# hsinnan75/GSAlign

Hardware: AMD Instinct MI355X
Metric: aligned query Gbp/s (whole node) (higher is better)
Workload: dtype u8; 1 GPU; full-human-sized pair (BASELINE configs[4]): 24 contigs with GRCh38 chromosome lengths, 3.08 Gbp, repeat injection, vs 1; inflight_contexts_per_gpu=8, world_size=1, parallelism=one GPU

## Files before the change

### gsalign_amd/csrc/gsa_api.hip

```cpp
#include <algorithm>
#include <atomic>
#include <chrono>
#include <cstring>
#include <mutex>
#include <thread>
#include <pthread.h>
#include <sched.h>
#include "gsa_ctx.h"

static thread_local std::string g_create_error;

int gsa_fail(gsa_ctx *ctx, int code, const std::string &msg)
{
	if (ctx) ctx->err = msg; else g_create_error = msg;
	return code;
}

int host_stage4_5_6(gsa_ctx *c, int stage);
int host_stage8_finish(gsa_ctx *c);
int build_block_view(gsa_ctx *c);
void bundle_split_lists(gsa_ctx *c);
void bundle_join_lists(gsa_ctx *c);

void collect_events(gsa_ctx *c)
{
	if (!c->profiling && !c->prof_seed) { c->ev_pending = 0; return; }
	float ms;
	if ((c->ev_pending & 1) && !c->profiling) { if (hipEventElapsedTime(&ms, c->ev[0], c->ev[1]) == hipSuccess) { c->kernel_ms[0] = ms; c->acc_seed_ms += ms; } c->ev_pending = 0; (void)hipGetLastError(); return; }
	if (c->ev_pending & 1) {
		if (hipEventElapsedTime(&ms, c->ev[0], c->ev[1]) == hipSuccess) c->kernel_ms[0] = ms;
		if (hipEventElapsedTime(&ms, c->ev[1], c->ev[2]) == hipSuccess) c->kernel_ms[1] = ms;
		if (hipEventElapsedTime(&ms, c->ev[2], c->ev[3]) == hipSuccess) c->kernel_ms[2] = ms;
	}
	if (c->ev_pending & 2) { if (hipEventElapsedTime(&ms, c->ev[4], c->ev[5]) == hipSuccess) c->kernel_ms[3] = ms; }
	c->ev_pending = 0;
	(void)hipGetLastError();
}

void Uploader::run()
{
	(void)hipSetDevice(device);
	for (;;) {
		Job j;
		{ std::unique_lock<std::mutex> g(mu); cv.wait(g, [&] { return stop || !q.empty(); }); if (q.empty()) return; j = std::move(q.front()); q.pop_front(); if (n_demand > 0) n_demand--; }
		const auto t0 = std::chrono::steady_clock::now();
		hipError_t e_first = hipSuccess;
		for (const Piece &p : j.pieces) if (p.n) { const hipError_t e = hipMemcpyAsync(p.dst, p.src, p.n, hipMemcpyHostToDevice, st); if (e != hipSuccess && e_first == hipSuccess) e_first = e; bytes += p.n; }
		{ const hipError_t e = hipStreamSynchronize(st); if (e != hipSuccess && e_first == hipSuccess) e_first = e; }
		(void)hipGetLastError();
		if (e_first != hipSuccess && j.err) { int none = 0; j.err->compare_exchange_strong(none, (int)e_first); }
		const auto t1 = std::chrono::steady_clock::now();
		{ std::lock_guard<std::mutex> g(mu); copy_ms += std::chrono::duration<double, std::milli>(t1 - t0).count(); wait_ms += std::chrono::duration<double, std::milli>(t0 - j.t_push).count(); jobs++; }
		j.busy->fetch_sub(1, std::memory_order_release);
	}
}

static int uploader_start(gsa_ctx *c)
{
	Uploader *u = new Uploader(); u->device = c->device;
	if (hipStreamCreateWithFlags(&u->st, hipStreamNonBlocking) != hipSuccess) { delete u; return gsa_fail(c, GSA_ERR_HIP, "hipStreamCreate (upload stream)"); }
	u->th = std::thread([u] { u->run(); });
	c->up = u; c->own_up = true;
	return GSA_OK;
}

static void uploader_stop(gsa_ctx *c)
{
	if (!c->up || !c->own_up) { c->up = nullptr; return; }
	Uploader *u = c->up;
	{ std::lock_guard<std::mutex> g(u->mu); u->stop = true; }
	u->cv.notify_all();
	if (u->th.joinable()) u->th.join();
#ifdef GSA_EXPERIMENTS
	if (getenv("GSA_UP_STATS") && u->jobs) fprintf(stderr, "[uploader] %lld jobs, %.1f MB each, %.2f ms in the queue, %.2f ms copying (%.1f GB/s)\n", (long long)u->jobs, u->bytes / 1e6 / u->jobs, u->wait_ms / u->jobs, u->copy_ms / u->jobs, u->bytes / 1e6 / u->copy_ms);
#endif
	if (u->st) hipStreamDestroy(u->st);
	delete u; c->up = nullptr;
}

static inline void slot_wait(QuerySlot &s) { while (s.busy.load(std::memory_order_acquire) > 0) std::this_thread::yield(); }
static void slot_demand(gsa_ctx *c, QuerySlot &s)
{
	if (s.busy.load(std::memory_order_acquire) > 0 && c->up) {
		Uploader *u = c->up;
		std::lock_guard<std::mutex> g(u->mu);
		for (size_t k = u->n_demand; k < u->q.size(); k++) if (u->q[k].busy == &s.busy) {
			Uploader::Job j = std::move(u->q[k]); u->q.erase(u->q.begin() + (long)k); u->q.insert(u->q.begin() + (long)u->n_demand, std::move(j)); u->n_demand++;
			break;
		}
	}
	slot_wait(s);
}

static int ctx_private_init(gsa_ctx *c, gsa_ctx *share = nullptr)
{
#ifdef GSA_EXPERIMENTS
	static const int prio = [] { const char *e = getenv("GSA_STREAM_PRIO"); return e ? atoi(e) : 0; }();
	if (prio) {
		int lo = 0, hi = 0; GSA_CHECK(c, hipDeviceGetStreamPriorityRange(&lo, &hi));
		GSA_CHECK(c, hipStreamCreateWithPriority(&c->stream, hipStreamDefault, hi));
		for (int i = 0; i < 4; i++) GSA_CHECK(c, hipStreamCreateWithPriority(&c->stream_aux[i], hipStreamDefault, (i == 0 || i == 3 || (prio > 1 && i == 1)) ? lo : hi));
	} else
#endif
	if (c->prio_mode > 0) {
		int lo = 0, hi = 0; GSA_CHECK(c, hipDeviceGetStreamPriorityRange(&lo, &hi));
		const int mid = (lo + hi) / 2;
		GSA_CHECK(c, hipStreamCreateWithPriority(&c->stream, hipStreamDefault, hi));
		GSA_CHECK(c, hipStreamCreateWithPriority(&c->stream_seed, hipStreamDefault, c->prio_mode == 2 ? lo : mid));
		GSA_CHECK(c, hipEventCreateWithFlags(&c->ev_seed_fork, hipEventDisableTiming));
		for (int i = 0; i < 4; i++) GSA_CHECK(c, hipStreamCreateWithPriority(&c->stream_aux[i], hipStreamDefault, (c->prio_mode == 3 && (i == 0 || i == 3)) ? lo : mid));
	} else {
	GSA_CHECK(c, hipStreamCreate(&c->stream));
	for (int i = 0; i < 4; i++) GSA_CHECK(c, hipStreamCreate(&c->stream_aux[i]));
	}
	if (share) { c->up = share->up; c->own_up = false; } else if (int rc = uploader_start(c)) return rc;
	for (int i = 0; i < 28; i++) GSA_CHECK(c, hipEventCreate(&c->ev[i]));
	GSA_CHECK(c, hipMalloc(&c->d_zero.p, 256)); c->d_zero.cap = 256; GSA_CHECK(c, hipMemset(c->d_zero.p, 0, 256));
	GSA_CHECK(c, hipMalloc(&c->d_cnt.p, 32 * sizeof(u64))); c->d_cnt.cap = 32 * sizeof(u64); GSA_CHECK(c, hipMemset(c->d_cnt.p, 0, 32 * sizeof(u64)));
	GSA_CHECK(c, hipHostMalloc((void **)&c->h_cnt, 16 * sizeof(u64)));
	GSA_CHECK(c, hipMalloc(&c->d_mail.p, MAIL_N * sizeof(i32))); c->d_mail.cap = MAIL_N * sizeof(i32);
	GSA_CHECK(c, hipMemset(c->d_mail.p, 0, MAIL_N * sizeof(i32)));
	GSA_CHECK(c, hipHostMalloc((void **)&c->h_mail, MAIL_N * sizeof(i32)));
	return GSA_OK;
}

static hipError_t h2d_big(void *dst, const void *src, size_t bytes)
{
	if (bytes >= ((size_t)64 << 20) && hipHostRegister(const_cast<void *>(src), bytes, hipHostRegisterDefault) == hipSuccess) {
		const hipError_t e = hipMemcpy(dst, src, bytes, hipMemcpyHostToDevice);
		(void)hipHostUnregister(const_cast<void *>(src));
		return e;
	}
	(void)hipGetLastError();
	return hipMemcpy(dst, src, bytes, hipMemcpyHostToDevice);
}

struct ReservedBuf { void *p = nullptr; size_t bytes = 0; };
static std::mutex g_res_mu; static ReservedBuf g_res[64][2];
void *dev_take_reserved(int device, size_t bytes, size_t *got)
{
	std::lock_guard<std::mutex> g(g_res_mu);
	for (int k = 0; k < 2; k++) { ReservedBuf &r = g_res[device & 63][k]; if (r.p && r.bytes >= bytes && r.bytes <= bytes + bytes / 8 + 4096) { void *p = r.p; *got = r.bytes; r.p = nullptr; r.bytes = 0; return p; } }
	return nullptr;
}

extern "C" {

void gsa_default_params(gsa_params *p)
{
	p->min_seed_len = 15; p->max_indel = 25; p->min_block_score = 200; p->min_aln_len = 200; p->min_identity = 70;
	p->sensitive = 0; p->one_on_one = 0;
}

const char *gsa_last_error(gsa_ctx *ctx) { return ctx ? ctx->err.c_str() : g_create_error.c_str(); }

static int reset_run_state(gsa_ctx *c)
{
	if (c->early_in_flight) { GSA_CHECK(c, hipStreamSynchronize(c->stream_aux[0])); c->early_in_flight = false; }
	c->n_early = 0; c->early_listed = false; c->early_consumed = false;
	c->stage = 0; c->split = false; c->b_lists.clear();
	c->n_seeds = 0; c->n_groups = 0; c->n_blocks2 = 0; c->blocks.clear(); c->frags_stage = 0; c->have_host_seeds = false; c->ev_pending = 0; c->s2_host = false;
	memset(c->counters, 0, sizeof(c->counters)); memset(c->kernel_ms, 0, sizeof(c->kernel_ms));
	return GSA_OK;
}

int gsa_set_params(gsa_ctx *c, const gsa_params *p)
{
	if (!c || !p) return GSA_ERR_ARG;
	if (p->min_seed_len < 1 || p->max_indel < 0) return gsa_fail(c, GSA_ERR_ARG, "bad parameter");
	GSA_CHECK(c, hipSetDevice(c->device));
	if (c->n_borrowers.load() > 0 && (p->sensitive ? 10 : p->min_seed_len) != c->prm.MinSeedLength)
		return gsa_fail(c, GSA_ERR_STATE, "gsa_set_params: contexts cloned from this one read its seed tables -- change -slen / -sen on the clones, or destroy them first");
	if (int rc = reset_run_state(c)) return rc;
	c->prm.MinSeedLength = p->sensitive ? 10 : p->min_seed_len;
	c->prm.MaxIndelSize = p->max_indel; c->prm.MinAlnBlockScore = p->min_block_score; c->prm.MinAlnLength = p->min_aln_len;
	c->prm.MinSeqIdy = p->min_identity; c->prm.bSensitive = p->sensitive ? 1 : 0; c->prm.OneOnOne = p->one_on_one ? 1 : 0;
	return build_presence(c);
}

int gsa_create(int device, const gsa_index_view *idx, const gsa_params *prm, gsa_ctx **out)
{
	return gsa_create_opts(device, idx, prm, 0u, out);
}

int gsa_create_opts(int device, const gsa_index_view *idx, const gsa_params *prm, uint32_t flags, gsa_ctx **out)
{
	if (!idx || !out || !idx->bwt || !idx->sa || !idx->ref || !idx->chr_len || idx->n_chr <= 0 || idx->G <= 0) return gsa_fail(nullptr, GSA_ERR_ARG, "gsa_create: bad index view");
	if (idx->L2[4] != (uint64_t)(2 * idx->G)) return gsa_fail(nullptr, GSA_ERR_ARG, "gsa_create: L2[4] != 2G");
	int ndev = 0;
	if (hipGetDeviceCount(&ndev) != hipSuccess || ndev <= 0) return gsa_fail(nullptr, GSA_ERR_HIP, "no HIP device available (libgsa_hip.so has no CPU path)");
	if (device < 0 || device >= ndev) return gsa_fail(nullptr, GSA_ERR_ARG, "gsa_create: bad device ordinal");
	if (flags & ~(uint32_t)(GSA_CREATE_WIDE | GSA_CREATE_KMER_K(15) | GSA_CREATE_PRIO(3) | GSA_CREATE_REF_PAC)) return gsa_fail(nullptr, GSA_ERR_ARG, "gsa_create_opts: unknown flag");
	{ const uint32_t kk = (flags >> 8) & 15u; if (kk == 1) return gsa_fail(nullptr, GSA_ERR_ARG, "gsa_create_opts: GSA_CREATE_KMER_K takes 2 .. 15 (0: chosen by text length and free memory)"); }
	gsa_ctx *c = new gsa_ctx();
	c->device = device; c->force_wide = (flags & GSA_CREATE_WIDE) != 0; c->opt.kmer_k = (int)((flags >> 8) & 15u); c->prio_mode = (int)((flags >> 16) & 3u);
	memset(c->kernel_ms, 0, sizeof(c->kernel_ms)); memset(c->counters, 0, sizeof(c->counters));
#define CK(call) do { hipError_t e_ = (call); if (e_ != hipSuccess) { gsa_fail(nullptr, GSA_ERR_HIP, std::string(#call) + ": " + hipGetErrorString(e_)); gsa_destroy(c); return GSA_ERR_HIP; } } while (0)
	CK(hipSetDevice(device));
	(void)hipSetDeviceFlags(hipDeviceScheduleSpin);
	(void)hipGetLastError();
	if (int rcp = ctx_private_init(c)) { g_create_error = c->err; gsa_destroy(c); return rcp; }
	const size_t bwt_bytes = ((idx->bwt_words + 15) / 16) * 64;
	CK(hipMalloc(&c->d_bwt_ref.p, bwt_bytes + 64)); c->d_bwt_ref.cap = bwt_bytes + 64;
	CK(hipMemset(c->d_bwt_ref.p, 0, bwt_bytes + 64));
	CK(h2d_big(c->d_bwt_ref.p, idx->bwt, idx->bwt_words * 4));
	CK(hipMalloc(&c->d_sa.p, idx->n_sa * 8)); c->d_sa.cap = idx->n_sa * 8;
	CK(h2d_big(c->d_sa.p, idx->sa, idx->n_sa * 8));
	CK(hipMalloc(&c->d_ref.p, (size_t)2 * idx->G + 64)); c->d_ref.cap = (size_t)2 * idx->G + 64;
	if (flags & GSA_CREATE_REF_PAC) {
		const size_t pac_bytes = ((size_t)idx->G + 3) / 4;
		void *d_pac = nullptr;
		CK(hipMalloc(&d_pac, pac_bytes + 64));
		if (h2d_big(d_pac, idx->ref, pac_bytes) != hipSuccess) { hipFree(d_pac); gsa_fail(nullptr, GSA_ERR_HIP, "hipMemcpy (.pac)"); gsa_destroy(c); return GSA_ERR_HIP; }
		const int rcu = unpack_pac(c, (const uint8_t *)d_pac, idx->G, (uint8_t *)c->d_ref.p);
		(void)hipStreamSynchronize(c->stream); hipFree(d_pac);
		if (rcu) { g_create_error = c->err; gsa_destroy(c); return rcu; }
	} else
	CK(h2d_big(c->d_ref.p, idx->ref, (size_t)2 * idx->G));
	c->G = idx->G;
	{
		i64 tot = 0; std::vector<std::pair<i64, i32> > ends;
		for (int i = 0; i < idx->n_chr; i++) {
			c->h_chr_len.push_back(idx->chr_len[i]); c->h_chr_fwd.push_back(tot); tot += idx->chr_len[i];
			ends.push_back(std::make_pair(c->h_chr_fwd[i] + idx->chr_len[i] - 1, i));
			ends.push_back(std::make_pair(2 * idx->G - tot + idx->chr_len[i] - 1, i));
		}
		if (tot != idx->G) { gsa_fail(nullptr, GSA_ERR_ARG, "gsa_create: sum(chr_len) != G"); gsa_destroy(c); return GSA_ERR_ARG; }
		std::sort(ends.begin(), ends.end());
		for (size_t i = 0; i < ends.size(); i++) { c->h_chr_end.push_back(ends[i].first); c->h_chr_of_end.push_back(ends[i].second); }
	}
	c->d_chr_end.cap = c->h_chr_end.size() * 8; c->d_chr_of_end.cap = c->h_chr_of_end.size() * 4;
	CK(hipMalloc(&c->d_chr_end.p, c->h_chr_end.size() * 8)); CK(hipMemcpy(c->d_chr_end.p, c->h_chr_end.data(), c->h_chr_end.size() * 8, hipMemcpyHostToDevice));
	CK(hipMalloc(&c->d_chr_of_end.p, c->h_chr_of_end.size() * 4)); CK(hipMemcpy(c->d_chr_of_end.p, c->h_chr_of_end.data(), c->h_chr_of_end.size() * 4, hipMemcpyHostToDevice));
#undef CK
	c->di.primary = idx->primary; for (int i = 0; i < 5; i++) c->di.L2[i] = idx->L2[i]; c->di.L2[0] = 0;
	c->di.seq_len = idx->L2[4];
	c->di.bwt = nullptr; c->di.occ_base = nullptr; c->di.occ_shift = 0; c->di.sa = c->d_sa.as<u64>(); c->di.ref = c->d_ref.as<uint8_t>(); c->di.G = idx->G;
	c->di.chr_end = c->d_chr_end.as<i64>(); c->di.chr_of_end = c->d_chr_of_end.as<i32>(); c->di.n_ends = (i32)c->h_chr_end.size();
	c->di.sa32 = nullptr; c->di.sa64 = nullptr; c->di.kmer = nullptr; c->di.kmer_k = 0; c->di.kmer_lo = nullptr; c->di.kmer_lo_k = 0; c->di.kmer_e16 = 0; c->di.ref2 = nullptr; c->di.pres = nullptr; c->di.pres_k = 0;
	{
		const int rco = build_occ(c, c->d_bwt_ref.p, bwt_bytes / 64);
		hipFree(c->d_bwt_ref.p); c->d_bwt_ref.p = nullptr; c->d_bwt_ref.cap = 0;
		if (rco) { g_create_error = c->err; gsa_destroy(c); return rco; }
	}
	if (int rcd = build_dense_sa(c, idx->n_sa)) { g_create_error = c->err; gsa_destroy(c); return rcd; }
	gsa_params dp; gsa_default_params(&dp);
	int rc = gsa_set_params(c, prm ? prm : &dp);
	if (rc) { g_create_error = c->err; gsa_destroy(c); return rc; }
	gsa_release_reserved(device);
	if (const unsigned long long ov = gsa_take_grid_overflow()) { gsa_fail(nullptr, GSA_ERR_LIMIT, "gsa_create: a table build needed a launch of " + std::to_string(ov) + " work-items (>= 2^32)"); gsa_destroy(c); return GSA_ERR_LIMIT; }
	*out = c;
	return GSA_OK;
}

#define GSA_DEVBUFS(X) X(d_bwt) X(d_bwt_ref) X(d_occ_base) X(d_sa) X(d_ref) X(d_chr_end) X(d_chr_of_end) X(qs[0].d_query) X(qs[1].d_query) X(qs[0].d_bndtab) X(qs[1].d_bndtab) X(tmp) X(d_cnt) X(d_zero) X(d_mail) X(d_lb_status[0]) X(d_lb_status[1]) X(d_sa_dense) X(d_kmer) X(d_kmer_lo) X(d_pres) X(d_ref2) X(d_cand_s) X(d_cand_len) X(d_cand_x0) X(d_cand_freq) X(d_onpath) X(d_cand_cnt) X(d_heavy) X(dn_lf) X(dn_x0) X(d_chunk_hits) X(d_chunk_base) X(d_key_a) X(d_key_b) X(d_val_a) X(d_val_b) X(s_q) X(s_len) X(s_r) X(s_gid) X(d_flag) X(d_scan) X(g_beg) X(w_j0) X(d_pdbm) X(d_pdby) X(d_pdcb) X(d_gpre) X(d_key_c) X(d_val_c) X(a_q) X(a_len) X(a_r) X(a_gb) X(a_ge) X(a_uniq) X(a_cu) X(a_alive) X(a_ws) X(a_wid) X(a_next) X(a_brk) X(a_aurank) X(a_aulist) X(a_runinfo) X(w_best) X(w_sum) X(w_n) X(d_btab) X(d_flag2) X(d_scan2) X(d_i64a) X(b_q) X(b_len) X(b_r) X(b_gb) X(b_ge) X(c_q) X(c_len) X(c_r) X(c_gb) X(c_ge) X(c_bid) X(blk_beg) X(blk_end) X(blk_score) X(r_q) X(r_len) X(r_r) X(r_bid) X(r_tmp_q) X(r_tmp_len) X(r_tmp_r) X(r_tmp_bid) X(r_cut4) X(r_cut5) X(r_simjob) X(r_simres) X(d_leaf) X(fb_seedbase) X(fb_sbeg) X(fb_fragbase) X(f_rec) X(f_rec16) X(f_type) X(f_mism) X(f_alnlen) X(f_job) X(f_score) X(d_dp_tiny) X(d_dp_bnd) X(d_dp_ctr) X(d_dp_jobs) X(d_dp_large) X(d_tail) X(e_id) X(e_rec) X(e_list) X(e_off1) X(e_off2) X(e_opsoff) X(e_nops) X(e_ops) X(e_rev) X(r_head) X(f_early) X(r_orig) X(r_tmp_orig) X(j_frag) X(j_opsoff) X(j_nops) X(d_ops) X(j_cells) X(d_alnoff) X(bl_alnlen) X(bl_score) X(d_bblk) X(d_dp_arena) X(d_vblk) X(d_vcnt) X(d_vwg) X(d_var) X(d_cblk) X(d_cout) X(d_ccnt) X(d_cwg) X(d_cpre) X(d_crun) X(d_cops) X(leaf[0]) X(leaf[1]) X(leaf[2]) X(leaf[3]) X(leaf[4]) X(leaf[5]) X(leaf[6]) X(leaf[7]) X(leaf[8])
void gsa_destroy(gsa_ctx *c)
{
	if (!c) return;
	hipSetDevice(c->device);
	if (c->stream) hipStreamSynchronize(c->stream);
	for (int i = 0; i < 2; i++) slot_wait(c->qs[i]);
	uploader_stop(c);
	if (c->lender) c->lender->n_borrowers.fetch_sub(1);
#define X(n) &c->n,
	DevBuf *bufs[] = { GSA_DEVBUFS(X) };
#undef X
	for (DevBuf *b : bufs) if (b->p) hipFree(b->p);
	if (c->h_cnt) hipHostFree(c->h_cnt);
	if (c->h_mail) hipHostFree(c->h_mail);
	for (DevBuf *b : { &c->p_frags, &c->p_tail, &c->p_leaf, &c->p_blk, &c->p_dp, &c->p_sj, &c->p_sj_early, &c->p_jpatch, &c->p_early, &c->qs[0].p_bndtab, &c->qs[1].p_bndtab, &c->p_bblk, &c->p_ba0, &c->p_vblk, &c->p_vhdr, &c->p_var, &c->p_cblk, &c->p_chdr, &c->p_cout, &c->p_cops }) if (b->p) hipHostFree(b->p);
	for (int i = 0; i < 2; i++) if (c->ev_var[i]) hipEventDestroy(c->ev_var[i]);
	for (int i = 0; i < 28; i++) if (c->ev[i]) hipEventDestroy(c->ev[i]);
	for (int i = 0; i < 4; i++) if (c->stream_aux[i]) hipStreamDestroy(c->stream_aux[i]);
	if (c->stream_seed) hipStreamDestroy(c->stream_seed);
	if (c->ev_seed_fork) hipEventDestroy(c->ev_seed_fork);
	if (c->stream) hipStreamDestroy(c->stream);
	delete c;
}

int gsa_clone(gsa_ctx *parent, gsa_ctx **out)
{
	if (!parent || !out) return GSA_ERR_ARG;
	if (hipSetDevice(parent->device) != hipSuccess) return gsa_fail(nullptr, GSA_ERR_HIP, "hipSetDevice");
	gsa_ctx *c = new gsa_ctx();
	c->device = parent->device; c->force_wide = parent->force_wide; c->prio_mode = parent->prio_mode;
	c->index_owner = parent->index_owner ? parent->index_owner : parent; c->seed_budget = parent->seed_budget; c->opt = parent->opt;
	memset(c->kernel_ms, 0, sizeof(c->kernel_ms)); memset(c->counters, 0, sizeof(c->counters));
	if (int rc = ctx_private_init(c, c->index_owner)) { g_create_error = c->err; gsa_destroy(c); return rc; }
	c->di = parent->di; c->G = parent->G;
	c->lender = parent; parent->n_borrowers.fetch_add(1);
	c->h_chr_end = parent->h_chr_end; c->h_chr_fwd = parent->h_chr_fwd; c->h_chr_of_end = parent->h_chr_of_end; c->h_chr_len = parent->h_chr_len;
	c->prm = parent->prm;
	*out = c;
	return GSA_OK;
}

int gsa_clone_to_device(gsa_ctx *parent, int device, gsa_ctx **out)
{
	if (!parent || !out) return GSA_ERR_ARG;
	int ndev = 0;
	if (hipGetDeviceCount(&ndev) != hipSuccess || device < 0 || device >= ndev) { (void)hipGetLastError(); return gsa_fail(nullptr, GSA_ERR_ARG, "gsa_clone_to_device: bad device ordinal"); }
	gsa_ctx *own = parent->index_owner ? parent->index_owner : parent;
	if (hipSetDevice(parent->device) != hipSuccess) return gsa_fail(nullptr, GSA_ERR_HIP, "hipSetDevice");
	if (hipStreamSynchronize(parent->stream) != hipSuccess || hipStreamSynchronize(own->stream) != hipSuccess) return gsa_fail(nullptr, GSA_ERR_HIP, "gsa_clone_to_device: the parent's stream");
	if (hipSetDevice(device) != hipSuccess) return gsa_fail(nullptr, GSA_ERR_HIP, "hipSetDevice");
	(void)hipSetDeviceFlags(hipDeviceScheduleSpin); (void)hipGetLastError();
	gsa_ctx *c = new gsa_ctx();
	c->device = device; c->force_wide = parent->force_wide; c->prio_mode = parent->prio_mode; c->seed_budget = parent->seed_budget; c->opt = parent->opt;
	memset(c->kernel_ms, 0, sizeof(c->kernel_ms)); memset(c->counters, 0, sizeof(c->counters));
	if (int rc = ctx_private_init(c)) { g_create_error = c->err; gsa_destroy(c); return rc; }
	struct Pair { const DevBuf *src; DevBuf *dst; };
	std::vector<Pair> tab = { { &own->d_bwt, &c->d_bwt }, { &own->d_occ_base, &c->d_occ_base }, { &own->d_sa, &c->d_sa }, { &own->d_ref, &c->d_ref }, { &own->d_chr_end, &c->d_chr_end },
		{ &own->d_chr_of_end, &c->d_chr_of_end }, { &own->d_sa_dense, &c->d_sa_dense }, { &own->d_kmer, &c->d_kmer }, { &own->d_ref2, &c->d_ref2 } };
	for (gsa_ctx *src = parent; src; src = src->lender) {
		if (!c->d_pres.cap && src->d_pres.p && (const void *)parent->di.pres == src->d_pres.p) { tab.push_back({ &src->d_pres, &c->d_pres }); c->d_pres.cap = 1; }
		if (!c->d_kmer_lo.cap && src->d_kmer_lo.p && (const void *)parent->di.kmer_lo == src->d_kmer_lo.p) { tab.push_back({ &src->d_kmer_lo, &c->d_kmer_lo }); c->d_kmer_lo.cap = 1; }
	}
	c->d_pres.cap = c->d_kmer_lo.cap = 0;
	auto fail = [&](int code, const std::string &m) { gsa_fail(nullptr, code, m); gsa_destroy(c); return code; };
	for (const Pair &t : tab) {
		if (!t.src->p) continue;
		const size_t bytes = t.src->len ? t.src->len : t.src->cap;
		if (bytes == 0) return fail(GSA_ERR_STATE, "gsa_clone_to_device: an index table of unknown size");
		if (hipMalloc(&t.dst->p, bytes + 256) != hipSuccess) { (void)hipGetLastError(); return fail(GSA_ERR_NOMEM, "gsa_clone_to_device: hipMalloc of an index table"); }
		t.dst->cap = bytes + 256; t.dst->len = bytes;
		const hipError_t e = (device == own->device) ? hipMemcpyAsync(t.dst->p, t.src->p, bytes, hipMemcpyDeviceToDevice, c->stream)
		                                             : hipMemcpyPeerAsync(t.dst->p, device, t.src->p, own->device, bytes, c->stream);
		if (e != hipSuccess) return fail(GSA_ERR_HIP, std::string("gsa_clone_to_device: device-to-device copy: ") + hipGetErrorString(e));
	}
	c->di = parent->di;
	auto move_ptr = [&](const void *p) -> const void * {
		if (!p) return nullptr;
		for (const Pair &t : tab) if (t.src->p && (const char *)p >= (const char *)t.src->p && (const char *)p < (const char *)t.src->p + (t.src->len ? t.src->len : t.src->cap)) return (const char *)t.dst->p + ((const char *)p - (const char *)t.src->p);
		return (const void *)~(uintptr_t)0;
	};
	bool lost = false;
#define MOVE(field, T) do { const void *q_ = move_ptr((const void *)c->di.field); if (q_ == (const void *)~(uintptr_t)0) lost = true; c->di.field = (T)q_; } while (0)
	MOVE(bwt, const uint4 *); MOVE(occ_base, const u64 *); MOVE(sa, const u64 *); MOVE(sa32, const u32 *); MOVE(sa64, const u64 *); MOVE(ref, const uint8_t *); MOVE(ref2, const u32 *);
	MOVE(chr_end, const i64 *); MOVE(chr_of_end, const i32 *); MOVE(kmer, const u64 *); MOVE(kmer_lo, const u64 *); MOVE(pres, const u32 *);
#undef MOVE
	if (lost) return fail(GSA_ERR_STATE, "gsa_clone_to_device: an index pointer outside the tables of its owner");
	c->G = parent->G;
	c->h_chr_end = parent->h_chr_end; c->h_chr_fwd = parent->h_chr_fwd; c->h_chr_of_end = parent->h_chr_of_end; c->h_chr_len = parent->h_chr_len;
	c->prm = parent->prm;
	if (hipStreamSynchronize(c->stream) != hipSuccess) return fail(GSA_ERR_HIP, "gsa_clone_to_device: waiting for the copies");
	*out = c;
	return GSA_OK;
}

static bool device_local_cpus(int device, cpu_set_t *set)
{
	char bus[64] = { 0 };
	if (hipDeviceGetPCIBusId(bus, (int)sizeof(bus) - 1, device) != hipSuccess) { (void)hipGetLastError(); return false; }
	for (char *p = bus; *p; p++) if (*p >= 'A' && *p <= 'Z') *p = (char)(*p - 'A' + 'a');
	char path[160]; snprintf(path, sizeof(path), "/sys/bus/pci/devices/%s/local_cpulist", bus);
	FILE *f = fopen(path, "r"); if (!f) return false;
	char line[4096]; const bool got = fgets(line, sizeof(line), f) != nullptr; fclose(f);
	if (!got) return false;
	CPU_ZERO(set); int n = 0;
	for (char *p = line; *p;) {
		while (*p == ',' || *p == ' ' || *p == '\n') p++;
		if (!*p) break;
		char *e; long a = strtol(p, &e, 10), b = a; if (e == p) break;
		if (*e == '-') { p = e + 1; b = strtol(p, &e, 10); if (e == p) break; }
		for (long k = a; k <= b && k < CPU_SETSIZE; k++) { CPU_SET((int)k, set); n++; }
		p = e;
	}
	return n > 0;
}
int gsa_reserve_index(int device, uint64_t seq_len, uint32_t flags)
{
	int ndev = 0;
	if (hipGetDeviceCount(&ndev) != hipSuccess || device < 0 || device >= ndev || seq_len == 0) { (void)hipGetLastError(); return GSA_ERR_ARG; }
	if (hipSetDevice(device) != hipSuccess) return GSA_ERR_HIP;
	const bool wide = (flags & GSA_CREATE_WIDE) != 0 || seq_len >= 0xFFFFFFF0ull;
	size_t want[2];
	want[0] = ((size_t)seq_len + 1 + 32) * (wide ? 8 : 4) + 256;
	{
		int k = 0; while ((1ull << (2 * k)) < seq_len) k++;
		k += 2; if (k > 15) k = 15;
		size_t fr = 0, tot = 0; if (hipMemGetInfo(&fr, &tot) != hipSuccess) { (void)hipGetLastError(); fr = 8ull << 30; }
		const size_t esz = wide ? 32 : 16;
		while (k > 2 && ((size_t)esz << (2 * k)) > fr / 4) k--;
		const int kk = (int)((flags >> 8) & 15u); if (kk >= 2 && kk <= 15 && ((size_t)esz << (2 * kk)) <= fr / 2) k = kk;
		want[1] = k >= 2 ? ((size_t)esz << (2 * k)) : 0;
	}
	gsa_release_reserved(device);
	for (int k = 0; k < 2; k++) {
		if (!want[k]) continue;
		void *p = nullptr;
		if (hipMalloc(&p, want[k]) != hipSuccess) { (void)hipGetLastError(); continue; }
		std::lock_guard<std::mutex> g(g_res_mu);
		g_res[device & 63][k].p = p; g_res[device & 63][k].bytes = want[k];
	}
	return GSA_OK;
}
void gsa_release_reserved(int device)
{
	void *f[2] = { nullptr, nullptr };
	{ std::lock_guard<std::mutex> g(g_res_mu); for (int k = 0; k < 2; k++) { f[k] = g_res[device & 63][k].p; g_res[device & 63][k].p = nullptr; g_res[device & 63][k].bytes = 0; } }
	if (f[0] || f[1]) { (void)hipSetDevice(device); for (int k = 0; k < 2; k++) if (f[k]) hipFree(f[k]); }
}

int gsa_bind_host_thread(int device)
{
	cpu_set_t set;
	if (!device_local_cpus(device, &set)) return GSA_OK;
	(void)pthread_setaffinity_np(pthread_self(), sizeof(set), &set);
	return GSA_OK;
}

void *gsa_host_alloc(size_t bytes)
{
	void *p = nullptr;
	if (hipHostMalloc(&p, bytes ? bytes : 1) != hipSuccess) { (void)hipGetLastError(); return nullptr; }
	return p;
}
void gsa_host_free(void *p) { if (p) (void)hipHostFree(p); }
int gsa_host_register(void *p, size_t bytes)
{
	if (!p || !bytes) return GSA_ERR_ARG;
	if (hipHostRegister(p, bytes, hipHostRegisterDefault) != hipSuccess) { (void)hipGetLastError(); return GSA_ERR_HIP; }
	return GSA_OK;
}
int gsa_host_unregister(void *p)
{
	if (!p) return GSA_ERR_ARG;
	if (hipHostUnregister(p) != hipSuccess) { (void)hipGetLastError(); return GSA_ERR_HIP; }
	return GSA_OK;
}

int gsa_set_option(gsa_ctx *c, const char *name, int64_t value)
{
	if (!c || !name) return GSA_ERR_ARG;
	const std::string k(name);
	auto in = [&](int64_t lo, int64_t hi) { return value >= lo && value <= hi; };
	const int64_t BIG = (int64_t)1 << 40;
	if (k == "split_min") { if (!in(0, BIG)) return gsa_fail(c, GSA_ERR_ARG, "split_min: 0 .. 2^40 bases"); c->opt.split_min = value; }
	else if (k == "bundle_contig") { if (!in(0, BIG)) return gsa_fail(c, GSA_ERR_ARG, "bundle_contig: 0 (no bundles) .. 2^40 bases"); c->opt.bundle_contig = value; }
	else if (k == "bundle_cap") { if (!in(1, BIG)) return gsa_fail(c, GSA_ERR_ARG, "bundle_cap: 1 .. 2^40 bases"); c->opt.bundle_cap = value; }
	else if (k == "seed_budget") { if (!in(1, 0xffffffffll)) return gsa_fail(c, GSA_ERR_ARG, "seed_budget: 1 .. 2^32 - 1 wave-iterations"); c->seed_budget = (u32)value; }
	else if (k == "dp_lane") { if (!in(0, 1 << 20)) return gsa_fail(c, GSA_ERR_ARG, "dp_lane: 0 (round 2's tiny / small split) .. 2^20 cells"); c->opt.dp_lane = (int)value; }
	else if (k == "seed_mode") { if (value < 0 || value > 2) return gsa_fail(c, GSA_ERR_ARG, "seed_mode: 0 sweep, 1 speculative, 2 search"); c->opt.seed_mode = (int)value; }
	else if (k == "pd_bitmap") c->opt.pd_bitmap = value != 0;
	else if (k == "dp_side") c->opt.dp_side = value != 0;
	else if (k == "dp_small_side") c->opt.dp_small_side = value != 0;
	else if (k == "pd_two_level_min") { if (!in(0, BIG)) return gsa_fail(c, GSA_ERR_ARG, "pd_two_level_min: >= 0 blocks"); c->opt.pd_two_level_min = value; }
	else if (k == "dp_occupancy") { if (!in(0, 16)) return gsa_fail(c, GSA_ERR_ARG, "dp_occupancy: 0 (off) .. 16 workgroups per CU"); c->opt.dp_occupancy = (int)value; }
	else if (k == "pd_bytes") { if (!in(0, 2)) return gsa_fail(c, GSA_ERR_ARG, "pd_bytes: 0 never, 1 by the hit count, 2 always"); c->opt.pd_bytes = (int)value; }
	else if (k == "pres_from_kmer") c->opt.pres_from_kmer = value != 0;
	else if (k == "walk_chain_min") { if (!in(0, BIG)) return gsa_fail(c, GSA_ERR_ARG, "walk_chain_min: >= 0 seeds"); c->opt.walk_chain_min = value; }
	else if (k == "sweep_shape") { if (value < -1 || value > 1) return gsa_fail(c, GSA_ERR_ARG, "sweep_shape: -1, 0 or 1"); c->opt.sweep_shape = (int)value; }
	else if (k == "dp_safe") c->dp_safe = value != 0;
	else if (k == "dp_fake_timeout") { if (!in(0, 1 << 20)) return gsa_fail(c, GSA_ERR_ARG, "dp_fake_timeout: >= 0"); c->dp_fake_timeout = (int)value; }
	else return gsa_fail(c, GSA_ERR_ARG, "gsa_set_option: unknown option " + k);
	return GSA_OK;
}

int gsa_get_wall_sums(gsa_ctx *c, double ms[10], int64_t *n)
{
	if (!c || !ms || !n) return GSA_ERR_ARG;
	memcpy(ms, c->wall_ms, sizeof(c->wall_ms)); *n = c->wall_n;
	if (c->up && c->own_up) { std::lock_guard<std::mutex> g(c->up->mu); ms[9] = c->up->jobs ? c->up->copy_ms / (double)c->up->jobs * (double)c->wall_n : 0.0; }
	return GSA_OK;
}

int gsa_get_alloc_stats(gsa_ctx *c, double *ms, int64_t *n, int64_t *bytes)
{
	if (!c) return GSA_ERR_ARG;
	if (ms) *ms = c->alloc_ms; if (n) *n = c->alloc_n; if (bytes) *bytes = c->alloc_bytes;
	return GSA_OK;
}
int gsa_debug_buffers(gsa_ctx *c, int top)
{
	if (!c) return GSA_ERR_ARG;
	struct E { const char *name; size_t cap, len; };
	std::vector<E> v;
#define X(n) if (c->n.p) v.push_back({ #n, c->n.cap, c->n.len });
	GSA_DEVBUFS(X)
#undef X
	std::sort(v.begin(), v.end(), [](const E &a, const E &b) { return a.cap > b.cap; });
	size_t tot = 0; for (const E &e : v) tot += e.cap;
	fprintf(stderr, "[gsa_debug_buffers] %zu device buffers, %.2f GB held\n", v.size(), (double)tot / 1e9);
	for (size_t k = 0; k < v.size() && (int)k < top; k++) fprintf(stderr, "  %-16s %10.1f MB held  %10.1f MB asked\n", v[k].name, (double)v[k].cap / 1e6, (double)v[k].len / 1e6);
	return GSA_OK;
}
int gsa_set_profiling(gsa_ctx *c, int enable) { if (!c) return GSA_ERR_ARG; c->acc_seed_ms = 0.0; memset(c->wall_ms, 0, sizeof(c->wall_ms)); c->wall_n = 0; if (c->up && c->own_up) { std::lock_guard<std::mutex> g(c->up->mu); c->up->copy_ms = c->up->wait_ms = c->up->bytes = 0; c->up->jobs = 0; } c->var_ms_sum = 0; c->var_calls = 0; c->prof_var = (enable & 8) != 0; c->profiling = (enable & 1) != 0; c->count_blocks = (enable & 2) != 0; c->prof_seed = (enable & 4) != 0; return GSA_OK; }

static int query_geometry(gsa_ctx *c, int32_t qlen)
{
	c->qlen = qlen;
	c->bnd.n = 0; c->bnd.lmax = qlen; c->bnd.pds = 0; c->bnd.off = (const i32 *)c->d_zero.p; c->bnd.chunk_contig = (const uint16_t *)c->d_zero.p;
	c->qbits = ceil_log2_u64((u64)qlen + 1); if (c->qbits < 1) c->qbits = 1;
	c->pd_span = 2 * c->G + (i64)qlen + 2;
	c->pdbits = ceil_log2_u64((u64)c->pd_span);
	if (c->qbits + c->pdbits > 64) return gsa_fail(c, GSA_ERR_LIMIT, "contig too long for the 64-bit seed key");
	return GSA_OK;
}

#define GSA_BUNDLE_MAX_CONTIGS 4096
static void *slot_ensure_bytes(gsa_ctx *c, DevBuf &b, size_t bytes, bool pinned)
{
	if (bytes && bytes <= b.cap) return b.p;
	return pinned ? (void *)pin_ensure<uint8_t>(c, b, bytes) : (void *)dev_ensure<uint8_t>(c, b, bytes);
}

static int slot_layout(gsa_ctx *c, QuerySlot &s, const char *const *query, const int32_t *qlen, int32_t n)
{
	s.b_off.assign((size_t)n + 1, 0); s.b_qlen.assign(qlen, qlen + n); s.src.assign(query, query + n);
	i64 tot = 0; i32 lmax = 0;
	for (int k = 0; k < n; k++) {
		if (qlen[k] < 0 || (qlen[k] > 0 && !query[k])) return GSA_ERR_ARG;
		s.b_off[(size_t)k] = (i32)tot;
		tot += ((i64)qlen[k] + GSA_CHUNK - 1) / GSA_CHUNK * GSA_CHUNK;
		if (tot >= (1ll << 31) - 2 * GSA_CHUNK) return gsa_fail(c, GSA_ERR_LIMIT, "bundle longer than 2^31 bases");
		if (qlen[k] > lmax) lmax = qlen[k];
	}
	s.b_off[(size_t)n] = (i32)tot; s.tot = tot; s.lmax = lmax; s.n = n;
	return GSA_OK;
}

__global__ void __launch_bounds__(256) k_bundle_pad(const i32 *__restrict__ off, const i32 *__restrict__ len, uint8_t *dst)
{
	const i32 k = blockIdx.x; const i64 b = (i64)off[k] + len[k], e = off[k + 1];
	for (i64 t = b + threadIdx.x; t < e; t += 256) dst[t] = (uint8_t)'N';
}

static int slot_upload(gsa_ctx *c, QuerySlot &s, const char *const *query, const int32_t *qlen, int32_t n)
{
	slot_wait(s);
	s.up_err.store(0);
	Uploader::Job job; job.busy = &s.busy; job.err = &s.up_err;
	if (n == 0) {
		s.n = 0; s.tot = qlen[0]; s.lmax = qlen[0]; s.src.assign(1, query[0]); s.b_qlen.assign(1, qlen[0]); s.b_off.clear();
		if (!slot_ensure_bytes(c, s.d_query, (size_t)qlen[0] + 64, false)) return GSA_ERR_NOMEM;
		size_t nb = (size_t)qlen[0];
#ifdef GSA_EXPERIMENTS
		{ static const long long cap = [] { const char *e = getenv("GSA_X_UPBYTES"); return e ? atoll(e) : -1ll; }(); if (cap >= 0 && (size_t)cap < nb) nb = (size_t)cap; }
#endif
		if (nb > 0) { job.pieces.push_back({ s.d_query.p, query[0], nb }); c->up->push(std::move(job)); }
		return GSA_OK;
	}
	if (int rc = slot_layout(c, s, query, qlen, n)) return rc;
	const i64 n_chunks = s.tot / GSA_CHUNK;
	s.o_cc = ((size_t)n + 1) * 4; s.o_src = (s.o_cc + (size_t)n_chunks * 2 + 15) & ~(size_t)15;
	const size_t t_bytes = s.o_src + (size_t)n * 4;
	if (!slot_ensure_bytes(c, s.p_bndtab, t_bytes + 16, true) || !slot_ensure_bytes(c, s.d_bndtab, t_bytes + 16, false) || !slot_ensure_bytes(c, s.d_query, (size_t)s.tot + 64, false)) return GSA_ERR_NOMEM;
	uint8_t *ht = s.p_bndtab.as<uint8_t>();
	memcpy(ht, s.b_off.data(), s.o_cc);
	{ uint16_t *cc = (uint16_t *)(ht + s.o_cc); for (int k = 0; k < n; k++) for (i64 ch = s.b_off[(size_t)k] / GSA_CHUNK; ch < s.b_off[(size_t)k + 1] / GSA_CHUNK; ch++) cc[ch] = (uint16_t)k; }
	memcpy(ht + s.o_src, qlen, (size_t)n * 4);
	job.pieces.push_back({ s.d_bndtab.p, ht, t_bytes });
	for (int k = 0; k < n; k++) if (qlen[k] > 0) job.pieces.push_back({ s.d_query.as<uint8_t>() + s.b_off[(size_t)k], query[k], (size_t)qlen[k] });
	c->up->push(std::move(job));
	return GSA_OK;
}

static int slot_finish(gsa_ctx *c, QuerySlot &s)
{
	slot_demand(c, s);
	if (const int e = s.up_err.exchange(0)) return gsa_fail(c, GSA_ERR_HIP, std::string("query upload (hipMemcpyAsync H2D): ") + hipGetErrorString((hipError_t)e));
	if (s.n > 0 && s.tot > 0) {
		const uint8_t *dt = s.d_bndtab.as<uint8_t>();
		hipLaunchKernelGGL(k_bundle_pad, dim3((unsigned)s.n), dim3(256), 0, c->stream, (const i32 *)dt, (const i32 *)(dt + s.o_src), s.d_query.as<uint8_t>());
		GSA_CHECK(c, hipGetLastError());
	}
	return GSA_OK;
}

static bool slot_holds(const QuerySlot &s, const char *const *query, const int32_t *qlen, int32_t n)
{
	if (!s.pending || s.n != n) return false;
	const int32_t m = n ? n : 1;
	if ((int32_t)s.src.size() != m || (int32_t)s.b_qlen.size() != m) return false;
	for (int32_t k = 0; k < m; k++) if (s.src[(size_t)k] != query[k] || s.b_qlen[(size_t)k] != qlen[k]) return false;
	return true;
}

static int slot_acquire(gsa_ctx *c, const char *const *query, const int32_t *qlen, int32_t n, int *which)
{
	for (int i = 0; i < 2; i++) if (slot_holds(c->qs[i], query, qlen, n)) {
		c->qs[i].pending = false; *which = i;
		return slot_finish(c, c->qs[i]);
	}
	int i = (c->q_cur == 1 && !c->qs[1].pending) ? 1 : 0;
	if (c->qs[i].pending) i ^= 1;
	if (c->qs[i].pending) return gsa_fail(c, GSA_ERR_STATE, "both query slots hold prefetched contigs: align them (or gsa_cancel_prefetch) first");
	*which = i;
	if (int rc = slot_upload(c, c->qs[i], query, qlen, n)) return rc;
	return slot_finish(c, c->qs[i]);
}

static int prefetch(gsa_ctx *c, const char *const *query, const int32_t *qlen, int32_t n)
{
	GSA_CHECK(c, hipSetDevice(c->device));
	int i = c->q_cur == 0 ? 1 : 0;
	if (c->qs[i].pending) i ^= 1;
	if (c->qs[i].pending) return gsa_fail(c, GSA_ERR_STATE, "gsa_prefetch: two contigs are waiting already");
	if (i == c->q_cur && c->stage > 0 && c->stage < 8) return gsa_fail(c, GSA_ERR_STATE, "gsa_prefetch: the free query slot holds the contig whose stages are still running (finish it with gsa_run_to(8) or gsa_set_query first)");
	if (i == c->q_cur) c->q_cur = -2;
	int rc = slot_upload(c, c->qs[i], query, qlen, n);
	if (rc == GSA_OK) c->qs[i].pending = true;
	return rc;
}

int gsa_prefetch_contig(gsa_ctx *c, const char *query, int32_t qlen)
{
	if (!c || !query || qlen < 0) return GSA_ERR_ARG;
	return prefetch(c, &query, &qlen, 0);
}

int gsa_prefetch_bundle(gsa_ctx *c, const char *const *query, const int32_t *qlen, int32_t n)
{
	if (!c || !query || !qlen) return GSA_ERR_ARG;
	if (n < 1 || n > GSA_BUNDLE_MAX_CONTIGS) return gsa_fail(c, GSA_ERR_ARG, "gsa_prefetch_bundle: 1 .. 4096 contigs");
	return prefetch(c, query, qlen, n);
}

int gsa_cancel_prefetch(gsa_ctx *c)
{
	if (!c) return GSA_ERR_ARG;
	if (!c->qs[0].pending && !c->qs[1].pending) return GSA_OK;
	c->qs[0].pending = c->qs[1].pending = false;
	return GSA_OK;
}

int gsa_set_query(gsa_ctx *c, const char *query, int32_t qlen)
{
	if (!c || !query || qlen < 0) return GSA_ERR_ARG;
	GSA_CHECK(c, hipSetDevice(c->device));
	if (int rc = reset_run_state(c)) return rc;
	int w = 0;
	const auto t0 = std::chrono::steady_clock::now();
	if (int rc = slot_acquire(c, &query, &qlen, 0, &w)) return rc;
	c->wall_ms[0] += std::chrono::duration<double, std::milli>(std::chrono::steady_clock::now() - t0).count();
	c->q_cur = w; c->q_dev = c->qs[w].d_query.as<uint8_t>();
	return query_geometry(c, qlen);
}

int gsa_set_query_device(gsa_ctx *c, const char *d_query, int32_t qlen)
{
	if (!c || !d_query || qlen < 0) return GSA_ERR_ARG;
	if (((uintptr_t)d_query & 15) != 0) return gsa_fail(c, GSA_ERR_ARG, "gsa_set_query_device: the buffer must be 16-byte aligned");
	GSA_CHECK(c, hipSetDevice(c->device));
	hipPointerAttribute_t at;
	if (hipPointerGetAttributes(&at, d_query) != hipSuccess || at.type != hipMemoryTypeDevice || at.device != c->device) { (void)hipGetLastError(); return gsa_fail(c, GSA_ERR_ARG, "gsa_set_query_device: not a device buffer of this context's GPU"); }
	if (int rc = reset_run_state(c)) return rc;
	c->q_dev = (const uint8_t *)d_query; c->q_cur = -1;
	return query_geometry(c, qlen);
}

void *gsa_device_alloc(int device, size_t bytes)
{
	void *p = nullptr;
	if (hipSetDevice(device) != hipSuccess || hipMalloc(&p, (bytes ? bytes : 1) + 64) != hipSuccess) { (void)hipGetLastError(); return nullptr; }
	return p;
}
void gsa_device_free(int device, void *p) { if (p && hipSetDevice(device) == hipSuccess) (void)hipFree(p); }
int gsa_device_upload(int device, void *dst, const void *src, size_t bytes)
{
	if (!dst || (!src && bytes)) return GSA_ERR_ARG;
	if (hipSetDevice(device) != hipSuccess || hipMemcpy(dst, src, bytes, hipMemcpyHostToDevice) != hipSuccess) { (void)hipGetLastError(); return GSA_ERR_HIP; }
	return GSA_OK;
}

static int rewind_to_hits(gsa_ctx *c)
{
	const i64 n_seeds = c->n_seeds; const i32 n_groups = c->n_groups;
	if (int rc = reset_run_state(c)) return rc;
	GSA_CHECK(c, hipStreamSynchronize(c->stream));
	c->n_seeds = n_seeds; c->n_groups = n_groups; c->counters[2] = c->counters[3] = (u64)n_seeds;
	c->stage = 1;
	return stage1_restore_pdbm(c);
}

int gsa_rewind(gsa_ctx *c)
{
	if (!c) return GSA_ERR_ARG;
	if (c->qlen <= 0) return gsa_fail(c, GSA_ERR_STATE, "gsa_set_query first");
	if (c->q_cur == -2) return gsa_fail(c, GSA_ERR_STATE, "gsa_rewind: the contig's device copy was overwritten by a prefetch");
	GSA_CHECK(c, hipSetDevice(c->device));
	return reset_run_state(c);
}

int gsa_run_to(gsa_ctx *c, int stage)
{
	if (!c || stage < 0 || stage > 8) return GSA_ERR_ARG;
	if (c->bnd.n && stage < 8 && !c->bundle_call) return gsa_fail(c, GSA_ERR_STATE, "gsa_run_to: the context holds a bundle (gsa_align_bundle runs it); gsa_set_query first");
	if (c->split) return gsa_fail(c, GSA_ERR_STATE, "gsa_run_to: a split contig is finished with gsa_finish_contig");
	GSA_CHECK(c, hipSetDevice(c->device));
	int rc = GSA_OK;
	auto t_prev = std::chrono::steady_clock::now();
	while (c->stage < stage && rc == GSA_OK) {
		const int next = c->stage + 1;
		switch (next) {
		case 1: rc = stage1_seed(c); break;
		case 2: rc = stage2_chain(c); break;
		case 3: rc = stage345_refine(c); if (rc == GSA_OK && c->bnd.n) bundle_split_lists(c); break;
		case 4: case 5: case 6: rc = host_stage4_5_6(c, next); break;
		case 7: if (c->bnd.n) bundle_join_lists(c); rc = stage7_fill(c); break;
		case 8: rc = stage78_extend(c); if (rc == GSA_OK) rc = host_stage8_finish(c); break;
		}
		if (rc == GSA_OK) { c->stage = next; c->frags_stage = (next == 8) ? 8 : 0; }
		{ const auto t_now = std::chrono::steady_clock::now(); c->wall_ms[next] += std::chrono::duration<double, std::milli>(t_now - t_prev).count(); t_prev = t_now; }
	}
	if (stage == 8) c->wall_n++;
	if (const unsigned long long ov = gsa_take_grid_overflow()) rc = gsa_fail(c, GSA_ERR_LIMIT, "a kernel launch of " + std::to_string(ov) + " work-items (>= 2^32) was needed: contig too large for this build");
	if (rc == GSA_OK) { GSA_CHECK(c, hipStreamSynchronize(c->stream)); collect_events(c); }
	if (c->early_in_flight && (rc != GSA_OK || !c->early_consumed)) GSA_CHECK(c, hipStreamSynchronize(c->stream_aux[0]));
	return rc;
}

static int align_uploaded(gsa_ctx *c, gsa_result *out);
int gsa_align_contig(gsa_ctx *c, const char *query, int32_t qlen, gsa_result *out)
{
	if (!c || !out) return GSA_ERR_ARG;
	int rc = gsa_set_query(c, query, qlen); if (rc) return rc;
	return align_uploaded(c, out);
}
int gsa_align_contig_device(gsa_ctx *c, const char *d_query, int32_t qlen, gsa_result *out)
{
	if (!c || !out) return GSA_ERR_ARG;
	int rc = gsa_set_query_device(c, d_query, qlen); if (rc) return rc;
	return align_uploaded(c, out);
}
static int align_uploaded(gsa_ctx *c, gsa_result *out)
{
	int rc;
	c->dp_timeout = false;
	rc = gsa_run_to(c, 8);
	if (rc == GSA_ERR_STATE && c->dp_timeout && !c->dp_safe) {
		c->dp_timeout = false; c->dp_safe = true;
		rc = gsa_rewind(c);
		if (rc == GSA_OK) rc = gsa_run_to(c, 8);
		c->dp_safe = false;
	}
	if (rc) return rc;
	return gsa_get_blocks(c, out);
}

struct BundleSrc { const uint8_t *p; i32 len, _pad; };
__global__ void __launch_bounds__(256) k_bundle_gather(const i32 *__restrict__ off, const uint16_t *__restrict__ chunk_contig, const BundleSrc *__restrict__ src, uint8_t *dst)
{
	const i32 chunk = blockIdx.x, ci = chunk_contig[chunk];
	const i64 g0 = (i64)chunk * GSA_CHUNK; const i32 l0 = (i32)(g0 - off[ci]);
	const BundleSrc sc = src[ci];
	const i32 have = sc.len - l0 < GSA_CHUNK ? sc.len - l0 : GSA_CHUNK;
	for (i32 t = threadIdx.x; t < GSA_CHUNK; t += 256) dst[g0 + t] = t < have ? sc.p[l0 + t] : (uint8_t)'N';
}

static int set_query_bundle(gsa_ctx *c, const char *const *query, const int32_t *qlen, int32_t n, bool dev_q)
{
	if (n < 1 || n > GSA_BUNDLE_MAX_CONTIGS) return gsa_fail(c, GSA_ERR_ARG, "gsa_align_bundle: 1 .. 4096 contigs");
	GSA_CHECK(c, hipSetDevice(c->device));
	if (int rc = reset_run_state(c)) return rc;
	int w = 0;
	if (!dev_q) { if (int rc = slot_acquire(c, query, qlen, n, &w)) return rc; }
	else {
		w = (c->q_cur == 1 && !c->qs[1].pending) ? 1 : 0;
		if (c->qs[w].pending) w ^= 1;
		if (c->qs[w].pending) return gsa_fail(c, GSA_ERR_STATE, "both query slots hold prefetched contigs");
		QuerySlot &s = c->qs[w];
		slot_wait(s);
		for (int k = 0; k < n; k++) if (qlen[k] > 0) {
			hipPointerAttribute_t at;
			if (!query[k] || hipPointerGetAttributes(&at, query[k]) != hipSuccess || at.type != hipMemoryTypeDevice || at.device != c->device) { (void)hipGetLastError(); return gsa_fail(c, GSA_ERR_ARG, "gsa_align_bundle (GSA_MANY_DEVICE): not a device buffer of this context's GPU"); }
		}
		if (int rc = slot_layout(c, s, query, qlen, n)) return rc;
		const i64 n_chunks = s.tot / GSA_CHUNK;
		s.o_cc = ((size_t)n + 1) * 4; s.o_src = (s.o_cc + (size_t)n_chunks * 2 + 15) & ~(size_t)15;
		const size_t t_bytes = s.o_src + (size_t)n * sizeof(BundleSrc);
		if (!slot_ensure_bytes(c, s.p_bndtab, t_bytes + 16, true) || !slot_ensure_bytes(c, s.d_bndtab, t_bytes + 16, false) || !slot_ensure_bytes(c, s.d_query, (size_t)s.tot + 64, false)) return GSA_ERR_NOMEM;
		uint8_t *ht = s.p_bndtab.as<uint8_t>();
		memcpy(ht, s.b_off.data(), s.o_cc);
		{ uint16_t *cc = (uint16_t *)(ht + s.o_cc); for (int k = 0; k < n; k++) for (i64 ch = s.b_off[(size_t)k] / GSA_CHUNK; ch < s.b_off[(size_t)k + 1] / GSA_CHUNK; ch++) cc[ch] = (uint16_t)k; }
		{ BundleSrc *bs = (BundleSrc *)(ht + s.o_src); for (int k = 0; k < n; k++) { bs[k].p = (const uint8_t *)query[k]; bs[k].len = qlen[k]; bs[k]._pad = 0; } }
		GSA_CHECK(c, hipMemcpyAsync(s.d_bndtab.p, ht, t_bytes, hipMemcpyHostToDevice, c->stream));
		const uint8_t *dt = s.d_bndtab.as<uint8_t>();
		if (s.tot > 0) {
			hipLaunchKernelGGL(k_bundle_gather, dim3((unsigned)n_chunks), dim3(256), 0, c->stream, (const i32 *)dt, (const uint16_t *)(dt + s.o_cc), (const BundleSrc *)(dt + s.o_src), s.d_query.as<uint8_t>());
			GSA_CHECK(c, hipGetLastError());
		}
	}
	const QuerySlot &s = c->qs[w];
	c->q_cur = w; c->b_off = s.b_off; c->b_qlen = s.b_qlen;
	const uint8_t *dt = s.d_bndtab.as<uint8_t>();
	c->q_dev = s.d_query.as<uint8_t>();
	c->qlen = (i32)s.tot;
	c->bnd.n = n; c->bnd.lmax = s.lmax; c->bnd.off = (const i32 *)dt; c->bnd.chunk_contig = (const uint16_t *)(dt + s.o_cc);
	c->bnd.pds = (2 * c->G + (i64)s.lmax + (i64)c->prm.MaxIndelSize + 64 + 31) & ~31ll;
	c->qbits = ceil_log2_u64((u64)s.tot + 1); if (c->qbits < 1) c->qbits = 1;
	c->pd_span = (i64)n * c->bnd.pds + 2;
	c->pdbits = ceil_log2_u64((u64)c->pd_span);
	if (c->qbits + c->pdbits > 64) return gsa_fail(c, GSA_ERR_LIMIT, "bundle too long for the 64-bit seed key");
	return GSA_OK;
}

static void bundle_result(gsa_ctx *c, int k, const std::vector<i64> &a0, size_t blk_at, gsa_result *out)
{
	out->n_blocks = c->b_nblk[(size_t)k]; out->blocks = c->h_blocks.data() + blk_at;
	out->n_frags = c->b_frag0[(size_t)k + 1] - c->b_frag0[(size_t)k]; out->recs = c->p_frags.as<gsa_rec>() + c->b_frag0[(size_t)k];
	out->n_aln = a0[(size_t)k + 1] - a0[(size_t)k]; out->aln1 = c->h_taln1 + a0[(size_t)k]; out->aln2 = c->h_taln2 + a0[(size_t)k];
}

int gsa_align_bundle(gsa_ctx *c, const char *const *query, const int32_t *qlen, int32_t n, uint32_t flags, gsa_result *out)
{
	if (!c || !query || !qlen || !out || (flags & ~(uint32_t)GSA_MANY_DEVICE)) return GSA_ERR_ARG;
	int rc = set_query_bundle(c, query, qlen, n, (flags & GSA_MANY_DEVICE) != 0); if (rc) return rc;
	c->dp_timeout = false;
	c->bundle_call = true;
	struct Clear { gsa_ctx *c; ~Clear() { c->bundle_call = false; } } clear_{ c };
	rc = gsa_run_to(c, 8);
	if (rc == GSA_ERR_STATE && c->dp_timeout && !c->dp_safe) {
		c->dp_timeout = false; c->dp_safe = true;
		{ const Bundle keep = c->bnd; rc = reset_run_state(c); c->bnd = keep; }
		if (rc == GSA_OK) rc = gsa_run_to(c, 8);
		c->dp_safe = false;
	}
	if (rc) return rc;
	const size_t nfb = c->b_blk0.empty() ? 0 : (size_t)c->b_blk0[(size_t)n];
	if (nfb == 0 || c->n_frags == 0) {
		for (int k = 0; k < n; k++) { out[k].n_blocks = 0; out[k].n_frags = 0; out[k].n_aln = 0; out[k].blocks = nullptr; out[k].recs = nullptr; out[k].aln1 = out[k].aln2 = nullptr; }
		return GSA_OK;
	}
	std::vector<i64> a0((size_t)n + 1, c->n_aln);
	for (int k = n - 1; k >= 0; k--) a0[(size_t)k] = c->b_blk0[(size_t)k] < c->b_blk0[(size_t)k + 1] ? c->p_ba0.as<i64>()[k] : a0[(size_t)k + 1];
	size_t at = 0;
	for (int k = 0; k < n; k++) { bundle_result(c, k, a0, at, &out[k]); at += (size_t)c->b_nblk[(size_t)k]; }
	return GSA_OK;
}

int gsa_seed_chunks(gsa_ctx *c, const char *query, int32_t qlen, int32_t chunk_beg, int32_t chunk_end)
{
	if (!c || chunk_beg < 0 || chunk_end < chunk_beg) return GSA_ERR_ARG;
	int rc = gsa_set_query(c, query, qlen); if (rc) return rc;
	c->split = true; c->rng_beg = chunk_beg; c->rng_end = chunk_end;
	rc = stage1_seed(c);
	if (rc == GSA_OK) GSA_CHECK(c, hipStreamSynchronize(c->stream));
	collect_events(c);
	return rc;
}

int64_t gsa_hit_count(gsa_ctx *c) { return (c && c->split) ? c->n_seeds : 0; }

int gsa_export_hits(gsa_ctx *c, uint64_t *keys, uint32_t *vals)
{
	if (!c || !c->split) return c ? gsa_fail(c, GSA_ERR_STATE, "gsa_seed_chunks first") : GSA_ERR_ARG;
	if (c->n_seeds == 0) return GSA_OK;
	if (!keys || !vals) return GSA_ERR_ARG;
	GSA_CHECK(c, hipSetDevice(c->device));
	GSA_CHECK(c, hipMemcpyAsync(keys, c->d_key_a.p, (size_t)c->n_seeds * 8, hipMemcpyDefault, c->stream));
	GSA_CHECK(c, hipMemcpyAsync(vals, c->d_val_a.p, (size_t)c->n_seeds * 4, hipMemcpyDefault, c->stream));
	GSA_CHECK(c, hipStreamSynchronize(c->stream));
	return GSA_OK;
}

int gsa_import_hits(gsa_ctx *c, const uint64_t *keys, const uint32_t *vals, int64_t n)
{
	if (!c || n < 0 || (n > 0 && (!keys || !vals))) return GSA_ERR_ARG;
	if (!c->split || c->stage != 0) return gsa_fail(c, GSA_ERR_STATE, "gsa_seed_chunks first");
	GSA_CHECK(c, hipSetDevice(c->device));
	return stage1_import_hits(c, (const u64 *)keys, (const u32 *)vals, n);
}

int gsa_finish_contig(gsa_ctx *c, gsa_result *out)
{
	if (!c || !out) return GSA_ERR_ARG;
	if (!c->split || c->stage != 0) return gsa_fail(c, GSA_ERR_STATE, "gsa_seed_chunks first");
	GSA_CHECK(c, hipSetDevice(c->device));
	int rc = stage1_finish_split(c); if (rc) return rc;
	c->stage = 1; c->split = false;
	c->dp_timeout = false;
	rc = gsa_run_to(c, 8);
	if (rc == GSA_ERR_STATE && c->dp_timeout && !c->dp_safe) {
		c->dp_timeout = false; c->dp_safe = true;
		rc = rewind_to_hits(c);
		if (rc == GSA_OK) rc = gsa_run_to(c, 8);
		c->dp_safe = false;
	}
	if (rc) return rc;
	return gsa_get_blocks(c, out);
}

int gsa_hit_buffers(gsa_ctx *c, const uint64_t **keys, const uint32_t **vals)
{
	if (!c || !keys || !vals) return GSA_ERR_ARG;
	if (!c->split) return gsa_fail(c, GSA_ERR_STATE, "gsa_seed_chunks first");
	*keys = c->d_key_a.as<uint64_t>(); *vals = c->d_val_a.as<uint32_t>();
	return GSA_OK;
}

static int align_split(gsa_ctx *const *grp, int n_grp, const char *query, int32_t qlen, gsa_result *out)
{
	const int32_t n_chunks = (int32_t)(((int64_t)qlen + GSA_CHUNK - 1) / GSA_CHUNK);
	std::vector<int> rcs((size_t)n_grp, GSA_OK);
	std::vector<std::thread> th;
	auto range = [&](int k, int32_t &b, int32_t &e) { const int32_t base = n_chunks / n_grp, extra = n_chunks % n_grp; b = k * base + (k < extra ? k : extra); e = b + base + (k < extra ? 1 : 0); };
	for (int k = 1; k < n_grp; k++) th.emplace_back([&, k] { int32_t b, e; range(k, b, e); rcs[(size_t)k] = gsa_seed_chunks(grp[k], query, qlen, b, e); });
	{ int32_t b, e; range(0, b, e); rcs[0] = gsa_seed_chunks(grp[0], query, qlen, b, e); }
	for (std::thread &t : th) t.join();
	for (int k = 0; k < n_grp; k++) if (rcs[(size_t)k] != GSA_OK) { if (k) gsa_fail(grp[0], rcs[(size_t)k], std::string("helper context: ") + gsa_last_error(grp[k])); return rcs[(size_t)k]; }
	for (int k = 1; k < n_grp; k++) {
		const uint64_t *kp = nullptr; const uint32_t *vp = nullptr;
		int rc = gsa_hit_buffers(grp[k], &kp, &vp);
		if (rc == GSA_OK) rc = gsa_import_hits(grp[0], kp, vp, gsa_hit_count(grp[k]));
		if (rc != GSA_OK) return rc;
	}
	return gsa_finish_contig(grp[0], out);
}

int gsa_call_variants(gsa_ctx *c, int32_t k, gsa_variants *out)
{
	if (!c || !out) return GSA_ERR_ARG;
	out->n = 0; out->v = nullptr; out->n_snv = out->n_ins = out->n_del = 0;
	if (c->stage != 8 || c->split) return gsa_fail(c, GSA_ERR_STATE, "gsa_call_variants: the context holds no finished (stage 8) result");
	if (c->q_cur == -2) return gsa_fail(c, GSA_ERR_STATE, "gsa_call_variants: the contig's device copy was overwritten by a prefetch");
	if (k < 0 || k >= (c->bnd.n ? c->bnd.n : 1)) return gsa_fail(c, GSA_ERR_ARG, "gsa_call_variants: contig index out of range");
	GSA_CHECK(c, hipSetDevice(c->device));
	return call_variants(c, k, out);
}

int gsa_get_variant_timing(gsa_ctx *c, double *ms_sum, int64_t *n_calls)
{
	if (!c || !ms_sum || !n_calls) return GSA_ERR_ARG;
	*ms_sum = c->var_ms_sum; *n_calls = (int64_t)c->var_calls;
	return GSA_OK;
}

int gsa_block_cigars(gsa_ctx *c, int32_t k, gsa_cigars *out)
{
	if (!c || !out) return GSA_ERR_ARG;
	out->n_blocks = 0; out->n_ops = 0; out->blk = nullptr; out->ops = nullptr;
	if (c->stage != 8 || c->split) return gsa_fail(c, GSA_ERR_STATE, "gsa_block_cigars: the context holds no finished (stage 8) result");
	if (c->q_cur == -2) return gsa_fail(c, GSA_ERR_STATE, "gsa_block_cigars: the contig's device copy was overwritten by a prefetch");
	if (k < 0 || k >= (c->bnd.n ? c->bnd.n : 1)) return gsa_fail(c, GSA_ERR_ARG, "gsa_block_cigars: contig index out of range");
	GSA_CHECK(c, hipSetDevice(c->device));
	const auto t0 = std::chrono::steady_clock::now();
	const int rc = block_cigars(c, k, out);
	c->cig_ms_sum += std::chrono::duration<double, std::milli>(std::chrono::steady_clock::now() - t0).count(); c->cig_calls++;
	return rc;
}

int gsa_get_cigar_timing(gsa_ctx *c, double *ms_sum, int64_t *n_calls)
{
	if (!c || !ms_sum || !n_calls) return GSA_ERR_ARG;
	*ms_sum = c->cig_ms_sum; *n_calls = (int64_t)c->cig_calls;
	return GSA_OK;
}

struct ManySink { gsa_result_fn on_result = nullptr; gsa_result_var_fn on_var = nullptr; gsa_result_ex_fn on_ex = nullptr; uint32_t want = 0; };
static int align_many_impl(gsa_ctx *const *ctx, int32_t n_ctx, const char *const *query, const int32_t *qlen, int32_t n, uint32_t flags, const ManySink &sk, void *user)
{
	auto deliver = [&](gsa_ctx *c, int32_t k, int32_t ci, const gsa_result *res) -> int {
		if (sk.on_var) { gsa_variants var; const int rcv = gsa_call_variants(c, k, &var); return rcv != GSA_OK ? rcv : sk.on_var(user, ci, res, &var); }
		if (sk.on_ex) {
			gsa_variants var; gsa_cigars cig; gsa_extras ex = { nullptr, nullptr };
			if (sk.want & GSA_WANT_VARIANTS) { const int rcv = gsa_call_variants(c, k, &var); if (rcv != GSA_OK) return rcv; ex.var = &var; }
			if (sk.want & GSA_WANT_CIGARS) { const int rcc = gsa_block_cigars(c, k, &cig); if (rcc != GSA_OK) return rcc; ex.cig = &cig; }
			return sk.on_ex(user, ci, res, &ex);
		}
		return sk.on_result ? sk.on_result(user, ci, res) : GSA_OK;
	};
	if (flags & ~(uint32_t)(GSA_MANY_IN_ORDER | GSA_MANY_DEVICE | GSA_MANY_NO_SPLIT | GSA_MANY_NO_BUNDLE | GSA_MANY_NO_PREFETCH)) return GSA_ERR_ARG;
	if (!ctx || n_ctx <= 0 || n < 0 || (n > 0 && (!query || !qlen))) return GSA_ERR_ARG;
	for (int k = 0; k < n_ctx; k++) if (!ctx[k]) return GSA_ERR_ARG;
	const bool dev_q = (flags & GSA_MANY_DEVICE) != 0;
	if (dev_q) for (int k = 1; k < n_ctx; k++) if (ctx[k]->device != ctx[0]->device) return gsa_fail(ctx[0], GSA_ERR_ARG, "GSA_MANY_DEVICE: the contexts must share one GPU (the contigs live in its memory)");
	if (n == 0) return GSA_OK;
	std::vector<int32_t> order((size_t)n);
	for (int32_t i = 0; i < n; i++) order[(size_t)i] = i;
	if (!(flags & GSA_MANY_IN_ORDER)) std::stable_sort(order.begin(), order.end(), [&](int32_t a, int32_t b) { return qlen[a] > qlen[b]; });
	std::atomic<int> err(GSA_OK);
	const int64_t split_min = ctx[0]->opt.split_min;
	int64_t longest = 0; for (int32_t i = 0; i < n; i++) if (qlen[i] > longest) longest = qlen[i];
	if (n < n_ctx && !dev_q && !(flags & GSA_MANY_NO_SPLIT) && longest >= split_min) {
		std::vector<int> gsz((size_t)n, 1);
		for (int left = n_ctx - n; left > 0; left--) {
			int best = -1; double load = 0;
			for (int i = 0; i < n; i++) { const int32_t ci = order[(size_t)i]; if ((int64_t)qlen[ci] < split_min) continue; const double l = (double)qlen[ci] / gsz[(size_t)i]; if (l > load) { load = l; best = i; } }
			if (best < 0) break;
			gsz[(size_t)best]++;
		}
		std::vector<std::thread> th; int at = 0;
		for (int i = 0; i < n; i++) {
			const int32_t ci = order[(size_t)i]; gsa_ctx *const *grp = ctx + at; const int ng = gsz[(size_t)i]; at += ng;
			th.emplace_back([&, ci, grp, ng] {
				gsa_result res;
				int rc = ng > 1 ? align_split(grp, ng, query[ci], qlen[ci], &res) : gsa_align_contig(grp[0], query[ci], qlen[ci], &res);
				if (rc == GSA_OK) rc = deliver(grp[0], 0, ci, &res);
				if (rc != GSA_OK) { int ok = GSA_OK; err.compare_exchange_strong(ok, rc); }
			});
		}
		for (std::thread &t : th) t.join();
		return err.load();
	}
	const int64_t bundle_contig = ctx[0]->opt.bundle_contig, bundle_cap = ctx[0]->opt.bundle_cap;
	std::vector<std::vector<int32_t> > units;
	{
		bool may = !(flags & GSA_MANY_NO_BUNDLE) && bundle_contig > 0;
		for (int k = 0; k < n_ctx; k++) if (ctx[k]->profiling || ctx[k]->count_blocks) may = false;
		int64_t small_total = 0; int32_t n_small = 0;
		for (int32_t i = 0; i < n; i++) if ((int64_t)qlen[i] <= bundle_contig) { small_total += qlen[i]; n_small++; }
		if (n_small < 2) may = false;
		size_t max_contigs = GSA_BUNDLE_MAX_CONTIGS;
		{
			const int qb = ceil_log2_u64((u64)(bundle_cap + bundle_cap / 8 + bundle_contig) + 1);
			const u64 stride = (u64)(2 * ctx[0]->G) + (u64)bundle_contig + (u64)ctx[0]->prm.MaxIndelSize + 96;
			const u64 fit = qb < 62 ? (1ull << (63 - qb)) / stride : 0;
			if (fit < max_contigs) max_contigs = (size_t)fit;
			if (max_contigs < 2) may = false;
		}
#ifdef GSA_EXPERIMENTS
		static const int64_t bundle_target = [] { const char *e = getenv("GSA_BUNDLE_TARGET"); return e ? (int64_t)atoll(e) : 0ll; }();
#else
		const int64_t bundle_target = 0;
#endif
		int64_t n_bundles = (small_total + bundle_cap - 1) / (bundle_cap > 0 ? bundle_cap : 1); if (n_bundles < 1) n_bundles = 1;
		n_bundles = (n_bundles + n_ctx - 1) / n_ctx * n_ctx;
		int64_t target = small_total / n_bundles + 1;
		if (bundle_target > 0) target = bundle_target;
		int64_t cur = 0;
		for (int32_t i = 0; i < n; i++) {
			const int32_t ci = order[(size_t)i];
			const bool small = may && (int64_t)qlen[ci] <= bundle_contig;
			if (!small) { units.push_back(std::vector<int32_t>(1, ci)); cur = 0; continue; }
			const int64_t padded = ((int64_t)qlen[ci] + GSA_CHUNK - 1) / GSA_CHUNK * GSA_CHUNK;
			if (cur > 0 && (cur + padded / 2 > target || cur + padded > bundle_cap + bundle_cap / 8 || units.back().size() >= max_contigs)) cur = 0;
			if (cur == 0) units.push_back(std::vector<int32_t>());
			units.back().push_back(ci); cur += padded > 0 ? padded : 1;
		}
	}
	const int32_t n_units = (int32_t)units.size();
	std::atomic<int32_t> next(0);
	auto one = [&](gsa_ctx *c, int32_t ci) {
		gsa_result res;
		int rc = dev_q ? gsa_align_contig_device(c, query[ci], qlen[ci], &res) : gsa_align_contig(c, query[ci], qlen[ci], &res);
		if (rc == GSA_OK) rc = deliver(c, 0, ci, &res);
		return rc;
	};
	const bool pre = !dev_q && !(flags & GSA_MANY_NO_PREFETCH);
	auto loop = [&](gsa_ctx *c) {
		std::vector<const char *> bq, pq; std::vector<int32_t> bl, pl; std::vector<gsa_result> br;
		auto fetch = [&](int32_t u) {
			if (!pre || u >= n_units) return;
			const std::vector<int32_t> &un = units[(size_t)u];
			if (un.size() == 1) (void)gsa_prefetch_contig(c, query[un[0]], qlen[un[0]]);
			else { pq.clear(); pl.clear(); for (int32_t ci : un) { pq.push_back(query[ci]); pl.push_back(qlen[ci]); } (void)gsa_prefetch_bundle(c, pq.data(), pl.data(), (int32_t)un.size()); }
		};
		(void)gsa_cancel_prefetch(c);
		int32_t u = next.fetch_add(1);
		fetch(u);
		for (;;) {
			if (u >= n_units || err.load() != GSA_OK) { (void)gsa_cancel_prefetch(c); return; }
			const int32_t u_next = next.fetch_add(1);
			fetch(u_next);
			const std::vector<int32_t> &un = units[(size_t)u];
			int rc = GSA_OK;
			if (un.size() == 1) rc = one(c, un[0]);
			else {
				bq.clear(); bl.clear(); br.resize(un.size());
				for (int32_t ci : un) { bq.push_back(query[ci]); bl.push_back(qlen[ci]); }
				rc = gsa_align_bundle(c, bq.data(), bl.data(), (int32_t)un.size(), dev_q ? GSA_MANY_DEVICE : 0u, br.data());
				if (rc == GSA_OK) { for (size_t k = 0; k < un.size() && rc == GSA_OK; k++) rc = deliver(c, (int32_t)k, un[k], &br[k]); }
				else if (rc == GSA_ERR_LIMIT) { rc = GSA_OK; for (size_t k = 0; k < un.size() && rc == GSA_OK; k++) rc = one(c, un[k]); }
			}
			if (rc != GSA_OK) { int ok = GSA_OK; err.compare_exchange_strong(ok, rc); (void)gsa_cancel_prefetch(c); return; }
			u = u_next;
		}
	};
	std::vector<std::thread> th;
	for (int k = 1; k < n_ctx && k < n_units; k++) th.emplace_back(loop, ctx[k]);
	loop(ctx[0]);
	for (std::thread &t : th) t.join();
	return err.load();
}

int gsa_align_many(gsa_ctx *const *ctx, int32_t n_ctx, const char *const *query, const int32_t *qlen, int32_t n, uint32_t flags, gsa_result_fn on_result, void *user)
{
	ManySink sk; sk.on_result = on_result;
	return align_many_impl(ctx, n_ctx, query, qlen, n, flags, sk, user);
}
int gsa_align_many_variants(gsa_ctx *const *ctx, int32_t n_ctx, const char *const *query, const int32_t *qlen, int32_t n, uint32_t flags, gsa_result_var_fn on_result, void *user)
{
	if (!on_result) return GSA_ERR_ARG;
	ManySink sk; sk.on_var = on_result;
	return align_many_impl(ctx, n_ctx, query, qlen, n, flags, sk, user);
}
int gsa_align_many_ex(gsa_ctx *const *ctx, int32_t n_ctx, const char *const *query, const int32_t *qlen, int32_t n, uint32_t flags, uint32_t want, gsa_result_ex_fn on_result, void *user)
{
	if (!on_result || (want & ~(uint32_t)(GSA_WANT_VARIANTS | GSA_WANT_CIGARS))) return GSA_ERR_ARG;
	ManySink sk; sk.on_ex = on_result; sk.want = want;
	return align_many_impl(ctx, n_ctx, query, qlen, n, flags, sk, user);
}

int64_t gsa_seed_count(gsa_ctx *c) { return c ? c->n_seeds : 0; }

int gsa_get_seeds(gsa_ctx *c, gsa_seed *out)
{
	if (!c || (!out && c->n_seeds)) return GSA_ERR_ARG;
	if (c->stage < 1) return gsa_fail(c, GSA_ERR_STATE, "run stage 1 first");
	const size_t n = (size_t)c->n_seeds; if (!n) return GSA_OK;
	{ int rc = seed_view_sort(c); if (rc) return rc; GSA_CHECK(c, hipStreamSynchronize(c->stream)); }
	std::vector<i32> q(n), l(n); std::vector<i64> r(n);
	GSA_CHECK(c, hipMemcpy(q.data(), c->s_q.p, n * 4, hipMemcpyDeviceToHost));
	GSA_CHECK(c, hipMemcpy(l.data(), c->s_len.p, n * 4, hipMemcpyDeviceToHost));
	GSA_CHECK(c, hipMemcpy(r.data(), c->s_r.p, n * 8, hipMemcpyDeviceToHost));
	for (size_t i = 0; i < n; i++) { out[i].qpos = q[i]; out[i].len = l[i]; out[i].rpos = r[i]; }
	return GSA_OK;
}

int gsa_group_count(gsa_ctx *c)
{
	if (!c) return 0;
	if (c->n_groups < 0) {
		if (seed_view_sort(c) != GSA_OK) return 0;
		hipStreamSynchronize(c->stream);
		i32 ng = 0;
		if (hipMemcpy(&ng, c->d_mail.as<i32>() + M_NG, 4, hipMemcpyDeviceToHost) != hipSuccess) return 0;
		c->n_groups = ng;
	}
	return c->n_groups;
}

int gsa_get_groups(gsa_ctx *c, int32_t *beg, int32_t *end)
{
	if (!c) return GSA_ERR_ARG;
	if (c->stage < 1) return gsa_fail(c, GSA_ERR_STATE, "run stage 1 first");
	const size_t ng = (size_t)gsa_group_count(c); if (!ng) return GSA_OK;
	std::vector<i32> gb(ng + 1);
	GSA_CHECK(c, hipMemcpy(gb.data(), c->g_beg.p, (ng + 1) * 4, hipMemcpyDeviceToHost));
	for (size_t i = 0; i < ng; i++) { beg[i] = gb[i]; end[i] = gb[i + 1]; }
	return GSA_OK;
}

int gsa_get_blocks(gsa_ctx *c, gsa_result *out)
{
	if (!c || !out) return GSA_ERR_ARG;
	if (c->stage < 2) return gsa_fail(c, GSA_ERR_STATE, "run stage 2 first");
	if (c->bnd.n && c->stage < 8) return gsa_fail(c, GSA_ERR_STATE, "gsa_get_blocks: the context holds a bundle -- only its finished result (gsa_align_bundle's out[]) is defined per contig");
	if (c->frags_stage != c->stage) { int rc = build_block_view(c); if (rc) return rc; }
	out->n_blocks = (int32_t)c->h_blocks.size(); out->blocks = c->h_blocks.data();
	if (c->result_pinned && c->stage == 8) {
		out->n_frags = c->n_frags; out->n_aln = c->n_aln;
		out->recs = c->p_frags.as<gsa_rec>(); out->aln1 = c->h_taln1; out->aln2 = c->h_taln2;
	} else {
		out->n_frags = (int64_t)c->h_frags.size(); out->n_aln = (int64_t)c->h_aln1.size();
		out->recs = c->h_frags.data(); out->aln1 = c->h_aln1.data(); out->aln2 = c->h_aln2.data();
	}
	return GSA_OK;
}

int gsa_get_counters(gsa_ctx *c, uint64_t counters[8]) { if (!c) return GSA_ERR_ARG; memcpy(counters, c->counters, sizeof(c->counters)); return GSA_OK; }
int gsa_get_timings(gsa_ctx *c, float ms[8]) { if (!c) return GSA_ERR_ARG; memcpy(ms, c->kernel_ms, sizeof(c->kernel_ms)); if (c->prof_seed && !c->profiling) ms[6] = (float)c->acc_seed_ms; return GSA_OK; }
int gsa_get_seed_stats(gsa_ctx *c, uint64_t st[8]) { if (!c) return GSA_ERR_ARG; memcpy(st, c->dbg, sizeof(c->dbg)); return GSA_OK; }

}
```

### gsalign_amd/csrc/gsa_ctx.h

```cpp
#ifndef GSA_CTX_H
#define GSA_CTX_H
#include <atomic>
#include <chrono>
#include <condition_variable>
#include <deque>
#include <mutex>
#include <thread>
#include "gsa_internal.h"

struct Leaf {
	i32 beg, end;
	i32 sumlen;
	i32 q_first, q_last_end;
	i64 r_first, r_last_end;
	i32 blk;
	i32 cut4, cut5;
	i32 blk_score;
};

enum { M_NB = 0, M_NC = 1, M_NBLK = 2, M_NG = 3, M_NR = 4, M_NJ = 5, M_NL = 6, M_LBERR = 7, M_ANY = 8, M_NTINY = 40, M_TICKET = 48, M_NBRAW = 49, M_NR2 = 50, M_NF = 51, M_NJOB = 52, M_OPSTOT = 53, M_NALN = 54, M_DPERR = 64, M_NLARGE = 65, M_DPERR2 = 66, M_CELLS = 68  , M_DPERR3 = 41, M_LBDONE = 42, M_LFSTEPS = 44 , M_NEARLY = 62, M_EOPS = 63, M_NTOUCH = 46 , M_MAXBLK = 56 , MAIL_N = 72 };
#define LEAF_CHUNK 1024

struct HostBlock {
	i32 leaf_beg, leaf_end;
	i32 score;
	i32 bdup;
	i32 aln_len, bdir, gpos, chr;
};

struct QuerySlot {
	DevBuf d_query;
	DevBuf d_bndtab, p_bndtab;
	std::vector<i32> b_off, b_qlen;
	std::vector<const char *> src;
	i32 n = 0;
	i32 lmax = 0; i64 tot = 0; size_t o_cc = 0, o_src = 0;
	bool pending = false;
	std::atomic<int> busy{0};
	std::atomic<int> up_err{0};
};

struct Uploader {
	struct Piece { void *dst; const void *src; size_t n; };
	struct Job { std::vector<Piece> pieces; std::atomic<int> *busy; std::atomic<int> *err; std::chrono::steady_clock::time_point t_push; };
	double copy_ms = 0, wait_ms = 0, bytes = 0; long long jobs = 0;
	int device = 0; hipStream_t st = nullptr;
	std::thread th; std::mutex mu; std::condition_variable cv; std::deque<Job> q; bool stop = false;
	size_t n_demand = 0;
	void run();
	void push(Job &&j) { j.busy->fetch_add(1); j.t_push = std::chrono::steady_clock::now(); { std::lock_guard<std::mutex> g(mu); q.push_back(std::move(j)); } cv.notify_one(); }
};

struct Options {
	int64_t split_min = 20000000;
	int64_t bundle_contig = 16000000;
	int64_t bundle_cap = 64000000;
	int dp_lane = 512;
	int seed_mode = 1;
	int pd_bitmap = 1;
	int sweep_shape = -1;
	int dp_small_side = 0;
	int dp_side = 0;
	int64_t walk_chain_min = 100000;
	int64_t pd_two_level_min = 2000000;
	int dp_occupancy = 0;
	int pd_bytes = 1;
	int pres_from_kmer = 1;
	int kmer_k = 0;
};

struct gsa_ctx {
	int device = 0;
	Options opt;
	Uploader *up = nullptr; bool own_up = false;
	hipStream_t stream = nullptr;
	hipStream_t stream_seed = nullptr;
	hipEvent_t ev_seed_fork = nullptr;
	u64 seed_ticket = 0;
	int n_cus = 0;
	hipStream_t stream_aux[4] = {nullptr, nullptr, nullptr, nullptr};
	std::string err;
	Params prm;
	DevIndex di;
	gsa_ctx *index_owner = nullptr;
	gsa_ctx *lender = nullptr;
	std::atomic<int> n_borrowers{0};
	int prio_mode = 0;
	bool force_wide = false;
	bool profiling = false;
	bool prof_seed = false;
	bool count_blocks = false;
	u64 dbg[8] = {0, 0, 0, 0, 0, 0, 0, 0};
	hipEvent_t ev[28];
	float kernel_ms[8];
	double wall_ms[10] = {0, 0, 0, 0, 0, 0, 0, 0, 0, 0}; int64_t wall_n = 0;
	double acc_seed_ms = 0.0;
	u64 counters[8];

	DevBuf d_bwt, d_bwt_ref, d_occ_base, d_sa, d_ref, d_chr_end, d_chr_of_end;
	std::vector<i64> h_chr_end, h_chr_fwd; std::vector<i32> h_chr_of_end, h_chr_len;
	i64 G = 0;

	QuerySlot qs[2]; int q_cur = -1;
	i32 qlen = 0; int stage = 0;
	const uint8_t *q_dev = nullptr;
	bool split = false; i64 rng_beg = 0, rng_end = 0;
	int qbits = 1, pdbits = 1;
	i64 pd_span = 0;

	Bundle bnd = { 0, 0, 0, nullptr, nullptr }; bool bundle_call = false;
	std::vector<i32> b_off, b_qlen;
	std::vector<std::vector<HostBlock> > b_lists;
	std::vector<i32> b_blk0;
	DevBuf d_bblk, p_bblk, p_ba0;
	std::vector<i32> b_nblk; std::vector<i64> b_frag0;

	DevBuf tmp;
	DevBuf leaf[9];
	DevBuf d_cnt; u64 *h_cnt = nullptr;
	DevBuf d_mail; i32 *h_mail = nullptr;
	DevBuf d_lb_status[2]; u32 lb_epoch = 0, lb_base = 0;
	DevBuf p_leaf;
	int ev_pending = 0;
	bool s2_host = false;

	DevBuf d_ref2;
	DevBuf d_kmer;
	DevBuf d_kmer_lo;
	DevBuf d_pres;
	DevBuf d_sa_dense;
	DevBuf d_cand_s, d_cand_len, d_cand_x0, d_cand_freq, d_onpath, d_cand_cnt;
	size_t cand_cap_per_chunk = 1536;
	DevBuf d_heavy, dn_lf, dn_x0;
	bool seed_sweep_next = false, seed_sweep_probe = false; int seed_sweep_run = 0, seed_sweep_period = 8;
	u32 seed_budget = 256;
	DevBuf d_chunk_hits, d_chunk_base;
	DevBuf d_key_a, d_key_b, d_val_a, d_val_b;
	i64 n_seeds = 0; bool hits_sorted = false;
	DevBuf s_q, s_len, s_r, s_gid;
	DevBuf d_flag, d_scan;
	i32 n_groups = 0;
	bool pd_path = false, seed_view_ready = false, pdbm_dirty = true; i64 pd_words = 0;
	DevBuf w_j0; u32 walk_ticket = 0, walk_epoch = 0;
	DevBuf d_zero;
	DevBuf d_pdby; bool pd_bytes = false;
	DevBuf d_pdcb;
	DevBuf d_pdbm, d_gpre, d_key_c, d_val_c;
	DevBuf g_beg;

	i64 n_a = 0;
	DevBuf a_q, a_len, a_r, a_gb, a_ge;
	DevBuf a_uniq, a_cu, a_alive, a_ws, a_wid;
	DevBuf a_next, a_brk, a_aurank, a_aulist, a_runinfo;
	DevBuf w_best, w_sum, w_n;
	DevBuf d_btab;
	DevBuf d_flag2, d_scan2, d_i64a;
	i64 n_b = 0, n_c = 0;
	DevBuf b_q, b_len, b_r, b_gb, b_ge;
	DevBuf c_q, c_len, c_r, c_gb, c_ge;
	DevBuf c_bid;
	i32 n_blocks2 = 0;
	DevBuf blk_beg, blk_end, blk_score;
	std::vector<i32> h_blk_beg, h_blk_end, h_blk_score;

	i64 n_r = 0;
	DevBuf r_q, r_len, r_r, r_bid, r_tmp_q, r_tmp_len, r_tmp_r, r_tmp_bid;
	DevBuf r_cut4, r_cut5, r_simjob, r_simres;
	DevBuf d_leaf; std::vector<Leaf> h_leaf;
	std::vector<HostBlock> blocks;
	std::vector<i32> h_r_q, h_r_len; std::vector<i64> h_r_r;
	bool have_host_seeds = false;

	i64 n_frags = 0, n_aln = 0;
	i32 n_large = 0;
	DevBuf p_jpatch; i32 n_jobs = 0;
	DevBuf d_tail, p_tail;
	const i32 *h_tmail = nullptr, *h_tpatch = nullptr; char *h_taln1 = nullptr, *h_taln2 = nullptr;
	i64 nf_ub = 0, span_ub = 0;
	DevBuf fb_seedbase, fb_sbeg, fb_fragbase;
	DevBuf f_rec;
	DevBuf f_rec16;
	DevBuf f_type, f_mism, f_alnlen, f_job, f_score;
	DevBuf j_frag, j_opsoff, j_nops, d_ops, j_cells;
	DevBuf d_dp_tiny;
	DevBuf d_dp_arena;
	DevBuf d_dp_bnd, d_dp_ctr, d_dp_jobs, d_dp_large;
	DevBuf e_id, e_rec, e_list, e_off1, e_off2, e_opsoff, e_nops, e_ops, e_rev, r_head, f_early, r_orig, r_tmp_orig, p_early;
	bool early_consumed = false;
	bool early_listed = false;
	i32 n_early = 0; bool early_in_flight = false; std::vector<i32> h_early;
	bool dp_dirty = true;
	bool dp_timeout = false, dp_safe = false;
	int dp_fake_timeout = 0;
	u32 dp_epoch = 0;
	DevBuf p_dp, p_sj, p_sj_early;
	DevBuf d_alnoff;
	DevBuf bl_alnlen, bl_score;
	std::vector<gsa_rec> h_frags; std::vector<gsa_block> h_blocks; std::vector<char> h_aln1, h_aln2;
	int frags_stage = 0;
	DevBuf p_frags, p_blk; bool result_pinned = false;
	DevBuf d_vblk, d_vcnt, d_vwg, d_var, p_vblk, p_vhdr, p_var;
	bool prof_var = false; hipEvent_t ev_var[2] = {nullptr, nullptr}; double var_ms_sum = 0; long long var_calls = 0;
	DevBuf d_cblk, d_cout, d_ccnt, d_cwg, d_cpre, d_crun, d_cops, p_cblk, p_chdr, p_cout, p_cops;
	double cig_ms_sum = 0; long long cig_calls = 0;
	double alloc_ms = 0; long long alloc_n = 0, alloc_bytes = 0;
};

static inline void ctx_quiesce(gsa_ctx *c)
{
	hipStreamSynchronize(c->stream);
	for (int i = 0; i < 4; i++) if (c->stream_aux[i]) hipStreamSynchronize(c->stream_aux[i]);
}

void *dev_take_reserved(int device, size_t bytes, size_t *got);
template <class T> static inline T *dev_ensure(gsa_ctx *c, DevBuf &b, size_t n, bool exact = false)
{
	size_t bytes = (n ? n : 1) * sizeof(T);
	b.len = bytes;
	if (bytes <= b.cap) return (T *)b.p;
	const auto t0_ = std::chrono::steady_clock::now();
	if (b.p) { ctx_quiesce(c); hipFree(b.p); b.p = nullptr; b.cap = 0; }
	size_t want = exact ? bytes + 256 : bytes + bytes / 2 + 256;
	if (exact && bytes >= ((size_t)1 << 30)) { size_t got = 0; if (void *r = dev_take_reserved(c->device, want, &got)) { b.p = r; b.cap = got; return (T *)b.p; } }
	if (hipMalloc(&b.p, want) != hipSuccess) { gsa_fail(c, GSA_ERR_NOMEM, "hipMalloc"); return nullptr; }
	b.cap = want;
	c->alloc_ms += std::chrono::duration<double, std::milli>(std::chrono::steady_clock::now() - t0_).count(); c->alloc_n++; c->alloc_bytes += (long long)want;
	return (T *)b.p;
}

template <class T> static inline T *pin_ensure(gsa_ctx *c, DevBuf &b, size_t n)
{
	size_t bytes = (n ? n : 1) * sizeof(T);
	if (bytes <= b.cap) return (T *)b.p;
	const auto t0_ = std::chrono::steady_clock::now();
	if (b.p) { ctx_quiesce(c); hipHostFree(b.p); b.p = nullptr; b.cap = 0; }
	size_t want = bytes + bytes / 4 + 4096;
	if (hipHostMalloc(&b.p, want) != hipSuccess) { gsa_fail(c, GSA_ERR_NOMEM, "hipHostMalloc"); return nullptr; }
	b.cap = want;
	c->alloc_ms += std::chrono::duration<double, std::milli>(std::chrono::steady_clock::now() - t0_).count(); c->alloc_n++; c->alloc_bytes += (long long)want;
	return (T *)b.p;
}

int build_dense_sa(gsa_ctx *c, u64 n_sa);
int unpack_pac(gsa_ctx *c, const uint8_t *d_pac, i64 G, uint8_t *d_ref);
int build_occ(gsa_ctx *c, const void *ref_layout, u64 n_blocks128);
int build_presence(gsa_ctx *c);
int stage1_seed(gsa_ctx *c);
int stage1_import_hits(gsa_ctx *c, const u64 *keys, const u32 *vals, i64 n);
int stage1_finish_split(gsa_ctx *c);
int stage1_restore_pdbm(gsa_ctx *c);
int seed_view_sort(gsa_ctx *c);
int stage2_chain(gsa_ctx *c);
int launch_early_dp(gsa_ctx *c);
int stage2_fetch_host(gsa_ctx *c);
void collect_events(gsa_ctx *c);
int stage345_refine(gsa_ctx *c);
int stage7_fill(gsa_ctx *c);
i64 frags_count(gsa_ctx *c);
int stage78_extend(gsa_ctx *c);
int run_gapsim_jobs(gsa_ctx *c, i32 n, const i32 *d_n, const i32 *d_q1, const i32 *d_q2, const i64 *d_r1, const i64 *d_r2, i32 *d_res, const i32 *d_jseed, i32 *d_cut4);
void dp_count_cells(gsa_ctx *c, i32 n_ub, const i32 *len1, const i32 *len2, hipStream_t stream);
int call_variants(gsa_ctx *c, i32 k, gsa_variants *out);
int block_cigars(gsa_ctx *c, i32 k, gsa_cigars *out);
struct LgJob { i32 job, m, n; };
int launch_stripes(gsa_ctx *c, hipStream_t ss, std::vector<LgJob> &large, const uint8_t *pool1, const i64 *off1, const uint8_t *pool2, const i64 *off2,
                   uint8_t *ops, const i64 *ops_off, i32 *ops_len, uint8_t *rev, int err_slot);
struct Ksw2Launch { i32 n = 0, nsmall = 0, nlarge = 0; bool small_in_flight = false; };
int run_ksw2_jobs(gsa_ctx *c, i32 n_ub, const uint8_t *pool1, const i64 *off1, const i32 *len1,
                  const uint8_t *pool2, const i64 *off2, const i32 *len2, uint8_t *ops, const i64 *ops_off, i32 *ops_len, i64 ops_total, Ksw2Launch *out,
                  const i32 *jfrag = nullptr, gsa_frag *frag = nullptr, bool mail_clean = false);

#endif
```

### gsalign_amd/csrc/gsa_scan.h

```cpp
#ifndef GSA_SCAN_H
#define GSA_SCAN_H
#include <algorithm>
#include "gsa_ctx.h"

#ifndef LB_TPB
#define LB_TPB 256
#endif
#ifndef LB_GRID_PER_CU
#define LB_GRID_PER_CU 2
#endif
#ifndef LB_BATCH
#define LB_BATCH 4
#endif
#ifndef LB_ITEMS
#define LB_ITEMS 8
#endif

#ifdef LB_TIMING
static __device__ unsigned long long g_lb_prof[8];
#define LB_T(K) { if (tid == 0) { const unsigned long long t_ = wall_clock64(); atomicAdd(&g_lb_prof[K], t_ - t_last); t_last = t_; } }
#else
#define LB_T(K)
#endif
struct LbArgs {
	unsigned long long *status[2];
	u32 *ticket;
	u32 base, epoch; i32 n_tiles;
	i32 *err;
	u32 *finished;
};
#include <type_traits>
template <class T, class = void> struct lb_has_finish : std::false_type {};
template <class T> struct lb_has_finish<T, std::void_t<decltype(&T::finish)>> : std::true_type {};
template <class T, class = void> struct lb_has_item : std::false_type {};
template <class T> struct lb_has_item<T, std::void_t<typename T::Item>> : std::true_type {};
template <class T, class = void> struct lb_is_clamped : std::false_type {};
template <class T> struct lb_is_clamped<T, std::void_t<decltype(T::clamped)>> : std::integral_constant<bool, T::clamped> {};
template <class T, class = void> struct lb_has_prep : std::false_type {};
template <class T> struct lb_has_prep<T, std::void_t<decltype(&T::prep)>> : std::true_type {};
template <class T> __device__ __forceinline__ void lb_pin(T &x)
{
	static_assert(sizeof(T) % 4 == 0, "Items are made of 32- and 64-bit fields");
	u32 w[sizeof(T) / 4];
	__builtin_memcpy(w, &x, sizeof(T));
#pragma unroll
	for (unsigned k = 0; k < sizeof(T) / 4; k++) asm volatile("" : "+v"(w[k]));
	__builtin_memcpy(&x, w, sizeof(T));
}
template <class T, class = void> struct lb_has_emit_all : std::false_type {};
template <class T> struct lb_has_emit_all<T, std::void_t<decltype(T::has_emit_all)>> : std::true_type {};
template <class T, bool = lb_has_item<T>::value> struct lb_item_of { struct type {}; };
template <class T> struct lb_item_of<T, true> { using type = typename T::Item; };

__device__ __forceinline__ unsigned long long lb_pack(u32 epoch, u32 flag, u32 val) { return ((unsigned long long)(epoch & 0x3fffffffu) << 34) | ((unsigned long long)flag << 32) | val; }

template <int NV>
__device__ __forceinline__ void lb_tile_prefix(const LbArgs &lb, int tile, const i32 (&agg)[NV], i32 (&pre)[NV], i32 *s_bcast)
{
	const int tid = threadIdx.x, lane = tid & 63;
	const u32 ep = lb.epoch & 0x3fffffffu;
	if (tile == 0) {
		if (tid == 0) {
#pragma unroll
			for (int c = 0; c < NV; c++) { __hip_atomic_store(&lb.status[c][0], lb_pack(ep, 2, (u32)agg[c]), __ATOMIC_RELAXED, __HIP_MEMORY_SCOPE_AGENT); s_bcast[c] = 0; }
		}
	} else if (tid < 64) {
		if (lane == 0) {
#pragma unroll
			for (int c = 0; c < NV; c++) __hip_atomic_store(&lb.status[c][tile], lb_pack(ep, 1, (u32)agg[c]), __ATOMIC_RELAXED, __HIP_MEMORY_SCOPE_AGENT);
		}
		i32 excl[NV]; bool fin[NV];
#pragma unroll
		for (int c = 0; c < NV; c++) { excl[c] = 0; fin[c] = false; }
#ifndef LB_WAIT_TICKS
#define LB_WAIT_TICKS 500000000ull
#endif
#ifndef LB_WIN
#define LB_WIN 64
#endif
		for (int base = tile - 1;; base -= LB_WIN) {
			const int idx = base - lane;
			unsigned long long w[NV];
			int first[NV];
			u32 spins = 0; unsigned long long t_spin0 = 0;
			for (;;) {
				bool settled = true;
#pragma unroll
				for (int c = 0; c < NV; c++) {
					w[c] = lb_pack(ep, 2, 0);
					first[c] = 0;
					if (fin[c]) continue;
					if (LB_WIN < 64 && lane >= LB_WIN) w[c] = lb_pack(ep, 1, 0);
					else if (idx >= 0) w[c] = __hip_atomic_load(&lb.status[c][idx], __ATOMIC_RELAXED, __HIP_MEMORY_SCOPE_AGENT);
				}
#pragma unroll
				for (int c = 0; c < NV; c++) {
					if (fin[c]) continue;
					const bool rdy = (u32)(w[c] >> 34) == ep && ((w[c] >> 32) & 3) != 0;
					const unsigned long long p2 = __ballot(rdy && ((w[c] >> 32) & 3) == 2), nr = __ballot(!rdy);
					first[c] = p2 ? __ffsll((long long)p2) - 1 : 64;
					const unsigned long long need = first[c] >= 63 ? ~0ull : ((2ull << first[c]) - 1ull);
					if (nr & need) settled = false;
				}
				if (settled) break;
				if ((++spins & 1023u) == 0 && (t_spin0 == 0 ? (t_spin0 = wall_clock64(), false) : wall_clock64() - t_spin0 > LB_WAIT_TICKS)) {
					if (lane == 0) *lb.err = 1;
#pragma unroll
					for (int c = 0; c < NV; c++) { w[c] = lb_pack(ep, 2, 0); first[c] = 0; }
					break;
				}
				__builtin_amdgcn_s_sleep(1);
			}
			bool all_fin = true;
#pragma unroll
			for (int c = 0; c < NV; c++) {
				if (fin[c]) continue;
				i32 v = lane <= first[c] ? (i32)(u32)w[c] : 0;
				for (int o = 32; o; o >>= 1) v += __shfl_xor(v, o);
				excl[c] += v;
				if (first[c] < 64) fin[c] = true; else all_fin = false;
			}
			if (all_fin) break;
		}
		if (lane == 0) {
#pragma unroll
			for (int c = 0; c < NV; c++) { __hip_atomic_store(&lb.status[c][tile], lb_pack(ep, 2, (u32)(excl[c] + agg[c])), __ATOMIC_RELAXED, __HIP_MEMORY_SCOPE_AGENT); s_bcast[c] = excl[c]; }
		}
	}
	__syncthreads();
#pragma unroll
	for (int c = 0; c < NV; c++) pre[c] = s_bcast[c];
}

__device__ __forceinline__ void lb_pub(i32 *p, i32 v) { __hip_atomic_store(p, v, __ATOMIC_RELAXED, __HIP_MEMORY_SCOPE_AGENT); }

__device__ __forceinline__ void lb_copy_out(i32 *dst, const i32 *src, i32 n, int tid)
{
	for (i32 t0 = 0; t0 < n; t0 += 8 * LB_TPB) {
		i32 v[8];
#pragma unroll
		for (int u = 0; u < 8; u++) { const i32 t = t0 + u * LB_TPB + tid; v[u] = t < n ? __hip_atomic_load(&src[t], __ATOMIC_RELAXED, __HIP_MEMORY_SCOPE_AGENT) : 0; }
#pragma unroll
		for (int u = 0; u < 8; u++) { const i32 t = t0 + u * LB_TPB + tid; if (t < n) dst[t] = v[u]; }
	}
}

#ifndef LB_MIN_WAVES
#define LB_MIN_WAVES 1
#endif
#ifdef LB_BISECT
template <class T, class = void> struct lb_id_of { static constexpr int value = -1; };
template <class T> struct lb_id_of<T, std::void_t<decltype(T::lb_id)>> { static constexpr int value = T::lb_id; };
#define LB_BOUND_OF(Op_) (lb_id_of<Op_>::value == (LB_BISECT) ? 4 : 1)
#else
#define LB_BOUND_OF(Op_) LB_MIN_WAVES
#endif
template <int NV, class Op, int ITEMS>
__global__ void __launch_bounds__(LB_TPB, LB_BOUND_OF(Op)) k_lb_pass(i64 n, Op op, LbArgs lb)
{
	constexpr int LB_TILE = LB_TPB * ITEMS;
	__shared__ i32 s_tile, s_bcast[2], s_wsum[NV][ITEMS][LB_TPB / 64];
	const int tid = threadIdx.x, lane = tid & 63, wv = tid >> 6;
#ifdef LB_TIMING
	unsigned long long t_last = wall_clock64();
#endif
	for (bool first = true;; first = false) {
	if (!first && (i32)gridDim.x >= lb.n_tiles) break;
	__syncthreads();
	if (tid == 0) s_tile = (i32)(atomicAdd(lb.ticket, 1u) - lb.base);
	__syncthreads();
	const int tile = s_tile;
	LB_T(0)
	if (tile >= lb.n_tiles) break;
	const i64 i0 = (i64)tile * LB_TILE + tid;
	i32 v[NV][ITEMS], inc[NV][ITEMS];
	typename lb_item_of<Op>::type item[ITEMS];
	if constexpr (lb_has_item<Op>::value) {
		if constexpr (lb_is_clamped<Op>::value) {
			if (n > 0) {
#pragma unroll
				for (int k0 = 0; k0 < ITEMS; k0 += LB_BATCH) {
#pragma unroll
					for (int k = k0; k < k0 + LB_BATCH && k < ITEMS; k++) { const i64 i = i0 + (i64)k * LB_TPB; item[k] = op.load(i < n ? i : n - 1); }
#pragma unroll
					for (int k = k0; k < k0 + LB_BATCH && k < ITEMS; k++) lb_pin(item[k]);
					if constexpr (lb_has_prep<Op>::value) {
#pragma unroll
						for (int k = k0; k < k0 + LB_BATCH && k < ITEMS; k++) { const i64 i = i0 + (i64)k * LB_TPB; if (i < n) op.prep(item[k], i); }
					}
				}
			}
		} else {
#pragma unroll
			for (int k = 0; k < ITEMS; k++) { const i64 i = i0 + (i64)k * LB_TPB; if (i < n) item[k] = op.load(i); }
			if constexpr (lb_has_prep<Op>::value) {
#pragma unroll
				for (int k = 0; k < ITEMS; k++) { const i64 i = i0 + (i64)k * LB_TPB; if (i < n) op.prep(item[k], i); }
			}
		}
	}
#pragma unroll
	for (int k = 0; k < ITEMS; k++) {
		const i64 i = i0 + (i64)k * LB_TPB;
#pragma unroll
		for (int c = 0; c < NV; c++) {
			if constexpr (lb_has_item<Op>::value) v[c][k] = i < n ? op.value(item[k], i, c) : 0;
			else v[c][k] = i < n ? op.value(i, c) : 0;
		}
	}
#pragma unroll
	for (int c = 0; c < NV; c++)
#pragma unroll
		for (int k = 0; k < ITEMS; k++) {
			i32 x = v[c][k];
			for (int o = 1; o < 64; o <<= 1) { const i32 t = __shfl_up(x, o); if (lane >= o) x += t; }
			inc[c][k] = x;
			if (lane == 63) s_wsum[c][k][wv] = x;
		}
	__syncthreads();
	i32 agg[NV];
#pragma unroll
	for (int c = 0; c < NV; c++) {
		i32 run = 0;
#pragma unroll
		for (int k = 0; k < ITEMS; k++) {
			i32 wo = 0, tot = 0;
#pragma unroll
			for (int w = 0; w < LB_TPB / 64; w++) { const i32 sw = s_wsum[c][k][w]; if (w < wv) wo += sw; tot += sw; }
			inc[c][k] += run + wo - v[c][k];
			run += tot;
		}
		agg[c] = run;
	}
	i32 pre[NV];
	LB_T(1)
	lb_tile_prefix<NV>(lb, tile, agg, pre, s_bcast);
	LB_T(2)
#ifdef LB_TIMING
	if (tid == 0) atomicAdd(&g_lb_prof[4], 1ull);
#endif
	i32 vv[NV], ee[NV];
	if constexpr (lb_has_emit_all<Op>::value) {
		static_assert(NV == 1, "emit_all: one component");
		i32 ex0[ITEMS]; bool in[ITEMS];
#pragma unroll
		for (int k = 0; k < ITEMS; k++) { ex0[k] = pre[0] + inc[0][k]; in[k] = i0 + (i64)k * LB_TPB < n; }
		op.emit_all(item, i0, in, v[0], ex0);
#pragma unroll
		for (int k = 0; k < ITEMS; k++) if (i0 + (i64)k * LB_TPB == n - 1) { i32 tt[1] = { ex0[k] + v[0][k] }; op.done(tt); }
	} else {
#pragma unroll
	for (int k = 0; k < ITEMS; k++) {
		const i64 i = i0 + (i64)k * LB_TPB;
#pragma unroll
		for (int c = 0; c < NV; c++) { vv[c] = v[c][k]; ee[c] = pre[c] + inc[c][k]; }
		if (i < n) {
			if constexpr (lb_has_item<Op>::value) op.emit(item[k], i, vv, ee);
			else op.emit(i, vv, ee);
			if (i == n - 1) { i32 tt[NV]; for (int c = 0; c < NV; c++) tt[c] = ee[c] + vv[c]; op.done(tt); }
		}
	}
	}
	if (n == 0 && tile == 0 && tid == 0) { i32 tt[NV]; for (int c = 0; c < NV; c++) tt[c] = 0; op.done(tt); }
#ifdef LB_TIMING
	asm volatile("s_waitcnt vmcnt(0)" ::: "memory");
#endif
	LB_T(3)
	}
	if constexpr (lb_has_finish<Op>::value) {
		__shared__ int s_last;
		asm volatile("s_waitcnt vmcnt(0)" ::: "memory");
		__syncthreads();
		if (tid == 0) {
			__builtin_amdgcn_fence(__ATOMIC_RELEASE, "workgroup");
			const u32 t = __hip_atomic_fetch_add(lb.finished, 1u, __ATOMIC_RELAXED, __HIP_MEMORY_SCOPE_AGENT);
			s_last = t == gridDim.x - 1 ? 1 : 0;
			if (s_last) __hip_atomic_store(lb.finished, 0u, __ATOMIC_RELAXED, __HIP_MEMORY_SCOPE_AGENT);
		}
		__syncthreads();
		if (s_last) op.finish(tid);
	}
}

template <int NV, int ITEMS = LB_ITEMS, class Op>
static inline int lb_launch(gsa_ctx *c, i64 n, const Op &op, hipStream_t stream = nullptr, int grid_per_cu = LB_GRID_PER_CU)
{
	if (!stream) stream = c->stream;
	if (c->n_cus <= 0) { hipDeviceProp_t pr; GSA_CHECK(c, hipGetDeviceProperties(&pr, c->device)); c->n_cus = pr.multiProcessorCount; }
	if constexpr (ITEMS > 4) { if (n <= (i64)LB_TPB * 4 * grid_per_cu * c->n_cus) return lb_launch<NV, 4>(c, n, op, stream, grid_per_cu); }
	constexpr i64 LB_TILE = (i64)LB_TPB * ITEMS;
	const size_t tiles = n > 0 ? (size_t)((n + LB_TILE - 1) / LB_TILE) : 1;
	for (int k = 0; k < 2; k++) {
		if (c->d_lb_status[k].cap < tiles * 8) {
			if (!dev_ensure<unsigned long long>(c, c->d_lb_status[k], tiles + 1024)) return GSA_ERR_NOMEM;
			GSA_CHECK(c, hipMemsetAsync(c->d_lb_status[k].p, 0, c->d_lb_status[k].cap, stream));
		}
	}
	c->lb_epoch++;
	if ((c->lb_epoch & 0x3fffffffu) == 0) {
		for (int k = 0; k < 2; k++) GSA_CHECK(c, hipMemsetAsync(c->d_lb_status[k].p, 0, c->d_lb_status[k].cap, stream));
		c->lb_epoch = 1;
	}
	LbArgs lb;
	lb.status[0] = c->d_lb_status[0].as<unsigned long long>(); lb.status[1] = c->d_lb_status[1].as<unsigned long long>();
	lb.ticket = c->d_mail.as<u32>() + M_TICKET; lb.base = c->lb_base; lb.epoch = c->lb_epoch; lb.err = c->d_mail.as<i32>() + M_LBERR; lb.finished = c->d_mail.as<u32>() + M_LBDONE;
	lb.n_tiles = (i32)tiles;
	const size_t grid = std::min<size_t>(tiles, (size_t)grid_per_cu * (size_t)c->n_cus);
	hipLaunchKernelGGL((k_lb_pass<NV, Op, ITEMS>), dim3((unsigned)grid), dim3(LB_TPB), 0, stream, n, op, lb);
	GSA_CHECK(c, hipGetLastError());
#ifdef LB_SYNC_DEBUG
	{ const hipError_t e_ = hipStreamSynchronize(stream); if (e_ != hipSuccess) { fprintf(stderr, "[LB_SYNC_DEBUG] %s: n = %lld, tiles = %zu, grid = %zu: %s\n", __PRETTY_FUNCTION__, (long long)n, tiles, grid, hipGetErrorString(e_)); return gsa_fail(c, GSA_ERR_HIP, "fused pass failed (LB_SYNC_DEBUG)"); } }
#endif
	c->lb_base += (u32)(tiles + (grid < tiles ? grid : 0));
	return GSA_OK;
}

#endif
```

### gsalign_amd/csrc/k_dp.hip

```cpp
#include <algorithm>
#include <cstring>
#include "gsa_ctx.h"
#include "gsa_dp.h"
#include "gsa_scan.h"
#include "gsa_gap.h"

#define SMALL_WAVES 4

__global__ void __launch_bounds__(64 * SMALL_WAVES) k_dp_small(i32 n_jobs, const i32 *__restrict__ order, const uint8_t *__restrict__ pool1, const i64 *__restrict__ off1,
                                                                const i32 *__restrict__ len1, const uint8_t *__restrict__ pool2, const i64 *__restrict__ off2,
                                                                const i32 *__restrict__ len2, uint8_t *ops, const i64 *__restrict__ ops_off, i32 *ops_len,
                                                                const i32 *__restrict__ jfrag, gsa_frag *frag)
{
	__shared__ uint8_t s_dir[SMALL_WAVES][(SMALL_ROWS / 2) * 64];
	__shared__ uint8_t s_rev[SMALL_WAVES][SMALL_ROWS + 64];
	__shared__ int s_n[SMALL_WAVES];
	const int w = threadIdx.x >> 6, lane = threadIdx.x & 63;
	const i32 slot = blockIdx.x * SMALL_WAVES + w;
	if (slot >= n_jobs) return;
	const i32 job = __builtin_amdgcn_readfirstlane(order[slot]);
	const int m = __builtin_amdgcn_readfirstlane(len1[job]), n = __builtin_amdgcn_readfirstlane(len2[job]);
	const uint8_t *s1 = pool1 + off1[job], *s2 = pool2 + off2[job];
	uint8_t *dir = s_dir[w], *rev = s_rev[w];
	const int cq = lane < n ? gsa_nt4(s2[lane]) : 4;
	const int c1a = lane < m ? gsa_nt4(s1[lane]) : 4, c1b = lane + 64 < m ? gsa_nt4(s1[lane + 64]) : 4;
	int u = lane ? 2 : 0, v = 0, x = 0, y = 0, wref = 4, dacc = 0;
	const int nr = m + n - 1;
	for (int r = 0; r < nr; r++) {
		const int inb = r < m ? (r < 64 ? __builtin_amdgcn_readlane(c1a, r) : __builtin_amdgcn_readlane(c1b, r - 64)) : 4;
		wref = wave_shr1(wref, inb);
		const int xt1 = wave_shr1(x, 0), vt1 = wave_shr1(v, r ? 2 : 0);
		const int jj = r - lane;
		int d = 0;
		if (lane < n && jj >= 0 && jj < m) {
			int un, vn, xn, yn;
			d = dp_cell(xt1, vt1, u, y, cq, wref, un, vn, xn, yn);
			u = un; v = vn; x = xn; y = yn;
		}
		const int nib = (d & 3) | ((d & 0x18) >> 1);
		if (r & 1) dir[(r >> 1) * 64 + lane] = (uint8_t)(dacc | (nib << 4)); else dacc = nib;
	}
	if (nr & 1) dir[(nr >> 1) * 64 + lane] = (uint8_t)dacc;
	__builtin_amdgcn_fence(__ATOMIC_RELEASE, "workgroup");
	__builtin_amdgcn_wave_barrier();
	__builtin_amdgcn_fence(__ATOMIC_ACQUIRE, "workgroup");
	if (lane == 0) {
		int i = n - 1, j = m - 1, state = 0, k = 0;
		while (i >= 0 && j >= 0) {
			const u32 nb = ((u32)dir[((i + j) >> 1) * 64 + i] >> (((i + j) & 1) << 2)) & 15u;
			const u32 tmp = (nb & 3u) | ((nb & 0xCu) << 1);
			int ns = state;
			if (ns != 0 && !((tmp >> (ns + 2)) & 1)) ns = 0;
			if (ns == 0) ns = (int)(tmp & 7);
			state = ns;
			const int isM = ns == 0 ? 1 : 0, isD = (ns == 1 || ns == 3) ? 1 : 0;
			rev[k++] = (uint8_t)(isM ? 'M' : (isD ? 'D' : 'I'));
			i -= isM | isD; j -= isM | (1 - isD);
		}
		for (; i >= 0; --i) rev[k++] = 'D';
		for (; j >= 0; --j) rev[k++] = 'I';
		s_n[w] = k;
	}
	__builtin_amdgcn_fence(__ATOMIC_RELEASE, "workgroup");
	__builtin_amdgcn_wave_barrier();
	__builtin_amdgcn_fence(__ATOMIC_ACQUIRE, "workgroup");
	const int nops = s_n[w];
	uint8_t *op = ops + ops_off[job];
	for (int p = lane; p < nops; p += 64) op[p] = rev[nops - 1 - p];
	if (lane == 0) { ops_len[job] = nops; if (frag) frag[jfrag[job]].aln_len = nops; }
}

#define TINY_ROWS 64
#define TINY_WAVES 4
__device__ __forceinline__ int row_shr1(int v, int fill) { return __builtin_amdgcn_update_dpp(fill, v, 0x111, 0xf, 0xf, false); }

__global__ void __launch_bounds__(64 * TINY_WAVES) k_dp_tiny(i32 n_jobs, const i32 *__restrict__ order, const uint8_t *__restrict__ pool1, const i64 *__restrict__ off1,
                                                              const i32 *__restrict__ len1, const uint8_t *__restrict__ pool2, const i64 *__restrict__ off2,
                                                              const i32 *__restrict__ len2, uint8_t *ops, const i64 *__restrict__ ops_off, i32 *ops_len,
                                                              const i32 *__restrict__ jfrag, gsa_frag *frag)
{
	__shared__ uint8_t s_dir[TINY_WAVES][TINY_ROWS * 64];
	__shared__ uint8_t s_ref[TINY_WAVES][4][TINY_ROWS];
	__shared__ uint8_t s_rev[TINY_WAVES][4][TINY_ROWS + 32];
	__shared__ int s_n[TINY_WAVES][4];
	const int w = threadIdx.x >> 6, lane = threadIdx.x & 63, q = lane >> 4, tl = lane & 15;
	const i32 slot = (blockIdx.x * TINY_WAVES + w) * 4 + q;
	if ((blockIdx.x * TINY_WAVES + w) * 4 >= n_jobs) return;
	const bool have = slot < n_jobs;
	const i32 job = have ? order[slot] : 0;
	const int m = have ? len1[job] : 0, n = have ? len2[job] : 0;
	const uint8_t *s1 = pool1 + off1[job], *s2 = pool2 + off2[job];
	uint8_t *dir = s_dir[w];
	for (int k = tl; k < TINY_ROWS; k += 16) s_ref[w][q][k] = (uint8_t)(k < m ? gsa_nt4(s1[k]) : 4);
	const int cq = tl < n ? gsa_nt4(s2[tl]) : 4;
	int u = tl ? 2 : 0, v = 0, x = 0, y = 0, wref = 4;
	int nr = have ? m + n - 1 : 0;
	nr = max(max(__builtin_amdgcn_readlane(nr, 0), __builtin_amdgcn_readlane(nr, 16)), max(__builtin_amdgcn_readlane(nr, 32), __builtin_amdgcn_readlane(nr, 48)));
	__builtin_amdgcn_fence(__ATOMIC_RELEASE, "workgroup");
	__builtin_amdgcn_wave_barrier();
	__builtin_amdgcn_fence(__ATOMIC_ACQUIRE, "workgroup");
	int inb = s_ref[w][q][0];
	for (int r = 0; r < nr; r++) {
		const int inb_next = s_ref[w][q][r + 1 < TINY_ROWS ? r + 1 : TINY_ROWS - 1];
		wref = row_shr1(wref, r < m ? inb : 4);
		const int xt1 = row_shr1(x, 0), vt1 = row_shr1(v, r ? 2 : 0);
		const int jj = r - tl;
		if (tl < n && jj >= 0 && jj < m) {
			int un, vn, xn, yn;
			const int d = dp_cell(xt1, vt1, u, y, cq, wref, un, vn, xn, yn);
			u = un; v = vn; x = xn; y = yn;
			dir[r * 64 + lane] = (uint8_t)d;
		}
		inb = inb_next;
	}
	__builtin_amdgcn_fence(__ATOMIC_RELEASE, "workgroup");
	__builtin_amdgcn_wave_barrier();
	__builtin_amdgcn_fence(__ATOMIC_ACQUIRE, "workgroup");
	if (tl == 0 && have) {
		uint8_t *rev = s_rev[w][q];
		int i = n - 1, j = m - 1, state = 0, k = 0;
		while (i >= 0 && j >= 0) {
			const u32 tmp = dir[(i + j) * 64 + (q << 4) + i];
			int ns = state;
			if (ns != 0 && !((tmp >> (ns + 2)) & 1)) ns = 0;
			if (ns == 0) ns = (int)(tmp & 7);
			state = ns;
			const int isM = ns == 0 ? 1 : 0, isD = (ns == 1 || ns == 3) ? 1 : 0;
			rev[k++] = (uint8_t)(isM ? 'M' : (isD ? 'D' : 'I'));
			i -= isM | isD; j -= isM | (1 - isD);
		}
		for (; i >= 0; --i) rev[k++] = 'D';
		for (; j >= 0; --j) rev[k++] = 'I';
		s_n[w][q] = k;
	}
	__builtin_amdgcn_fence(__ATOMIC_RELEASE, "workgroup");
	__builtin_amdgcn_wave_barrier();
	__builtin_amdgcn_fence(__ATOMIC_ACQUIRE, "workgroup");
	if (have) {
		const int nops = s_n[w][q];
		uint8_t *op = ops + ops_off[job];
		for (int p = tl; p < nops; p += 16) op[p] = s_rev[w][q][nops - 1 - p];
		if (tl == 0) { ops_len[job] = nops; if (frag) frag[jfrag[job]].aln_len = nops; }
	}
}

#define LANE_TILE 512
#define LANE_BINS 128
#define LANE_KMAX 576
#ifndef LANE_WGS
#define LANE_WGS 1024
#endif
#define LANE_LDS_WAVE 8448
__device__ __forceinline__ u32 lane_bin(u32 cells)
{
	const int msb = 31 - __clz((int)cells);
	const u32 frac = msb >= 3 ? (cells >> (msb - 3)) & 7u : (cells << (3 - msb)) & 7u;
	return ((u32)msb << 3) | frac;
}

__global__ void __launch_bounds__(256) k_dp_lane(i32 n_tiny, const i32 *__restrict__ order_tiny, i32 n_small, const i32 *__restrict__ order_small,
                                                  const uint8_t *__restrict__ pool1, const i64 *__restrict__ off1, const i32 *__restrict__ len1,
                                                  const uint8_t *__restrict__ pool2, const i64 *__restrict__ off2, const i32 *__restrict__ len2,
                                                  uint8_t *ops, const i64 *__restrict__ ops_off, i32 *ops_len, const i32 *__restrict__ jfrag, gsa_frag *frag, u32 *arena_all, u32 kstride)
{
	__shared__ u32 s_hist[LANE_BINS];
	__shared__ i32 s_sorted[LANE_TILE];
	__shared__ int s_next;
	__shared__ __attribute__((aligned(16))) uint8_t s_work[4][LANE_LDS_WAVE];
	const int tid = threadIdx.x, lane = tid & 63, w = tid >> 6;
	const i64 n_all = (i64)n_tiny + n_small;
	u32 *arena = arena_all + ((size_t)blockIdx.x * 4 + w) * 64 * kstride + lane;
	uint16_t *col = (uint16_t *)s_work[w] + lane;
	uint8_t *revb = s_work[w] + lane;
	for (i64 t0 = (i64)blockIdx.x * LANE_TILE; t0 < n_all; t0 += (i64)gridDim.x * LANE_TILE) {
		if (tid < LANE_BINS) s_hist[tid] = 0;
		if (tid == 0) s_next = 0;
		__syncthreads();
		i32 jb[LANE_TILE / 256]; u32 key[LANE_TILE / 256], rk[LANE_TILE / 256];
#pragma unroll
		for (int k = 0; k < LANE_TILE / 256; k++) {
			const i64 idx = t0 + k * 256 + tid;
			jb[k] = -1; key[k] = 0; rk[k] = 0;
			if (idx < n_all) {
				const i32 job = idx < n_tiny ? order_tiny[idx] : order_small[idx - n_tiny];
				jb[k] = job; key[k] = lane_bin((u32)len1[job] * (u32)len2[job]); rk[k] = atomicAdd(&s_hist[key[k]], 1u);
			}
		}
		__syncthreads();
		if (tid < 64) {
			const u32 a = s_hist[LANE_BINS - 1 - 2 * lane], b = s_hist[LANE_BINS - 2 - 2 * lane];
			u32 inc = a + b;
			for (int o = 1; o < 64; o <<= 1) { const u32 t = __shfl_up(inc, o); if (lane >= o) inc += t; }
			const u32 ex = inc - (a + b);
			s_hist[LANE_BINS - 1 - 2 * lane] = ex; s_hist[LANE_BINS - 2 - 2 * lane] = ex + a;
		}
		__syncthreads();
#pragma unroll
		for (int k = 0; k < LANE_TILE / 256; k++) if (jb[k] >= 0) s_sorted[s_hist[key[k]] + rk[k]] = jb[k];
		__syncthreads();
		const int nt = (int)(n_all - t0 < LANE_TILE ? n_all - t0 : LANE_TILE), nb = (nt + 63) >> 6;
		for (;;) {
			int b = 0;
			if (lane == 0) b = atomicAdd(&s_next, 1);
			b = __builtin_amdgcn_readfirstlane(b);
			if (b >= nb) break;
			const int p = b * 64 + lane;
			const bool have = p < nt;
			const i32 job = have ? s_sorted[p] : 0;
			const int m = have ? len1[job] : 0, n = have ? len2[job] : 0;
			const uint8_t *s1 = pool1 + off1[job], *s2 = pool2 + off2[job];
			const int nw = (n + 7) >> 3;
			int nmax = n;
			for (int o = 32; o; o >>= 1) { const int t = __shfl_xor(nmax, o); nmax = t > nmax ? t : nmax; }
			for (int i = 0; i < nmax; i++) if (i < n) col[i * 64] = (uint16_t)((i ? 2 : 0) | (gsa_nt4(s2[i]) << 12));
			bool act = have && m > 0 && n > 0;
			int g = 0, j = 0, x = 0, v = 0, kk = 0;
			auto row_table = [](int b) -> u32 { return b == 4 ? 0x66666u : 0x65555u + (2u << (4 * b)); };
			u32 tbl = row_table(act ? gsa_nt4(s1[0]) : 4);
			uint8_t raw_next = (act && m > 1) ? s1[1] : (uint8_t)'N';
			while (__any(act)) {
				if (act) {
					uint16_t *cg = col + g * 8 * 64;
					u32 e[8];
#pragma unroll
					for (int k = 0; k < 8; k++) e[k] = cg[k * 64];
					u32 acc = 0;
					const int left = n - g * 8;
#pragma unroll
					for (int k = 0; k < 8; k++) {
						if (k < left) {
							const int u = (int)(e[k] & 31u), y = (int)((e[k] >> 5) & 31u);
							const u32 c4 = e[k] >> 10;
							int z = (int)((tbl >> c4) & 15u);
							int a = x + v, b = y + u;
							int d = a > z ? 1 : 0; z = z > a ? z : a;
							if (b > z) d = 2;
							z = z > b ? z : b;
							z = z < 7 ? z : 7;
							const int un = z - v, vn = z - u;
							z -= 2; a -= z; b -= z;
							if (a > 0) d |= 0x08; else a = 0;
							if (b > 0) d |= 0x10; else b = 0;
							cg[k * 64] = (uint16_t)((u32)un | ((u32)b << 5) | (c4 << 10));
							x = a; v = vn;
							acc |= (u32)((d & 3) | ((d & 0x18) >> 1)) << (4 * k);
						}
					}
					arena[(size_t)kk * 64] = acc; kk++;
					g++;
					if (g == nw) {
						g = 0; j++; x = 0; v = 2;
						if (j >= m) act = false;
						else { tbl = row_table(gsa_nt4(raw_next)); raw_next = j + 1 < m ? s1[j + 1] : (uint8_t)'N'; }
					}
				}
			}
			int ti = n - 1, tj = m - 1, state = 0, k = 0;
			bool tb = have && ti >= 0 && tj >= 0;
			while (__any(tb)) {
				if (tb) {
					const u32 wd = arena[(size_t)(tj * nw + (ti >> 3)) * 64];
					const u32 nbv = (wd >> ((ti & 7) << 2)) & 15u;
					const u32 tmp = (nbv & 3u) | ((nbv & 0xCu) << 1);
					int ns = state;
					if (ns != 0 && !((tmp >> (ns + 2)) & 1)) ns = 0;
					if (ns == 0) ns = (int)(tmp & 7);
					state = ns;
					const int isM = ns == 0 ? 1 : 0, isD = (ns == 1 || ns == 3) ? 1 : 0;
					revb[k * 64] = (uint8_t)(isM ? 'M' : (isD ? 'D' : 'I'));
					k++;
					ti -= isM | isD; tj -= isM | (1 - isD);
					tb = ti >= 0 && tj >= 0;
				}
			}
			if (have) {
				for (; ti >= 0; --ti) { revb[k * 64] = 'D'; k++; }
				for (; tj >= 0; --tj) { revb[k * 64] = 'I'; k++; }
				uint8_t *op = ops + ops_off[job];
				for (int q = 0; q < k; q++) op[q] = revb[(k - 1 - q) * 64];
				ops_len[job] = k;
				if (frag) frag[jfrag[job]].aln_len = k;
			}
		}
		__syncthreads();
	}
}

struct StripeJob { i32 job, m, n, P; i64 diroff, bndoff; i32 ctr, first_block; };
#define DP_TILE_ROWS 160
#define DP_STRIPE_BYTES(M) ((((size_t)(M) + 63 + 7) >> 3) << 8)
#define DP_C1_PAD 320
#define DP_TILE_SLACK 16
#ifndef DP_G
#define DP_G 8
#endif
#ifdef GSA_DP_TIMING
#define DPT(...) __VA_ARGS__
#else
#define DPT(...)
#endif
#ifndef DP_EXP
#define DP_EXP 0
#endif
#if DP_EXP & 1
#define DPX_STORE(...)
#else
#define DPX_STORE(...) __VA_ARGS__
#endif
#if DP_EXP & 2
#define DPX_TB(...) __VA_ARGS__
#else
#define DPX_TB(...)
#endif
#define DP_LOOK 21
#define DP_WAIT_TICKS 200000000ull
#define DP_CLASS_M 768
#define DP_CLASS_TOP 1536
#define DP_CLASS_MIN_JOBS 4096
#define DP_LDS_M 3968

#ifdef DP_PK_ASM
#define PK2(NAME, INS) __device__ __forceinline__ u32 NAME(u32 a, u32 b) { u32 d; asm(INS " %0, %1, %2" : "=v"(d) : "v"(a), "v"(b)); return d; }
PK2(pk_add, "v_pk_add_u16") PK2(pk_sub, "v_pk_sub_u16") PK2(pk_max, "v_pk_max_u16") PK2(pk_min, "v_pk_min_u16")
__device__ __forceinline__ u32 pk_sub_sat(u32 a, u32 b) { u32 d; asm("v_pk_sub_u16 %0, %1, %2 clamp" : "=v"(d) : "v"(a), "v"(b)); return d; }
__device__ __forceinline__ u32 pk_mad(u32 a, u32 b, u32 c) { u32 d; asm("v_pk_mad_u16 %0, %1, %2, %3" : "=v"(d) : "v"(a), "v"(b), "v"(c)); return d; }
__device__ __forceinline__ u32 pk_shl(u32 a, u32 sh) { u32 d; asm("v_pk_lshlrev_b16 %0, %1, %2" : "=v"(d) : "v"(sh), "v"(a)); return d; }
#define DP_OPAQUE(X)
#else
typedef unsigned short v2u16 __attribute__((ext_vector_type(2)));
#define V2(X) __builtin_bit_cast(v2u16, (u32)(X))
#define U1(X) __builtin_bit_cast(u32, (v2u16)(X))
__device__ __forceinline__ u32 pk_add(u32 a, u32 b) { return U1(V2(a) + V2(b)); }
__device__ __forceinline__ u32 pk_sub(u32 a, u32 b) { return U1(V2(a) - V2(b)); }
__device__ __forceinline__ u32 pk_max(u32 a, u32 b) { return U1(__builtin_elementwise_max(V2(a), V2(b))); }
__device__ __forceinline__ u32 pk_min(u32 a, u32 b) { return U1(__builtin_elementwise_min(V2(a), V2(b))); }
__device__ __forceinline__ u32 pk_sub_sat(u32 a, u32 b) { return U1(__builtin_elementwise_sub_sat(V2(a), V2(b))); }
__device__ __forceinline__ u32 pk_mad(u32 a, u32 b, u32 c) { return U1(V2(a) * V2(b) + V2(c)); }
__device__ __forceinline__ u32 pk_shl(u32 a, u32 sh) { return U1(V2(a) << V2(sh)); }
#define DP_OPAQUE(X) asm volatile("" : "+v"(X))
#endif

template <int WPB>
__global__ void __launch_bounds__(64 * WPB) k_dp_stripe(const i32 *__restrict__ blk2job, const StripeJob *__restrict__ sjobs, const uint8_t *__restrict__ pool1, const i64 *__restrict__ off1,
                                                   const uint8_t *__restrict__ pool2, const i64 *__restrict__ off2, uint8_t *dirbase, u32 *bndbase, u32 *ctr,
                                                   uint8_t *revbase, uint8_t *ops, const i64 *__restrict__ ops_off, i32 *ops_len, u32 ep, i32 lds_c1, i32 lds_rows, u32 *err, i32 tick_slot)
{
	extern __shared__ __attribute__((aligned(16))) u32 C2[];
	uint8_t *tile = (uint8_t *)C2;
	__shared__ u32 s_bid, s_tick;
	if (threadIdx.x == 0) {
		s_tick = 0;
		const u32 tk = __hip_atomic_fetch_add(&ctr[tick_slot], 1u, __ATOMIC_RELAXED, __HIP_MEMORY_SCOPE_AGENT);
		if (tk == gridDim.x - 1) __hip_atomic_store(&ctr[tick_slot], 0u, __ATOMIC_RELAXED, __HIP_MEMORY_SCOPE_AGENT);
		s_bid = tk;
	}
	__syncthreads();
	const u32 bid = s_bid;
#ifndef DP_PRIO_BLOCKS
#define DP_PRIO_BLOCKS 96
#endif
	if (bid < DP_PRIO_BLOCKS) __builtin_amdgcn_s_setprio(3);
	const StripeJob sj = sjobs[blk2job[bid]];
	const int lane = threadIdx.x & 63, wave = threadIdx.x >> 6;
	const int m = sj.m, n = sj.n, P = sj.P, PP = (P + 1) >> 1;
	const int pp = ((int)bid - sj.first_block) * WPB + wave;
	const uint8_t *s1 = pool1 + off1[sj.job], *s2 = pool2 + off2[sj.job];
	const size_t pitch = (size_t)DP_STRIPE_BYTES(m);
	const int nblk = (m + 63 + 7) >> 3;
	uint8_t *dir = dirbase + sj.diroff;
	u32 *bnd_in = bndbase + sj.bndoff + (size_t)(pp - 1) * m, *bnd_out = bndbase + sj.bndoff + (size_t)pp * m;
	{
		int fe = (m + DP_C1_PAD + 63) & ~63; fe = fe < (lds_c1 >> 2) ? fe : (lds_c1 >> 2);
		for (int t = threadIdx.x; t < fe; t += 64 * WPB) {
			const int j = t - 128, jb = j - 64;
			const u32 ca = (j >= 0 && j < m) ? (u32)gsa_nt4(s1[j]) : 4u, cb = (jb >= 0 && jb < m) ? (u32)gsa_nt4(s1[jb]) : 4u;
			C2[t] = (ca < 4 ? ca : 0x0cu) | 0x0c000c00u | ((cb < 4 ? 4u + cb : 0x0cu) << 16);
		}
	}
	u32 *lds_bnd = C2 + (lds_c1 >> 2);
	if (WPB > 1) for (int t = threadIdx.x; t < (WPB - 1) * lds_rows; t += 64 * WPB) lds_bnd[t] = 0;
	u32 *lin = lds_bnd + (size_t)(wave > 0 ? wave - 1 : 0) * lds_rows, *lout = lds_bnd + (size_t)(wave < WPB - 1 ? wave : 0) * lds_rows;
	const bool out_lds = WPB > 1 && wave < WPB - 1;
	const int tA = pp * 128 + lane, tB = tA + 64;
	const bool hasB = 2 * pp + 1 < P;
	const int WpB = !hasB ? 0 : (n - pp * 128 - 64 < 64 ? n - pp * 128 - 64 : 64);
	const int WpA = n - pp * 128 < 64 ? n - pp * 128 : 64;
	const int cqA = tA < n ? gsa_nt4(s2[tA]) : 4, cqB = tB < n ? gsa_nt4(s2[tB]) : 4;
	u32 tblA = 0, tblB = 0;
#pragma unroll
	for (int cc = 0; cc < 4; cc++) {
		tblA |= (u32)(cqA == 4 ? 0 : (cqA == cc ? 7 ^ 6 : 5 ^ 6)) << (8 * cc);
		tblB |= (u32)(cqB == 4 ? 0 : (cqB == cc ? 7 ^ 6 : 5 ^ 6)) << (8 * cc);
	}
	const u32 uinit2 = (tA ? 2u : 0u) | (2u << 16);
	u32 u2 = uinit2, y2 = 0;
	u32 bin = 0, gnext = 0;
	__syncthreads();
	if (pp >= PP) return;
	const int S_end = hasB ? 64 + m + WpB - 1 : m + WpA - 1;
	DPT(const unsigned long long T0c = wall_clock64();)
	u32 *dirA = (u32 *)(dir + (size_t)(2 * pp) * pitch), *dirB = (u32 *)(dir + (size_t)(2 * pp + 1) * pitch);
	if (pp > 0) {
		const int row = (lane & (DP_G - 1)) < m ? (lane & (DP_G - 1)) : m - 1;
		gnext = (WPB > 1 && wave > 0) ? __hip_atomic_load(&lin[row], __ATOMIC_RELAXED, __HIP_MEMORY_SCOPE_WORKGROUP) : __hip_atomic_load(&bnd_in[row], __ATOMIC_RELAXED, __HIP_MEMORY_SCOPE_AGENT);
	}
	asm volatile("" :: "v"(gnext));
	const bool pub_stripe = pp < PP - 1;
	u32 pk2 = 0;
	u32 hb = 0;
	const u32 selx = lane ? 0x0c060c04u : 0x0c040c00u, selv = lane ? 0x0c070c05u : 0x0c050c01u;
	u32 acc = 0, r0 = 0;
	u32 c1 = 0x00010001u, c2 = 0x00020002u, c4 = 0x00040004u, c7 = 0x00070007u, c16 = 0x00100010u;
	DP_OPAQUE(c1); DP_OPAQUE(c2); DP_OPAQUE(c4); DP_OPAQUE(c7); DP_OPAQUE(c16);
#define DP_WL_LIT(HB, VAL, K) asm("v_writelane_b32 %0, %1, %2" : "+v"(HB) : "s"(VAL), "n"(K));
#define DP_WL_VAR(HB, VAL, K) if (lane == (K)) HB = (VAL);
#define DP_LOADG(MODE, ROW) ((MODE) == 2 ? __hip_atomic_load(&lin[ROW], __ATOMIC_RELAXED, __HIP_MEMORY_SCOPE_WORKGROUP) : __hip_atomic_load(&bnd_in[ROW], __ATOMIC_RELAXED, __HIP_MEMORY_SCOPE_AGENT))
#define DP_STEP(K2, MODE, WSEL, GUARD, WL)                                                                       \
	{                                                                                                           \
		const int s_ = s0 + (K2);                                                                               \
		if (((K2) & (DP_G - 1)) == 0) {                                                                         \
			if ((MODE) == 0) bin = (s_ == 0 && lane == 0) ? 0u : 0x200u;     \
			else if (s_ < m) {                                                                                  \
				 \
				const int row = s_ + (lane & (DP_G - 1));                                                       \
				const bool need = lane < DP_G && row < m;                                                       \
				u32 g = gnext;                                                                                  \
				if (!__all(!need || (g >> 16) == ep)) {       \
					u32 spins = 0; const unsigned long long t_wait0 = wall_clock64();                          \
					do {                                                                                        \
						if ((++spins & 255) == 0 && (wall_clock64() - t_wait0 > DP_WAIT_TICKS || __hip_atomic_load(err, __ATOMIC_RELAXED, __HIP_MEMORY_SCOPE_AGENT))) { if (lane == 0) __hip_atomic_store(err, 1u, __ATOMIC_RELAXED, __HIP_MEMORY_SCOPE_AGENT); break; } \
						__builtin_amdgcn_s_sleep(1);                                                            \
						if (need) g = DP_LOADG(MODE, row);                                                      \
					} while (!__all(!need || (g >> 16) == ep));                                                  \
				}                                                                                               \
				bin = g & 0xffffu;                                                                              \
				 \
				const int rown = row + DP_G < m ? row + DP_G : m - 1;                                           \
				gnext = DP_LOADG(MODE, rown);                                                                   \
			}                                                                                                   \
		}                                                                                                       \
		               \
		                          \
		const u32 bin0 = (u32)__builtin_amdgcn_readlane((int)bin, (K2) & (DP_G - 1));                           \
		const u32 rot = (u32)__builtin_amdgcn_mov_dpp((int)pk2, 0x13C, 0xf, 0xf, true);                         \
		WL(hb, (u32)__builtin_amdgcn_readlane((int)pk2, 63) >> 16, (K2) & 7)       \
		const u32 x1 = __builtin_amdgcn_perm(rot, bin0, selx), v1 = __builtin_amdgcn_perm(rot, bin0, selv);     \
		const u32 z0 = __builtin_amdgcn_perm(tblB, tblA, (WSEL)) ^ 0x00060006u;                                 \
		const u32 a = pk_add(x1, v1), b = pk_add(y2, u2);                                                       \
		const u32 z1 = pk_max(z0, a), z2 = pk_max(z1, b);                                                       \
		const u32 ta = pk_min(pk_sub(z1, z0), c1), tb = pk_min(pk_sub(z2, z1), c1);       \
		const u32 zc = pk_min(z2, c7);                                                                          \
		const u32 un = pk_sub(zc, v1), vn = pk_sub(zc, u2), zz = pk_sub(zc, c2);                                \
		const u32 xa = pk_sub_sat(a, zz), yb = pk_sub_sat(b, zz);                                                \
		const u32 fa = pk_min(xa, c1), fb = pk_min(yb, c1);                                                      \
		 \
		acc = pk_mad(acc, c16, pk_mad(pk_mad(fb, c2, fa), c4, pk_mad(tb, c2, ta)));                             \
		u2 = un; y2 = yb;                                                                                       \
		pk2 = __builtin_amdgcn_perm(vn, xa, 0x06020400u);       \
		if (GUARD) {                                                                                            \
			const u32 keep = (lane <= s_ ? 0xffffu : 0u) | (lane <= s_ - 64 ? 0xffff0000u : 0u);               \
			u2 = (u2 & keep) | (uinit2 & ~keep); y2 &= keep;                                                    \
		}                                                                                                       \
		if (((K2) & 7) == 3) r0 = acc;                                                                  \
		if (((K2) & 7) == 7) {                                                                                  \
			const int blk = s_ >> 3;                                                                            \
			if (!(GUARD) || blk < nblk) { DPX_STORE(dirA[((size_t)blk << 6) + lane] = __builtin_amdgcn_perm(acc, r0, 0x05040100u);) } \
			if (hasB && (!(GUARD) || (blk >= 8 && blk - 8 < nblk))) { DPX_STORE(dirB[((size_t)(blk - 8) << 6) + lane] = __builtin_amdgcn_perm(acc, r0, 0x07060302u);) } \
		}                                                                                                       \
		if (((K2) & 7) == 7 && pub_stripe && s_ >= 135) {                                                       \
			   \
			const int row = s_ - 135 + lane;                                                                    \
			if (lane < 8 && row < m) {                                                                          \
				if (out_lds) __hip_atomic_store(&lout[row], (ep << 16) | hb, __ATOMIC_RELAXED, __HIP_MEMORY_SCOPE_WORKGROUP); \
				else __hip_atomic_store(&bnd_out[row], (ep << 16) | hb, __ATOMIC_RELAXED, __HIP_MEMORY_SCOPE_AGENT); \
			}                                                                                                   \
		}                                                                                                       \
	}
#define DP_LOOP(MODE)                                                                                           \
	for (int s0 = 0; s0 < S_end; s0 += 16) {                                                                    \
		const u32 *crow = C2 + 128 + s0 - lane;                                  \
		if (s0 + 16 <= S_end) {                                                                                 \
			u32 w[16];                                                                                          \
			_Pragma("unroll") for (int k2 = 0; k2 < 16; k2++) w[k2] = crow[k2];                                   \
			if (s0 >= 128 && s0 + 16 <= 8 * nblk) {                                                             \
				 \
				DP_STEP(0, MODE, w[0], 0, DP_WL_LIT) DP_STEP(1, MODE, w[1], 0, DP_WL_LIT) DP_STEP(2, MODE, w[2], 0, DP_WL_LIT) DP_STEP(3, MODE, w[3], 0, DP_WL_LIT) DP_STEP(4, MODE, w[4], 0, DP_WL_LIT) DP_STEP(5, MODE, w[5], 0, DP_WL_LIT) DP_STEP(6, MODE, w[6], 0, DP_WL_LIT) DP_STEP(7, MODE, w[7], 0, DP_WL_LIT) \
				DP_STEP(8, MODE, w[8], 0, DP_WL_LIT) DP_STEP(9, MODE, w[9], 0, DP_WL_LIT) DP_STEP(10, MODE, w[10], 0, DP_WL_LIT) DP_STEP(11, MODE, w[11], 0, DP_WL_LIT) DP_STEP(12, MODE, w[12], 0, DP_WL_LIT) DP_STEP(13, MODE, w[13], 0, DP_WL_LIT) DP_STEP(14, MODE, w[14], 0, DP_WL_LIT) DP_STEP(15, MODE, w[15], 0, DP_WL_LIT) \
			} else {                                                                                            \
				DP_STEP(0, MODE, w[0], 1, DP_WL_LIT) DP_STEP(1, MODE, w[1], 1, DP_WL_LIT) DP_STEP(2, MODE, w[2], 1, DP_WL_LIT) DP_STEP(3, MODE, w[3], 1, DP_WL_LIT) DP_STEP(4, MODE, w[4], 1, DP_WL_LIT) DP_STEP(5, MODE, w[5], 1, DP_WL_LIT) DP_STEP(6, MODE, w[6], 1, DP_WL_LIT) DP_STEP(7, MODE, w[7], 1, DP_WL_LIT) \
				DP_STEP(8, MODE, w[8], 1, DP_WL_LIT) DP_STEP(9, MODE, w[9], 1, DP_WL_LIT) DP_STEP(10, MODE, w[10], 1, DP_WL_LIT) DP_STEP(11, MODE, w[11], 1, DP_WL_LIT) DP_STEP(12, MODE, w[12], 1, DP_WL_LIT) DP_STEP(13, MODE, w[13], 1, DP_WL_LIT) DP_STEP(14, MODE, w[14], 1, DP_WL_LIT) DP_STEP(15, MODE, w[15], 1, DP_WL_LIT) \
			}                                                                                                   \
		} else {                                                                                                \
			for (int k2 = 0; s0 + k2 < S_end; k2++) DP_STEP(k2, MODE, crow[k2], 1, DP_WL_VAR)                                 \
		}                                                                                                       \
	}
	if (pp == 0) { DP_LOOP(0) } else if (WPB > 1 && wave > 0) { DP_LOOP(2) } else { DP_LOOP(1) }
#undef DP_LOOP
#undef DP_STEP
#undef DP_LOADG
	if (S_end & 7) {
		if (S_end & 3) acc = pk_shl(acc, (u32)(4 * (4 - (S_end & 3))) * 0x00010001u);
		if ((S_end & 7) < 4) r0 = acc;
		const int blk = S_end >> 3;
		if (blk < nblk) { DPX_STORE(dirA[((size_t)blk << 6) + lane] = __builtin_amdgcn_perm(acc, r0, 0x05040100u);) }
		if (hasB && blk >= 8 && blk - 8 < nblk) { DPX_STORE(dirB[((size_t)(blk - 8) << 6) + lane] = __builtin_amdgcn_perm(acc, r0, 0x07060302u);) }
	}
	if (pub_stripe) {
		if (lane == (S_end & 7)) hb = (u32)__builtin_amdgcn_readlane((int)pk2, 63) >> 16;
		const int row = (S_end & ~7) - 128 + lane;
		if (lane <= (S_end & 7) && row >= 0 && row < m) {
			if (out_lds) __hip_atomic_store(&lout[row], (ep << 16) | hb, __ATOMIC_RELAXED, __HIP_MEMORY_SCOPE_WORKGROUP);
			else __hip_atomic_store(&bnd_out[row], (ep << 16) | hb, __ATOMIC_RELAXED, __HIP_MEMORY_SCOPE_AGENT);
		}
	}
	DPT(if (pp == 0 && lane == 0) ctr[sj.ctr + 40] = (u32)(wall_clock64() - T0c); if (pp == PP - 1 && lane == 0) ctr[sj.ctr + 41] = (u32)(wall_clock64() - T0c);)
	const bool one_wg = WPB > 1 && PP <= WPB;
	const int first_p = ((int)bid - sj.first_block) * WPB;
	const int mine = PP - first_p < WPB ? PP - first_p : WPB, n_wg = (PP + WPB - 1) / WPB;
	u32 ticket = 0;
	if (WPB > 1) {
		__builtin_amdgcn_fence(__ATOMIC_RELEASE, "workgroup");
		asm volatile("s_waitcnt vmcnt(0)" ::: "memory");
		if (lane == 0) ticket = __hip_atomic_fetch_add(&s_tick, 1u, __ATOMIC_RELAXED, __HIP_MEMORY_SCOPE_WORKGROUP);
		ticket = (u32)__builtin_amdgcn_readfirstlane((int)ticket);
		if ((int)ticket != mine - 1) return;
		__builtin_amdgcn_fence(__ATOMIC_ACQUIRE, "workgroup");
	}
	if (!one_wg) {
		__builtin_amdgcn_fence(__ATOMIC_RELEASE, "agent");
		asm volatile("s_waitcnt vmcnt(0)" ::: "memory");
		if (lane == 0) ticket = __hip_atomic_fetch_add(&ctr[sj.ctr], 1u, __ATOMIC_RELAXED, __HIP_MEMORY_SCOPE_AGENT);
		ticket = (u32)__builtin_amdgcn_readfirstlane((int)ticket);
		if ((int)ticket != (WPB > 1 ? n_wg : PP) - 1) return;
		if (lane == 0) ctr[sj.ctr] = 0;
		__builtin_amdgcn_fence(__ATOMIC_ACQUIRE, "agent");
	}
	DPX_TB(if (lane == 0) ops_len[sj.job] = 0; return;)
	DPT(const unsigned long long T1c = wall_clock64(); int ntile = 0, nrun = 0;)
	uint8_t *rev = revbase + ops_off[sj.job], *op = ops + ops_off[sj.job];
	int i = n - 1, j = m - 1, state = 0, k = 0;
	const int g = lane / DP_LOOK, e = lane - g * DP_LOOK;
	const int dlc = g == 2 ? 0 : -e, drl = g == 0 ? -2 * e : -e;
	constexpr int TB_BLKS = DP_TILE_ROWS / 8, TB_VEC = TB_BLKS * 16 / 64;
	static_assert(TB_VEC == 5, "the prefetched tile is five named registers (an array was kept in scratch: 96 bytes per lane)");
	uint4 pf0 = {0, 0, 0, 0}, pf1 = pf0, pf2 = pf0, pf3 = pf0, pf4 = pf0;
#define PF_EACH(X) X(0, pf0) X(1, pf1) X(2, pf2) X(3, pf3) X(4, pf4)
	int pf_sp = -1, pf_lo = 0, pf_hi = -1;
	const int rl_max = m - 1 + 63;
	const u32 *tile32 = (const u32 *)tile;
	while (i >= 0 && j >= 0) {
		i = __builtin_amdgcn_readfirstlane(i); j = __builtin_amdgcn_readfirstlane(j);
		DPT(ntile++;)
		const int sp = i >> 6, rl_hi = j + (i & 63);
		int rl_lo;
		uint4 *dst = (uint4 *)tile;
		if (sp == pf_sp && rl_hi <= pf_hi && rl_hi - pf_lo >= 64) {
			rl_lo = pf_lo;
			DPT(nrun += 1 << 16;)
#define PF_PUT(Q, R) dst[(Q) * 64 + lane] = R;
			PF_EACH(PF_PUT)
#undef PF_PUT
		} else {
			const int b_hi = rl_hi >> 3, b_lo = b_hi - (TB_BLKS - 1) > 0 ? b_hi - (TB_BLKS - 1) : 0;
			rl_lo = b_lo << 3;
			const uint4 *src = (const uint4 *)(dir + (size_t)sp * pitch + ((size_t)b_lo << 8));
			const int nvec = (b_hi - b_lo + 1) * 16;
#pragma unroll
			for (int q2 = 0; q2 < TB_VEC; q2++) { const int id = q2 * 64 + lane; if (id < nvec) dst[id] = src[id]; }
		}
		pf_sp = -1;
		{
			const int jp = j - ((i & 63) + 1);
			if (sp > 0 && jp >= 0) {
				int hi = jp + 63 + DP_TILE_SLACK; hi = hi < rl_max ? hi : rl_max;
				const int pb_hi = hi >> 3, pb_lo = pb_hi - (TB_BLKS - 1) > 0 ? pb_hi - (TB_BLKS - 1) : 0;
				const uint4 *src = (const uint4 *)(dir + (size_t)(sp - 1) * pitch + ((size_t)pb_lo << 8));
				const int nvec = (pb_hi - pb_lo + 1) * 16;
#define PF_GET(Q, R) { const int id = (Q) * 64 + lane; R = src[id < nvec ? id : 0]; }
				PF_EACH(PF_GET)
#undef PF_GET
				pf_sp = sp - 1; pf_lo = pb_lo << 3; pf_hi = (pb_hi << 3) + 7 < rl_max ? (pb_hi << 3) + 7 : rl_max;
			}
		}
		__builtin_amdgcn_fence(__ATOMIC_RELEASE, "workgroup");
		__builtin_amdgcn_wave_barrier();
		__builtin_amdgcn_fence(__ATOMIC_ACQUIRE, "workgroup");
		for (;;) {
			i = __builtin_amdgcn_readfirstlane(i); j = __builtin_amdgcn_readfirstlane(j);
			state = __builtin_amdgcn_readfirstlane(state); k = __builtin_amdgcn_readfirstlane(k);
			if (i < 0 || j < 0) break;
			const int lc = i - (sp << 6), rl = j + lc;
			if (lc < 0 || rl < rl_lo) break;
			const int lc2 = lc + dlc, rl2 = rl + drl;
			const bool valid = lane < 3 * DP_LOOK && lc2 >= 0 && rl2 >= rl_lo && rl2 - lc2 >= 0;
			u32 tmp = 0xffu;
			if (valid) {
				const u32 nb = (tile32[(((rl2 - rl_lo) >> 3) << 6) + lc2] >> ((((rl2 & 7) >> 2) << 4) + ((3 - (rl2 & 3)) << 2))) & 15u;
				tmp = ((nb & 2u) ? 2u : (nb & 1u)) | ((nb & 0xCu) << 1);
			}
			const u32 cur = (u32)__builtin_amdgcn_readfirstlane((int)tmp);
			int S = state;
			if (S != 0 && !((cur >> (S + 2)) & 1)) S = 0;
			if (S == 0) S = (int)(cur & 7);
			const int isM = S == 0 ? 1 : 0, isD = (S == 1 || S == 3) ? 1 : 0;
			const int gS = isM ? 0 : (isD ? 1 : 2);
			const bool cont = valid && g == gS && (isM ? (tmp & 7) == 0 : (((tmp >> (S + 2)) & 1) != 0 || (int)(tmp & 7) == S));
			const unsigned long long bal = __ballot(cont) >> (gS * DP_LOOK + 1);
			int run = __builtin_ctzll(~bal);
			run = run < DP_LOOK - 1 ? run : DP_LOOK - 1;
			const int L = 1 + run;
			if (lane < L) rev[k + lane] = (uint8_t)(isM ? 'M' : (isD ? 'D' : 'I'));
			k += L; state = S; DPT(nrun++;)
			i -= (isM | isD) ? L : 0; j -= (isM | (1 - isD)) ? L : 0;
		}
	}
	DPT(if (lane == 0) { ctr[sj.ctr + 42] = (u32)(wall_clock64() - T1c); ctr[sj.ctr + 43] = ntile; ctr[sj.ctr + 44] = nrun; ctr[sj.ctr + 45] = (u32)(wall_clock64() - T0c); })
	if (lane == 0) {
		for (; i >= 0; --i) rev[k++] = 'D';
		for (; j >= 0; --j) rev[k++] = 'I';
		ops_len[sj.job] = k;
	}
	k = __builtin_amdgcn_readfirstlane(k);
	__builtin_amdgcn_fence(__ATOMIC_RELEASE, "workgroup");
	asm volatile("s_waitcnt vmcnt(0)" ::: "memory");
	__builtin_amdgcn_fence(__ATOMIC_ACQUIRE, "workgroup");
	for (int q2 = lane; q2 < k; q2 += 64) op[q2] = rev[k - 1 - q2];
}

struct OpClassify {
	const i32 *len1, *len2; i32 *order, *order_tiny, *lg, *jlarge, *mail;
	static constexpr bool clamped = true;
	struct Item { i32 in, m, n; };
	__device__ Item load(i64 j) const { Item it; it.in = 0; it.m = len1[j]; it.n = len2[j]; return it; }
	__device__ void prep(Item &it, i64 j) const { it.in = j < mail[M_NJOB] ? 1 : 0; if (!it.in) it.m = it.n = 0; }
	__device__ i32 value(const Item &it, i64, int c) const
	{
		if (!it.in) return 0;
		const i32 m = it.m, n = it.n;
		if (c == 0) return dp_is_large(m, n) ? 1 : 0;
		if (dp_is_large(m, n)) return 0;
		if (lane_cells > 0) return m * n <= lane_cells ? 1 : 0;
		return (n <= 16 && m + n - 1 <= TINY_ROWS) ? 1 : 0;
	}
	__device__ void emit(const Item &it, i64 j, const i32 *v, const i32 *ex) const
	{
		if (!it.in) return;
		const i32 m = it.m, n = it.n;
		if (m <= 0 || n <= 0) lb_pub(&mail[M_DPERR], 2);
		jlarge[j] = v[0];
		if (v[0]) { i32 *e = lg + 3 * (size_t)ex[0]; lb_pub(&e[0], (i32)j); lb_pub(&e[1], m); lb_pub(&e[2], n); }
		else if (v[1]) order_tiny[ex[1]] = (i32)j;
		else order[j - ex[0] - ex[1]] = (i32)j;
	}
	__device__ void done(const i32 *t) const { lb_pub(&mail[M_NLARGE], t[0]); lb_pub(&mail[M_NTINY], t[1]); }
	i32 *h_out; i32 h_cap; i32 lane_cells;
	__device__ void finish(int tid) const
	{
		if (tid < MAIL_N) h_out[tid] = __hip_atomic_load(&mail[tid], __ATOMIC_RELAXED, __HIP_MEMORY_SCOPE_AGENT);
		i32 nl = __hip_atomic_load(&mail[M_NLARGE], __ATOMIC_RELAXED, __HIP_MEMORY_SCOPE_AGENT); if (nl > h_cap) nl = h_cap;
		lb_copy_out(h_out + MAIL_N, lg, 3 * nl, tid);
	}
};

__global__ void k_dp_cells(const i32 *__restrict__ mail, const i32 *__restrict__ len1, const i32 *__restrict__ len2, unsigned long long *out)
{
	const i64 j = (i64)blockIdx.x * blockDim.x + threadIdx.x;
	const bool in = j < mail[M_NJOB];
	unsigned long long v = in ? (unsigned long long)len1[j] * (unsigned long long)len2[j] : 0, w = in ? (unsigned long long)(len1[j] + len2[j]) : 0;
	for (int o = 32; o; o >>= 1) { v += __shfl_xor(v, o); w += __shfl_xor(w, o); }
	if ((threadIdx.x & 63) == 0 && v) { atomicAdd(out, v); atomicAdd(out + 1, w); }
}

void dp_count_cells(gsa_ctx *c, i32 n_ub, const i32 *len1, const i32 *len2, hipStream_t stream)
{
	hipLaunchKernelGGL(k_dp_cells, dim3(grid_for((size_t)n_ub, 256)), dim3(256), 0, stream, c->d_mail.as<i32>(), len1, len2, (unsigned long long *)(c->d_mail.as<i32>() + M_CELLS));
}

#define LG_CHUNK 2048

int launch_stripes(gsa_ctx *c, hipStream_t st, std::vector<LgJob> &large, const uint8_t *pool1, const i64 *off1, const uint8_t *pool2, const i64 *off2,
                   uint8_t *ops, const i64 *ops_off, i32 *ops_len, uint8_t *rev, int err_slot)
{
	if (large.empty()) return GSA_OK;
	i32 *mail = c->d_mail.as<i32>();
	{
		auto by_cells = [](const LgJob &a, const LgJob &b) { const i64 ca = (i64)a.m * a.n, cb = (i64)b.m * b.n; return ca != cb ? ca > cb : a.job < b.job; };
		if (large.size() > 512) std::partial_sort(large.begin(), large.begin() + 256, large.end(), by_cells);
		else std::sort(large.begin(), large.end(), by_cells);
	}
	size_t n_xl = 0, n_top = large.size(), n_hi = large.size();
	{
		auto it0 = std::stable_partition(large.begin(), large.end(), [](const LgJob &g) { return g.m > DP_LDS_M; });
		n_xl = (size_t)(it0 - large.begin());
		if (large.size() >= DP_CLASS_MIN_JOBS) {
			auto it1 = std::stable_partition(it0, large.end(), [](const LgJob &g) { return g.m > DP_CLASS_TOP; });
			auto it = std::stable_partition(it1, large.end(), [](const LgJob &g) { return g.m > DP_CLASS_M; });
			n_top = (size_t)(it1 - large.begin()); n_hi = (size_t)(it - large.begin());
		}
	}
	for (const LgJob &g : large) if ((((g.m + 63) & ~63) + DP_C1_PAD) * 4 > 150 * 1024) return gsa_fail(c, GSA_ERR_LIMIT, "DP reference-side fragment longer than 38000 bases");
	const i64 budget = 12ll << 30;
	size_t first = 0;
	while (first < large.size()) {
		size_t cnt = 0;
		if (c->dp_safe) cnt = 1;
		else { size_t l = first; i64 db = 128; while (l < large.size()) { const i64 cells = (((i64)large[l].n + 63) / 64) * (i64)DP_STRIPE_BYTES(large[l].m); if (l > first && db + cells > budget) break; db += cells + 128; l++; } cnt = l - first; }
		DevBuf &psj = err_slot == M_DPERR3 ? c->p_sj_early : c->p_sj;
		const size_t s0 = std::min(std::max(n_xl, first), first + cnt), stp = std::min(std::max(n_top, first), first + cnt), s1 = std::min(std::max(n_hi, first), first + cnt);
		constexpr int NSEG = 4;
		struct Seg { size_t b, e; int mmax, wpb, mpad, lds_rows; size_t dyn_lds; i32 *b2j; i32 nblocks; } seg[NSEG] = { { first, s0 }, { s0, stp }, { stp, s1 }, { s1, first + cnt } };
		size_t nb_ub = 0;
		for (Seg &sg : seg) {
			sg.mmax = 1;
			for (size_t k = sg.b; k < sg.e; k++) if (large[k].m > sg.mmax) sg.mmax = large[k].m;
			sg.mpad = ((sg.mmax + 63) & ~63) + DP_C1_PAD;
			sg.wpb = sg.mmax <= DP_LDS_M ? 4 : 1;
			sg.lds_rows = (sg.mmax + 15) & ~15;
			sg.dyn_lds = (size_t)sg.mpad * 4 + (sg.wpb > 1 ? (size_t)(sg.wpb - 1) * sg.lds_rows * 4 : 0);
			if (sg.dyn_lds < (size_t)DP_TILE_ROWS * 32) sg.dyn_lds = (size_t)DP_TILE_ROWS * 32;
			if (c->opt.dp_occupancy > 0 && sg.wpb == 4) { const size_t want = (size_t)(160 * 1024) / (size_t)c->opt.dp_occupancy - 1024; if (sg.dyn_lds < want && want <= 64 * 1024) sg.dyn_lds = want; }
			for (size_t k = sg.b; k < sg.e; k++) nb_ub += (size_t)((((large[k].n + 63) / 64 + 1) / 2 + sg.wpb - 1) / sg.wpb);
		}
		if (!pin_ensure<char>(c, psj, (cnt + 1) * sizeof(StripeJob) + (nb_ub + 2) * 4)) return GSA_ERR_NOMEM;
		StripeJob *sj = psj.as<StripeJob>();
		i32 *b2j_all = (i32 *)(sj + cnt + 1);
		i64 dbytes = 128, bwords = 0; i32 nctr = NSEG; size_t b2j_used = 0;
		for (Seg &sg : seg) {
			sg.b2j = b2j_all + b2j_used; sg.nblocks = 0;
			for (size_t k = sg.b; k < sg.e; k++) {
				const LgJob &g = large[k];
				const i64 cells = (((i64)g.n + 63) / 64) * (i64)DP_STRIPE_BYTES(g.m);
				StripeJob s; s.job = g.job; s.m = g.m; s.n = g.n; s.P = (g.n + 63) / 64;
				s.diroff = dbytes; dbytes += cells + 128;
				s.bndoff = bwords; bwords += (i64)(s.P - 1) * g.m;
				s.ctr = nctr++; s.first_block = sg.nblocks;
				for (int b = 0; b < ((s.P + 1) / 2 + sg.wpb - 1) / sg.wpb; b++) sg.b2j[sg.nblocks++] = (i32)(k - first);
				sj[k - first] = s;
			}
			b2j_used += (size_t)sg.nblocks;
		}
		const size_t last = first + cnt;
		uint8_t *dir = dev_ensure<uint8_t>(c, c->d_scan2, (size_t)dbytes + 512);
		const size_t bnd_cap0 = c->d_dp_bnd.cap;
		u32 *bnd = dev_ensure<u32>(c, c->d_dp_bnd, (size_t)bwords + 64);
		const size_t ctr_cap0 = c->d_dp_ctr.cap;
		u32 *ctr = dev_ensure<u32>(c, c->d_dp_ctr, (size_t)nctr + 64);
		if (!dir || !bnd || !ctr) return GSA_ERR_NOMEM;
		c->dp_epoch = (c->dp_epoch + 1) & 0xffffu;
		if (c->dp_epoch == 0 || c->d_dp_bnd.cap != bnd_cap0) { GSA_CHECK(c, hipMemsetAsync(bnd, 0, c->d_dp_bnd.cap, st)); if (c->dp_epoch == 0) c->dp_epoch = 1; }
		if (c->d_dp_ctr.cap != ctr_cap0 || c->dp_dirty) { GSA_CHECK(c, hipMemsetAsync(ctr, 0, c->d_dp_ctr.cap, st)); GSA_CHECK(c, hipMemsetAsync(mail + err_slot, 0, 4, st)); c->dp_dirty = false; }
		const bool side = c->opt.dp_side && c->stream_aux[3] && seg[NSEG - 1].nblocks > 0 && (seg[0].nblocks > 0 || seg[1].nblocks > 0 || seg[2].nblocks > 0);
		if (side) { GSA_CHECK(c, hipEventRecord(c->ev[24], st)); GSA_CHECK(c, hipStreamWaitEvent(c->stream_aux[3], c->ev[24], 0)); }
		hipStream_t st_main = st;
		for (int si = 0; si < NSEG; si++) {
			const Seg &sg = seg[si];
			if (sg.nblocks == 0) continue;
			hipStream_t st = (side && si == NSEG - 1) ? c->stream_aux[3] : st_main;
			if (sg.wpb == 4) hipLaunchKernelGGL(k_dp_stripe<4>, dim3((unsigned)sg.nblocks), dim3(256), sg.dyn_lds, st, (const i32 *)sg.b2j, (const StripeJob *)sj, pool1, off1, pool2, off2, dir + 256, bnd, ctr, rev, ops, ops_off, ops_len, c->dp_epoch, (i32)(sg.mpad * 4), (i32)sg.lds_rows, (u32 *)(mail + err_slot), si);
			else hipLaunchKernelGGL(k_dp_stripe<1>, dim3((unsigned)sg.nblocks), dim3(64), sg.dyn_lds, st, (const i32 *)sg.b2j, (const StripeJob *)sj, pool1, off1, pool2, off2, dir + 256, bnd, ctr, rev, ops, ops_off, ops_len, c->dp_epoch, (i32)(sg.mpad * 4), (i32)sg.lds_rows, (u32 *)(mail + err_slot), si);
		}
		if (side) { GSA_CHECK(c, hipEventRecord(c->ev[25], c->stream_aux[3])); GSA_CHECK(c, hipStreamWaitEvent(st, c->ev[25], 0)); }
		GSA_CHECK(c, hipGetLastError());
		DPT(GSA_CHECK(c, hipStreamSynchronize(st)); if (cnt == 1) { u32 hh[6]; hipMemcpy(hh, ctr + sj[0].ctr + 40, 24, hipMemcpyDeviceToHost); fprintf(stderr, "[dp] %d x %d: fwd0 %.1f us  fwdlast %.1f us  traceback %.1f us (tiles %u runs %u)  total %.1f us\n", sj[0].m, sj[0].n, hh[0] * 0.01, hh[1] * 0.01, hh[2] * 0.01, hh[3], hh[4], hh[5] * 0.01); })
		if (last < large.size()) {
			i32 *h = c->h_mail;
			GSA_CHECK(c, hipMemcpyAsync(h, mail, MAIL_N * sizeof(i32), hipMemcpyDeviceToHost, st));
			GSA_CHECK(c, hipStreamSynchronize(st));
			if (h[err_slot]) { c->dp_dirty = c->dp_timeout = true; return gsa_fail(c, GSA_ERR_STATE, "internal: DP stripe hand-off timed out"); }
		}
		first = last;
	}
	return GSA_OK;
}

int run_ksw2_jobs(gsa_ctx *c, i32 n_ub, const uint8_t *pool1, const i64 *off1, const i32 *len1,
                  const uint8_t *pool2, const i64 *off2, const i32 *len2, uint8_t *ops, const i64 *ops_off, i32 *ops_len, i64 ops_total, Ksw2Launch *out,
                  const i32 *jfrag, gsa_frag *frag, bool mail_clean)
{
	*out = Ksw2Launch();
	if (n_ub <= 0) return GSA_OK;
	hipStream_t st = c->stream;
	i32 *mail = c->d_mail.as<i32>();
	i32 *d_order = dev_ensure<i32>(c, c->d_flag2, (size_t)n_ub + 2);
	i32 *d_order_tiny = dev_ensure<i32>(c, c->d_dp_tiny, (size_t)n_ub + 2);
	i32 *d_lg = dev_ensure<i32>(c, c->d_dp_large, 4 * ((size_t)n_ub + 1));
	i32 *d_jlarge = d_lg ? d_lg + 3 * ((size_t)n_ub + 1) : nullptr;
	uint8_t *rev = dev_ensure<uint8_t>(c, c->d_i64a, (size_t)ops_total + 64);
	if (!d_order || !d_order_tiny || !d_lg || !rev) return GSA_ERR_NOMEM;
	if (!pin_ensure<i32>(c, c->p_dp, (size_t)MAIL_N + 3 * LG_CHUNK)) return GSA_ERR_NOMEM;
	if (!mail_clean) GSA_CHECK(c, hipMemsetAsync(mail + M_DPERR, 0, 8 * sizeof(i32), st));
	i32 *h = c->p_dp.as<i32>();
	const size_t first_lg = (size_t)std::min<i64>(n_ub, LG_CHUNK);
	const int dp_lane = c->opt.dp_lane;
	{ OpClassify op = { len1, len2, d_order, d_order_tiny, d_lg, d_jlarge, mail, h, (i32)first_lg, dp_lane }; int rc = lb_launch<2>(c, n_ub, op); if (rc) return rc; }
	GSA_CHECK(c, hipStreamSynchronize(st));
	if (h[M_LBERR]) return gsa_fail(c, GSA_ERR_STATE, "internal: look-back scan timed out");
	if (h[M_DPERR]) return gsa_fail(c, GSA_ERR_ARG, "DP job with an empty side");
	const i32 n = h[M_NJOB], nlarge = h[M_NLARGE], ntiny = h[M_NTINY], nsmall = n - nlarge - ntiny;
	out->n = n; out->nsmall = nsmall + ntiny; out->nlarge = nlarge;
	if (n <= 0) return GSA_OK;
	c->counters[5] += (u64)n;
	if ((size_t)nlarge > first_lg) {
		i32 keep[MAIL_N]; memcpy(keep, h, sizeof(keep));
		if (!pin_ensure<i32>(c, c->p_dp, (size_t)MAIL_N + 3 * (size_t)nlarge)) return GSA_ERR_NOMEM;
		h = c->p_dp.as<i32>(); memcpy(h, keep, sizeof(keep));
		GSA_CHECK(c, hipMemcpyAsync(h + MAIL_N, d_lg, (size_t)nlarge * 12, hipMemcpyDeviceToHost, st));
		GSA_CHECK(c, hipStreamSynchronize(st));
	}
	std::vector<LgJob> large((const LgJob *)(h + MAIL_N), (const LgJob *)(h + MAIL_N) + nlarge);
	hipEvent_t ev_fork = c->ev[10], ev_j2 = c->ev[12];
#ifdef GSA_EXPERIMENTS
	static const int dp_order = [] { const char *e = getenv("GSA_DP_ORDER"); return e ? atoi(e) : 0; }();
	static const int dp_after_early = [] { const char *e = getenv("GSA_DP_AFTER_EARLY"); return e ? atoi(e) : 0; }();
#else
	const int dp_order = 0, dp_after_early = 0;
#endif
	if (nsmall + ntiny > 0 && dp_lane > 0) {
		GSA_CHECK(c, hipEventRecord(ev_fork, st));
		GSA_CHECK(c, hipStreamWaitEvent(c->stream_aux[1], ev_fork, 0));
		if (dp_after_early && c->early_in_flight) GSA_CHECK(c, hipStreamWaitEvent(c->stream_aux[1], c->ev[14], 0));
		if (ntiny > 0) {
			const i64 tiles = ((i64)ntiny + LANE_TILE - 1) / LANE_TILE;
			const unsigned nwg = (unsigned)(tiles < LANE_WGS ? tiles : LANE_WGS);
			u32 kstride = 1;
			for (int nn = 1; nn <= 64; nn++) { int mm = 128 - nn + 1; if (dp_lane > 0 && dp_lane / nn < mm) mm = dp_lane / nn; if (mm < 1) continue; const u32 kd = (u32)mm * (u32)((nn + 7) / 8); if (kd > kstride) kstride = kd; }
			if (kstride > LANE_KMAX) kstride = LANE_KMAX;
			u32 *arena = dev_ensure<u32>(c, c->d_dp_arena, (size_t)nwg * 4 * 64 * kstride);
			if (!arena) return GSA_ERR_NOMEM;
			hipLaunchKernelGGL(k_dp_lane, dim3(nwg), dim3(256), 0, c->stream_aux[1], ntiny, d_order_tiny, 0, d_order, pool1, off1, len1, pool2, off2, len2, ops, ops_off, ops_len, jfrag, frag, arena, kstride);
		}
		if (nsmall > 0) {
			const bool own = c->opt.dp_small_side && c->stream_aux[3] && ntiny > 0;
			hipStream_t s2 = own ? c->stream_aux[3] : (ntiny > 0 ? st : c->stream_aux[1]);
			if (own) GSA_CHECK(c, hipStreamWaitEvent(s2, ev_fork, 0));
			const unsigned nb = (unsigned)((nsmall + SMALL_WAVES - 1) / SMALL_WAVES);
			hipLaunchKernelGGL(k_dp_small, dim3(nb), dim3(64 * SMALL_WAVES), 0, s2, nsmall, d_order, pool1, off1, len1, pool2, off2, len2, ops, ops_off, ops_len, jfrag, frag);
			if (ntiny > 0) { GSA_CHECK(c, hipEventRecord(c->ev[18], s2)); GSA_CHECK(c, hipStreamWaitEvent(c->stream_aux[1], c->ev[18], 0)); }
		}
		GSA_CHECK(c, hipGetLastError());
		GSA_CHECK(c, hipEventRecord(ev_j2, c->stream_aux[1]));
		out->small_in_flight = true;
	} else if (nsmall + ntiny > 0 && dp_order == 1) {
		if (ntiny > 0) {
			const unsigned nb = (unsigned)((ntiny + 4 * TINY_WAVES - 1) / (4 * TINY_WAVES));
			hipLaunchKernelGGL(k_dp_tiny, dim3(nb), dim3(64 * TINY_WAVES), 0, st, ntiny, d_order_tiny, pool1, off1, len1, pool2, off2, len2, ops, ops_off, ops_len, jfrag, frag);
		}
		if (nsmall > 0) {
			const unsigned nb = (unsigned)((nsmall + SMALL_WAVES - 1) / SMALL_WAVES);
			hipLaunchKernelGGL(k_dp_small, dim3(nb), dim3(64 * SMALL_WAVES), 0, st, nsmall, d_order, pool1, off1, len1, pool2, off2, len2, ops, ops_off, ops_len, jfrag, frag);
		}
		GSA_CHECK(c, hipGetLastError());
		GSA_CHECK(c, hipEventRecord(ev_j2, st));
		GSA_CHECK(c, hipStreamWaitEvent(c->stream_aux[1], ev_j2, 0));
		out->small_in_flight = true;
	} else
	if (nsmall + ntiny > 0) {
		GSA_CHECK(c, hipEventRecord(ev_fork, st));
		GSA_CHECK(c, hipStreamWaitEvent(c->stream_aux[1], ev_fork, 0));
		if (ntiny > 0) {
			const unsigned nb = (unsigned)((ntiny + 4 * TINY_WAVES - 1) / (4 * TINY_WAVES));
			hipLaunchKernelGGL(k_dp_tiny, dim3(nb), dim3(64 * TINY_WAVES), 0, c->stream_aux[1], ntiny, d_order_tiny, pool1, off1, len1, pool2, off2, len2, ops, ops_off, ops_len, jfrag, frag);
		}
		if (nsmall > 0) {
			hipStream_t s2 = ntiny > 0 ? st : c->stream_aux[1];
			const unsigned nb = (unsigned)((nsmall + SMALL_WAVES - 1) / SMALL_WAVES);
			hipLaunchKernelGGL(k_dp_small, dim3(nb), dim3(64 * SMALL_WAVES), 0, s2, nsmall, d_order, pool1, off1, len1, pool2, off2, len2, ops, ops_off, ops_len, jfrag, frag);
			if (ntiny > 0) { GSA_CHECK(c, hipEventRecord(c->ev[18], s2)); GSA_CHECK(c, hipStreamWaitEvent(c->stream_aux[1], c->ev[18], 0)); }
		}
		GSA_CHECK(c, hipGetLastError());
		GSA_CHECK(c, hipEventRecord(ev_j2, c->stream_aux[1]));
		out->small_in_flight = true;
	}
	if (nlarge > 0) {
		if (c->early_in_flight) GSA_CHECK(c, hipStreamWaitEvent(st, c->ev[14], 0));
		int rc = launch_stripes(c, st, large, pool1, off1, pool2, off2, ops, ops_off, ops_len, rev, M_DPERR2);
		if (rc) return rc;
	}
	return GSA_OK;
}

extern "C" int gsa_ksw2_batch(gsa_ctx *c, int32_t n_pairs, const char *pool1, const int64_t *off1, const int32_t *len1,
                              const char *pool2, const int64_t *off2, const int32_t *len2, char *ops, const int64_t *ops_off, int32_t *ops_len)
{
	if (!c || n_pairs < 0) return GSA_ERR_ARG;
	if (n_pairs == 0) return GSA_OK;
	hipStream_t st = c->stream;
	const size_t n = (size_t)n_pairs;
	i64 p1 = 0, p2 = 0, po = 0;
	for (size_t i = 0; i < n; i++) {
		if (len1[i] < 0 || len2[i] < 0) return gsa_fail(c, GSA_ERR_ARG, "negative fragment length");
		if (off1[i] + len1[i] > p1) p1 = off1[i] + len1[i];
		if (off2[i] + len2[i] > p2) p2 = off2[i] + len2[i];
		if (ops_off[i] + len1[i] + len2[i] > po) po = ops_off[i] + len1[i] + len2[i];
	}
	uint8_t *d_p1 = dev_ensure<uint8_t>(c, c->leaf[0], (size_t)p1 + 1), *d_p2 = dev_ensure<uint8_t>(c, c->leaf[1], (size_t)p2 + 1), *d_ops = dev_ensure<uint8_t>(c, c->leaf[2], (size_t)po + 1);
	i64 *d_o1 = dev_ensure<i64>(c, c->leaf[3], n), *d_o2 = dev_ensure<i64>(c, c->leaf[4], n), *d_oo = dev_ensure<i64>(c, c->leaf[5], n);
	i32 *d_l1 = dev_ensure<i32>(c, c->leaf[6], n), *d_l2 = dev_ensure<i32>(c, c->leaf[7], n), *d_ol = dev_ensure<i32>(c, c->leaf[8], n);
	if (!d_p1 || !d_p2 || !d_ops || !d_o1 || !d_o2 || !d_oo || !d_l1 || !d_l2 || !d_ol) return GSA_ERR_NOMEM;
	GSA_CHECK(c, hipMemcpyAsync(d_p1, pool1, p1, hipMemcpyHostToDevice, st)); GSA_CHECK(c, hipMemcpyAsync(d_p2, pool2, p2, hipMemcpyHostToDevice, st));
	GSA_CHECK(c, hipMemcpyAsync(d_o1, off1, n * 8, hipMemcpyHostToDevice, st)); GSA_CHECK(c, hipMemcpyAsync(d_o2, off2, n * 8, hipMemcpyHostToDevice, st));
	GSA_CHECK(c, hipMemcpyAsync(d_oo, ops_off, n * 8, hipMemcpyHostToDevice, st));
	GSA_CHECK(c, hipMemcpyAsync(d_l1, len1, n * 4, hipMemcpyHostToDevice, st)); GSA_CHECK(c, hipMemcpyAsync(d_l2, len2, n * 4, hipMemcpyHostToDevice, st));
	const i32 cnts[2] = { n_pairs, (i32)po };
	GSA_CHECK(c, hipMemcpyAsync(c->d_mail.as<i32>() + M_NJOB, cnts, 8, hipMemcpyHostToDevice, st));
	Ksw2Launch kl;
	int rc = run_ksw2_jobs(c, n_pairs, d_p1, d_o1, d_l1, d_p2, d_o2, d_l2, d_ops, d_oo, d_ol, po, &kl);
	if (rc == GSA_OK && kl.small_in_flight) GSA_CHECK(c, hipStreamWaitEvent(st, c->ev[12], 0));
	if (rc == GSA_OK) {
		i32 err = 0;
		GSA_CHECK(c, hipMemcpyAsync(ops, d_ops, po, hipMemcpyDeviceToHost, st));
		GSA_CHECK(c, hipMemcpyAsync(ops_len, d_ol, n * 4, hipMemcpyDeviceToHost, st));
		GSA_CHECK(c, hipMemcpyAsync(&err, c->d_mail.as<i32>() + M_DPERR2, 4, hipMemcpyDeviceToHost, st));
		GSA_CHECK(c, hipStreamSynchronize(st));
		if (err) { c->dp_dirty = c->dp_timeout = true; rc = gsa_fail(c, GSA_ERR_STATE, "internal: DP stripe hand-off timed out"); }
	}
	return rc;
}
```

Measured before the change: 33.09 Gbp/s.

## Pack two narrow small-DP alignments per wavefront and drop the tiny DP kernel

The job classifier now produces three classes: one-lane jobs, jobs with query length at most 32 (handled two per wavefront by a templated k_dp_small<32> with a seam at lane 32), and the rest (k_dp_small<64>). The 16-wide k_dp_tiny kernel and its launch paths are removed, and the look-back scan gets a third status array. The goal is to keep wavefront lanes busy on narrow alignments instead of leaving half of a 64-wide wave idle. In exchange, paired jobs run to the longer anti-diagonal count of the two, and jobs that used to go to the tiny kernel now run at 32 lanes, or 64 lanes when dp_lane is 0.

```diff
diff --git a/gsalign_amd/csrc/gsa_api.hip b/gsalign_amd/csrc/gsa_api.hip
--- a/gsalign_amd/csrc/gsa_api.hip
+++ b/gsalign_amd/csrc/gsa_api.hip
@@ -253,7 +253,7 @@
 	return GSA_OK;
 }
 
-#define GSA_DEVBUFS(X) X(d_bwt) X(d_bwt_ref) X(d_occ_base) X(d_sa) X(d_ref) X(d_chr_end) X(d_chr_of_end) X(qs[0].d_query) X(qs[1].d_query) X(qs[0].d_bndtab) X(qs[1].d_bndtab) X(tmp) X(d_cnt) X(d_zero) X(d_mail) X(d_lb_status[0]) X(d_lb_status[1]) X(d_sa_dense) X(d_kmer) X(d_kmer_lo) X(d_pres) X(d_ref2) X(d_cand_s) X(d_cand_len) X(d_cand_x0) X(d_cand_freq) X(d_onpath) X(d_cand_cnt) X(d_heavy) X(dn_lf) X(dn_x0) X(d_chunk_hits) X(d_chunk_base) X(d_key_a) X(d_key_b) X(d_val_a) X(d_val_b) X(s_q) X(s_len) X(s_r) X(s_gid) X(d_flag) X(d_scan) X(g_beg) X(w_j0) X(d_pdbm) X(d_pdby) X(d_pdcb) X(d_gpre) X(d_key_c) X(d_val_c) X(a_q) X(a_len) X(a_r) X(a_gb) X(a_ge) X(a_uniq) X(a_cu) X(a_alive) X(a_ws) X(a_wid) X(a_next) X(a_brk) X(a_aurank) X(a_aulist) X(a_runinfo) X(w_best) X(w_sum) X(w_n) X(d_btab) X(d_flag2) X(d_scan2) X(d_i64a) X(b_q) X(b_len) X(b_r) X(b_gb) X(b_ge) X(c_q) X(c_len) X(c_r) X(c_gb) X(c_ge) X(c_bid) X(blk_beg) X(blk_end) X(blk_score) X(r_q) X(r_len) X(r_r) X(r_bid) X(r_tmp_q) X(r_tmp_len) X(r_tmp_r) X(r_tmp_bid) X(r_cut4) X(r_cut5) X(r_simjob) X(r_simres) X(d_leaf) X(fb_seedbase) X(fb_sbeg) X(fb_fragbase) X(f_rec) X(f_rec16) X(f_type) X(f_mism) X(f_alnlen) X(f_job) X(f_score) X(d_dp_tiny) X(d_dp_bnd) X(d_dp_ctr) X(d_dp_jobs) X(d_dp_large) X(d_tail) X(e_id) X(e_rec) X(e_list) X(e_off1) X(e_off2) X(e_opsoff) X(e_nops) X(e_ops) X(e_rev) X(r_head) X(f_early) X(r_orig) X(r_tmp_orig) X(j_frag) X(j_opsoff) X(j_nops) X(d_ops) X(j_cells) X(d_alnoff) X(bl_alnlen) X(bl_score) X(d_bblk) X(d_dp_arena) X(d_vblk) X(d_vcnt) X(d_vwg) X(d_var) X(d_cblk) X(d_cout) X(d_ccnt) X(d_cwg) X(d_cpre) X(d_crun) X(d_cops) X(leaf[0]) X(leaf[1]) X(leaf[2]) X(leaf[3]) X(leaf[4]) X(leaf[5]) X(leaf[6]) X(leaf[7]) X(leaf[8])
+#define GSA_DEVBUFS(X) X(d_bwt) X(d_bwt_ref) X(d_occ_base) X(d_sa) X(d_ref) X(d_chr_end) X(d_chr_of_end) X(qs[0].d_query) X(qs[1].d_query) X(qs[0].d_bndtab) X(qs[1].d_bndtab) X(tmp) X(d_cnt) X(d_zero) X(d_mail) X(d_lb_status[0]) X(d_lb_status[1]) X(d_lb_status[2]) X(d_sa_dense) X(d_kmer) X(d_kmer_lo) X(d_pres) X(d_ref2) X(d_cand_s) X(d_cand_len) X(d_cand_x0) X(d_cand_freq) X(d_onpath) X(d_cand_cnt) X(d_heavy) X(dn_lf) X(dn_x0) X(d_chunk_hits) X(d_chunk_base) X(d_key_a) X(d_key_b) X(d_val_a) X(d_val_b) X(s_q) X(s_len) X(s_r) X(s_gid) X(d_flag) X(d_scan) X(g_beg) X(w_j0) X(d_pdbm) X(d_pdby) X(d_pdcb) X(d_gpre) X(d_key_c) X(d_val_c) X(a_q) X(a_len) X(a_r) X(a_gb) X(a_ge) X(a_uniq) X(a_cu) X(a_alive) X(a_ws) X(a_wid) X(a_next) X(a_brk) X(a_aurank) X(a_aulist) X(a_runinfo) X(w_best) X(w_sum) X(w_n) X(d_btab) X(d_flag2) X(d_scan2) X(d_i64a) X(b_q) X(b_len) X(b_r) X(b_gb) X(b_ge) X(c_q) X(c_len) X(c_r) X(c_gb) X(c_ge) X(c_bid) X(blk_beg) X(blk_end) X(blk_score) X(r_q) X(r_len) X(r_r) X(r_bid) X(r_tmp_q) X(r_tmp_len) X(r_tmp_r) X(r_tmp_bid) X(r_cut4) X(r_cut5) X(r_simjob) X(r_simres) X(d_leaf) X(fb_seedbase) X(fb_sbeg) X(fb_fragbase) X(f_rec) X(f_rec16) X(f_type) X(f_mism) X(f_alnlen) X(f_job) X(f_score) X(d_dp_tiny) X(d_dp_bnd) X(d_dp_ctr) X(d_dp_jobs) X(d_dp_large) X(d_tail) X(e_id) X(e_rec) X(e_list) X(e_off1) X(e_off2) X(e_opsoff) X(e_nops) X(e_ops) X(e_rev) X(r_head) X(f_early) X(r_orig) X(r_tmp_orig) X(j_frag) X(j_opsoff) X(j_nops) X(d_ops) X(j_cells) X(d_alnoff) X(bl_alnlen) X(bl_score) X(d_bblk) X(d_dp_arena) X(d_vblk) X(d_vcnt) X(d_vwg) X(d_var) X(d_cblk) X(d_cout) X(d_ccnt) X(d_cwg) X(d_cpre) X(d_crun) X(d_cops) X(leaf[0]) X(leaf[1]) X(leaf[2]) X(leaf[3]) X(leaf[4]) X(leaf[5]) X(leaf[6]) X(leaf[7]) X(leaf[8])
 void gsa_destroy(gsa_ctx *c)
 {
 	if (!c) return;
@@ -440,7 +440,7 @@
 	else if (k == "bundle_contig") { if (!in(0, BIG)) return gsa_fail(c, GSA_ERR_ARG, "bundle_contig: 0 (no bundles) .. 2^40 bases"); c->opt.bundle_contig = value; }
 	else if (k == "bundle_cap") { if (!in(1, BIG)) return gsa_fail(c, GSA_ERR_ARG, "bundle_cap: 1 .. 2^40 bases"); c->opt.bundle_cap = value; }
 	else if (k == "seed_budget") { if (!in(1, 0xffffffffll)) return gsa_fail(c, GSA_ERR_ARG, "seed_budget: 1 .. 2^32 - 1 wave-iterations"); c->seed_budget = (u32)value; }
-	else if (k == "dp_lane") { if (!in(0, 1 << 20)) return gsa_fail(c, GSA_ERR_ARG, "dp_lane: 0 (round 2's tiny / small split) .. 2^20 cells"); c->opt.dp_lane = (int)value; }
+	else if (k == "dp_lane") { if (!in(0, 1 << 20)) return gsa_fail(c, GSA_ERR_ARG, "dp_lane: 0 (no per-lane class) .. 2^20 cells"); c->opt.dp_lane = (int)value; }
 	else if (k == "seed_mode") { if (value < 0 || value > 2) return gsa_fail(c, GSA_ERR_ARG, "seed_mode: 0 sweep, 1 speculative, 2 search"); c->opt.seed_mode = (int)value; }
 	else if (k == "pd_bitmap") c->opt.pd_bitmap = value != 0;
 	else if (k == "dp_side") c->opt.dp_side = value != 0;
diff --git a/gsalign_amd/csrc/gsa_ctx.h b/gsalign_amd/csrc/gsa_ctx.h
--- a/gsalign_amd/csrc/gsa_ctx.h
+++ b/gsalign_amd/csrc/gsa_ctx.h
@@ -18,7 +18,7 @@
 	i32 blk_score;
 };
 
-enum { M_NB = 0, M_NC = 1, M_NBLK = 2, M_NG = 3, M_NR = 4, M_NJ = 5, M_NL = 6, M_LBERR = 7, M_ANY = 8, M_NTINY = 40, M_TICKET = 48, M_NBRAW = 49, M_NR2 = 50, M_NF = 51, M_NJOB = 52, M_OPSTOT = 53, M_NALN = 54, M_DPERR = 64, M_NLARGE = 65, M_DPERR2 = 66, M_CELLS = 68  , M_DPERR3 = 41, M_LBDONE = 42, M_LFSTEPS = 44 , M_NEARLY = 62, M_EOPS = 63, M_NTOUCH = 46 , M_MAXBLK = 56 , MAIL_N = 72 };
+enum { M_NB = 0, M_NC = 1, M_NBLK = 2, M_NG = 3, M_NR = 4, M_NJ = 5, M_NL = 6, M_LBERR = 7, M_ANY = 8, M_NTINY = 40, M_NPAIR = 43 , M_TICKET = 48, M_NBRAW = 49, M_NR2 = 50, M_NF = 51, M_NJOB = 52, M_OPSTOT = 53, M_NALN = 54, M_DPERR = 64, M_NLARGE = 65, M_DPERR2 = 66, M_CELLS = 68  , M_DPERR3 = 41, M_LBDONE = 42, M_LFSTEPS = 44 , M_NEARLY = 62, M_EOPS = 63, M_NTOUCH = 46 , M_MAXBLK = 56 , MAIL_N = 72 };
 #define LEAF_CHUNK 1024
 
 struct HostBlock {
@@ -119,7 +119,7 @@
 	DevBuf leaf[9];
 	DevBuf d_cnt; u64 *h_cnt = nullptr;
 	DevBuf d_mail; i32 *h_mail = nullptr;
-	DevBuf d_lb_status[2]; u32 lb_epoch = 0, lb_base = 0;
+	DevBuf d_lb_status[3]; u32 lb_epoch = 0, lb_base = 0;
 	DevBuf p_leaf;
 	int ev_pending = 0;
 	bool s2_host = false;
diff --git a/gsalign_amd/csrc/gsa_scan.h b/gsalign_amd/csrc/gsa_scan.h
--- a/gsalign_amd/csrc/gsa_scan.h
+++ b/gsalign_amd/csrc/gsa_scan.h
@@ -22,8 +22,9 @@
 #else
 #define LB_T(K)
 #endif
+#define LB_MAX_NV 3
 struct LbArgs {
-	unsigned long long *status[2];
+	unsigned long long *status[LB_MAX_NV];
 	u32 *ticket;
 	u32 base, epoch; i32 n_tiles;
 	i32 *err;
@@ -159,7 +160,7 @@
 __global__ void __launch_bounds__(LB_TPB, LB_BOUND_OF(Op)) k_lb_pass(i64 n, Op op, LbArgs lb)
 {
 	constexpr int LB_TILE = LB_TPB * ITEMS;
-	__shared__ i32 s_tile, s_bcast[2], s_wsum[NV][ITEMS][LB_TPB / 64];
+	__shared__ i32 s_tile, s_bcast[LB_MAX_NV], s_wsum[NV][ITEMS][LB_TPB / 64];
 	const int tid = threadIdx.x, lane = tid & 63, wv = tid >> 6;
 #ifdef LB_TIMING
 	unsigned long long t_last = wall_clock64();
@@ -290,7 +291,8 @@
 	if constexpr (ITEMS > 4) { if (n <= (i64)LB_TPB * 4 * grid_per_cu * c->n_cus) return lb_launch<NV, 4>(c, n, op, stream, grid_per_cu); }
 	constexpr i64 LB_TILE = (i64)LB_TPB * ITEMS;
 	const size_t tiles = n > 0 ? (size_t)((n + LB_TILE - 1) / LB_TILE) : 1;
-	for (int k = 0; k < 2; k++) {
+	static_assert(NV <= LB_MAX_NV, "a status array per scanned component");
+	for (int k = 0; k < NV; k++) {
 		if (c->d_lb_status[k].cap < tiles * 8) {
 			if (!dev_ensure<unsigned long long>(c, c->d_lb_status[k], tiles + 1024)) return GSA_ERR_NOMEM;
 			GSA_CHECK(c, hipMemsetAsync(c->d_lb_status[k].p, 0, c->d_lb_status[k].cap, stream));
@@ -298,11 +300,11 @@
 	}
 	c->lb_epoch++;
 	if ((c->lb_epoch & 0x3fffffffu) == 0) {
-		for (int k = 0; k < 2; k++) GSA_CHECK(c, hipMemsetAsync(c->d_lb_status[k].p, 0, c->d_lb_status[k].cap, stream));
+		for (int k = 0; k < LB_MAX_NV; k++) if (c->d_lb_status[k].p) GSA_CHECK(c, hipMemsetAsync(c->d_lb_status[k].p, 0, c->d_lb_status[k].cap, stream));
 		c->lb_epoch = 1;
 	}
 	LbArgs lb;
-	lb.status[0] = c->d_lb_status[0].as<unsigned long long>(); lb.status[1] = c->d_lb_status[1].as<unsigned long long>();
+	for (int k = 0; k < LB_MAX_NV; k++) lb.status[k] = c->d_lb_status[k].as<unsigned long long>();
 	lb.ticket = c->d_mail.as<u32>() + M_TICKET; lb.base = c->lb_base; lb.epoch = c->lb_epoch; lb.err = c->d_mail.as<i32>() + M_LBERR; lb.finished = c->d_mail.as<u32>() + M_LBDONE;
 	lb.n_tiles = (i32)tiles;
 	const size_t grid = std::min<size_t>(tiles, (size_t)grid_per_cu * (size_t)c->n_cus);
diff --git a/gsalign_amd/csrc/k_dp.hip b/gsalign_amd/csrc/k_dp.hip
--- a/gsalign_amd/csrc/k_dp.hip
+++ b/gsalign_amd/csrc/k_dp.hip
@@ -6,48 +6,68 @@
 #include "gsa_gap.h"
 
 #define SMALL_WAVES 4
-
+#define SMALL_REV (SMALL_ROWS + 8)
+
+template <int SEG>
 __global__ void __launch_bounds__(64 * SMALL_WAVES) k_dp_small(i32 n_jobs, const i32 *__restrict__ order, const uint8_t *__restrict__ pool1, const i64 *__restrict__ off1,
                                                                 const i32 *__restrict__ len1, const uint8_t *__restrict__ pool2, const i64 *__restrict__ off2,
                                                                 const i32 *__restrict__ len2, uint8_t *ops, const i64 *__restrict__ ops_off, i32 *ops_len,
                                                                 const i32 *__restrict__ jfrag, gsa_frag *frag)
 {
+	static_assert(SEG == 64 || SEG == 32, "one or two alignments per wavefront");
+	constexpr int JPW = 64 / SEG;
+	constexpr int NCH = SMALL_ROWS / SEG;
 	__shared__ uint8_t s_dir[SMALL_WAVES][(SMALL_ROWS / 2) * 64];
-	__shared__ uint8_t s_rev[SMALL_WAVES][SMALL_ROWS + 64];
-	__shared__ int s_n[SMALL_WAVES];
-	const int w = threadIdx.x >> 6, lane = threadIdx.x & 63;
-	const i32 slot = blockIdx.x * SMALL_WAVES + w;
-	if (slot >= n_jobs) return;
-	const i32 job = __builtin_amdgcn_readfirstlane(order[slot]);
-	const int m = __builtin_amdgcn_readfirstlane(len1[job]), n = __builtin_amdgcn_readfirstlane(len2[job]);
+	__shared__ uint8_t s_rev[SMALL_WAVES][JPW][SMALL_REV];
+	__shared__ int s_n[SMALL_WAVES][JPW];
+	const int w = threadIdx.x >> 6, lane = threadIdx.x & 63, q = lane / SEG, tl = lane & (SEG - 1);
+	const i32 slot0 = (blockIdx.x * SMALL_WAVES + w) * JPW;
+	if (slot0 >= n_jobs) return;
+	const bool have = JPW == 1 || slot0 + q < n_jobs;
+	i32 job = have ? order[slot0 + q] : 0;
+	int m = have ? len1[job] : 0, n = have ? len2[job] : 0;
+	if (JPW == 1) { job = __builtin_amdgcn_readfirstlane(job); m = __builtin_amdgcn_readfirstlane(m); n = __builtin_amdgcn_readfirstlane(n); }
 	const uint8_t *s1 = pool1 + off1[job], *s2 = pool2 + off2[job];
-	uint8_t *dir = s_dir[w], *rev = s_rev[w];
-	const int cq = lane < n ? gsa_nt4(s2[lane]) : 4;
-	const int c1a = lane < m ? gsa_nt4(s1[lane]) : 4, c1b = lane + 64 < m ? gsa_nt4(s1[lane + 64]) : 4;
-	int u = lane ? 2 : 0, v = 0, x = 0, y = 0, wref = 4, dacc = 0;
-	const int nr = m + n - 1;
-	for (int r = 0; r < nr; r++) {
-		const int inb = r < m ? (r < 64 ? __builtin_amdgcn_readlane(c1a, r) : __builtin_amdgcn_readlane(c1b, r - 64)) : 4;
-		wref = wave_shr1(wref, inb);
-		const int xt1 = wave_shr1(x, 0), vt1 = wave_shr1(v, r ? 2 : 0);
-		const int jj = r - lane;
-		int d = 0;
-		if (lane < n && jj >= 0 && jj < m) {
-			int un, vn, xn, yn;
-			d = dp_cell(xt1, vt1, u, y, cq, wref, un, vn, xn, yn);
-			u = un; v = vn; x = xn; y = yn;
-		}
-		const int nib = (d & 3) | ((d & 0x18) >> 1);
-		if (r & 1) dir[(r >> 1) * 64 + lane] = (uint8_t)(dacc | (nib << 4)); else dacc = nib;
-	}
-	if (nr & 1) dir[(nr >> 1) * 64 + lane] = (uint8_t)dacc;
+	uint8_t *dir = s_dir[w], *rev = s_rev[w][q];
+	const int cq = tl < n ? gsa_nt4(s2[tl]) : 4;
+	int c1[NCH];
+#pragma unroll
+	for (int k = 0; k < NCH; k++) c1[k] = k * SEG + tl < m ? gsa_nt4(s1[k * SEG + tl]) : 4;
+	int u = tl ? 2 : 0, v = 0, x = 0, y = 0, wref = 4, dacc = 0;
+	int nr = m + n - 1;
+	if (JPW == 2) { const int na = __builtin_amdgcn_readlane(nr, 0), nb = __builtin_amdgcn_readlane(nr, 32); nr = na > nb ? na : nb; }
+#pragma unroll
+	for (int k = 0; k < NCH; k++) {
+		const int r_end = nr < (k + 1) * SEG ? nr : (k + 1) * SEG;
+		for (int r = k * SEG; r < r_end; r++) {
+			const int inb = __builtin_amdgcn_readlane(c1[k], r - k * SEG);
+			wref = wave_shr1(wref, inb);
+			int xt1 = wave_shr1(x, 0), vt1 = wave_shr1(v, r ? 2 : 0);
+			if (JPW == 2) {
+				const int inb2 = __builtin_amdgcn_readlane(c1[k], 32 + r - k * SEG);
+				const bool seam = lane == 32;
+				wref = seam ? inb2 : wref; xt1 = seam ? 0 : xt1; vt1 = seam ? (r ? 2 : 0) : vt1;
+			}
+			const int jj = r - tl;
+			int d = 0;
+			if (tl < n && jj >= 0 && jj < m) {
+				int un, vn, xn, yn;
+				d = dp_cell(xt1, vt1, u, y, cq, wref, un, vn, xn, yn);
+				u = un; v = vn; x = xn; y = yn;
+			}
+			const int nib = (d & 3) | ((d & 0x18) >> 1);
+			if (r & 1) dir[(r >> 1) * 64 + lane] = (uint8_t)(dacc | (nib << 4)); else dacc = nib;
+		}
+	}
+	if (nr > 0 && (nr & 1)) dir[(nr >> 1) * 64 + lane] = (uint8_t)dacc;
 	__builtin_amdgcn_fence(__ATOMIC_RELEASE, "workgroup");
 	__builtin_amdgcn_wave_barrier();
 	__builtin_amdgcn_fence(__ATOMIC_ACQUIRE, "workgroup");
-	if (lane == 0) {
+	if (tl == 0 && have) {
+		const uint8_t *dseg = dir + q * SEG;
 		int i = n - 1, j = m - 1, state = 0, k = 0;
 		while (i >= 0 && j >= 0) {
-			const u32 nb = ((u32)dir[((i + j) >> 1) * 64 + i] >> (((i + j) & 1) << 2)) & 15u;
+			const u32 nb = ((u32)dseg[((i + j) >> 1) * 64 + i] >> (((i + j) & 1) << 2)) & 15u;
 			const u32 tmp = (nb & 3u) | ((nb & 0xCu) << 1);
 			int ns = state;
 			if (ns != 0 && !((tmp >> (ns + 2)) & 1)) ns = 0;
@@ -59,78 +79,6 @@
 		}
 		for (; i >= 0; --i) rev[k++] = 'D';
 		for (; j >= 0; --j) rev[k++] = 'I';
-		s_n[w] = k;
-	}
-	__builtin_amdgcn_fence(__ATOMIC_RELEASE, "workgroup");
-	__builtin_amdgcn_wave_barrier();
-	__builtin_amdgcn_fence(__ATOMIC_ACQUIRE, "workgroup");
-	const int nops = s_n[w];
-	uint8_t *op = ops + ops_off[job];
-	for (int p = lane; p < nops; p += 64) op[p] = rev[nops - 1 - p];
-	if (lane == 0) { ops_len[job] = nops; if (frag) frag[jfrag[job]].aln_len = nops; }
-}
-
-#define TINY_ROWS 64
-#define TINY_WAVES 4
-__device__ __forceinline__ int row_shr1(int v, int fill) { return __builtin_amdgcn_update_dpp(fill, v, 0x111, 0xf, 0xf, false); }
-
-__global__ void __launch_bounds__(64 * TINY_WAVES) k_dp_tiny(i32 n_jobs, const i32 *__restrict__ order, const uint8_t *__restrict__ pool1, const i64 *__restrict__ off1,
-                                                              const i32 *__restrict__ len1, const uint8_t *__restrict__ pool2, const i64 *__restrict__ off2,
-                                                              const i32 *__restrict__ len2, uint8_t *ops, const i64 *__restrict__ ops_off, i32 *ops_len,
-                                                              const i32 *__restrict__ jfrag, gsa_frag *frag)
-{
-	__shared__ uint8_t s_dir[TINY_WAVES][TINY_ROWS * 64];
-	__shared__ uint8_t s_ref[TINY_WAVES][4][TINY_ROWS];
-	__shared__ uint8_t s_rev[TINY_WAVES][4][TINY_ROWS + 32];
-	__shared__ int s_n[TINY_WAVES][4];
-	const int w = threadIdx.x >> 6, lane = threadIdx.x & 63, q = lane >> 4, tl = lane & 15;
-	const i32 slot = (blockIdx.x * TINY_WAVES + w) * 4 + q;
-	if ((blockIdx.x * TINY_WAVES + w) * 4 >= n_jobs) return;
-	const bool have = slot < n_jobs;
-	const i32 job = have ? order[slot] : 0;
-	const int m = have ? len1[job] : 0, n = have ? len2[job] : 0;
-	const uint8_t *s1 = pool1 + off1[job], *s2 = pool2 + off2[job];
-	uint8_t *dir = s_dir[w];
-	for (int k = tl; k < TINY_ROWS; k += 16) s_ref[w][q][k] = (uint8_t)(k < m ? gsa_nt4(s1[k]) : 4);
-	const int cq = tl < n ? gsa_nt4(s2[tl]) : 4;
-	int u = tl ? 2 : 0, v = 0, x = 0, y = 0, wref = 4;
-	int nr = have ? m + n - 1 : 0;
-	nr = max(max(__builtin_amdgcn_readlane(nr, 0), __builtin_amdgcn_readlane(nr, 16)), max(__builtin_amdgcn_readlane(nr, 32), __builtin_amdgcn_readlane(nr, 48)));
-	__builtin_amdgcn_fence(__ATOMIC_RELEASE, "workgroup");
-	__builtin_amdgcn_wave_barrier();
-	__builtin_amdgcn_fence(__ATOMIC_ACQUIRE, "workgroup");
-	int inb = s_ref[w][q][0];
-	for (int r = 0; r < nr; r++) {
-		const int inb_next = s_ref[w][q][r + 1 < TINY_ROWS ? r + 1 : TINY_ROWS - 1];
-		wref = row_shr1(wref, r < m ? inb : 4);
-		const int xt1 = row_shr1(x, 0), vt1 = row_shr1(v, r ? 2 : 0);
-		const int jj = r - tl;
-		if (tl < n && jj >= 0 && jj < m) {
-			int un, vn, xn, yn;
-			const int d = dp_cell(xt1, vt1, u, y, cq, wref, un, vn, xn, yn);
-			u = un; v = vn; x = xn; y = yn;
-			dir[r * 64 + lane] = (uint8_t)d;
-		}
-		inb = inb_next;
-	}
-	__builtin_amdgcn_fence(__ATOMIC_RELEASE, "workgroup");
-	__builtin_amdgcn_wave_barrier();
-	__builtin_amdgcn_fence(__ATOMIC_ACQUIRE, "workgroup");
-	if (tl == 0 && have) {
-		uint8_t *rev = s_rev[w][q];
-		int i = n - 1, j = m - 1, state = 0, k = 0;
-		while (i >= 0 && j >= 0) {
-			const u32 tmp = dir[(i + j) * 64 + (q << 4) + i];
-			int ns = state;
-			if (ns != 0 && !((tmp >> (ns + 2)) & 1)) ns = 0;
-			if (ns == 0) ns = (int)(tmp & 7);
-			state = ns;
-			const int isM = ns == 0 ? 1 : 0, isD = (ns == 1 || ns == 3) ? 1 : 0;
-			rev[k++] = (uint8_t)(isM ? 'M' : (isD ? 'D' : 'I'));
-			i -= isM | isD; j -= isM | (1 - isD);
-		}
-		for (; i >= 0; --i) rev[k++] = 'D';
-		for (; j >= 0; --j) rev[k++] = 'I';
 		s_n[w][q] = k;
 	}
 	__builtin_amdgcn_fence(__ATOMIC_RELEASE, "workgroup");
@@ -139,7 +87,7 @@
 	if (have) {
 		const int nops = s_n[w][q];
 		uint8_t *op = ops + ops_off[job];
-		for (int p = tl; p < nops; p += 16) op[p] = s_rev[w][q][nops - 1 - p];
+		for (int p = tl; p < nops; p += SEG) op[p] = rev[nops - 1 - p];
 		if (tl == 0) { ops_len[job] = nops; if (frag) frag[jfrag[job]].aln_len = nops; }
 	}
 }
@@ -628,7 +576,7 @@
 }
 
 struct OpClassify {
-	const i32 *len1, *len2; i32 *order, *order_tiny, *lg, *jlarge, *mail;
+	const i32 *len1, *len2; i32 *order, *order_tiny, *order_pair, *lg, *jlarge, *mail;
 	static constexpr bool clamped = true;
 	struct Item { i32 in, m, n; };
 	__device__ Item load(i64 j) const { Item it; it.in = 0; it.m = len1[j]; it.n = len2[j]; return it; }
@@ -639,8 +587,9 @@
 		const i32 m = it.m, n = it.n;
 		if (c == 0) return dp_is_large(m, n) ? 1 : 0;
 		if (dp_is_large(m, n)) return 0;
-		if (lane_cells > 0) return m * n <= lane_cells ? 1 : 0;
-		return (n <= 16 && m + n - 1 <= TINY_ROWS) ? 1 : 0;
+		const bool one_lane = m * n <= lane_cells;
+		if (c == 1) return one_lane ? 1 : 0;
+		return !one_lane && n <= 32 ? 1 : 0;
 	}
 	__device__ void emit(const Item &it, i64 j, const i32 *v, const i32 *ex) const
 	{
@@ -650,9 +599,10 @@
 		jlarge[j] = v[0];
 		if (v[0]) { i32 *e = lg + 3 * (size_t)ex[0]; lb_pub(&e[0], (i32)j); lb_pub(&e[1], m); lb_pub(&e[2], n); }
 		else if (v[1]) order_tiny[ex[1]] = (i32)j;
-		else order[j - ex[0] - ex[1]] = (i32)j;
-	}
-	__device__ void done(const i32 *t) const { lb_pub(&mail[M_NLARGE], t[0]); lb_pub(&mail[M_NTINY], t[1]); }
+		else if (v[2]) order_pair[ex[2]] = (i32)j;
+		else order[j - ex[0] - ex[1] - ex[2]] = (i32)j;
+	}
+	__device__ void done(const i32 *t) const { lb_pub(&mail[M_NLARGE], t[0]); lb_pub(&mail[M_NTINY], t[1]); lb_pub(&mail[M_NPAIR], t[2]); }
 	i32 *h_out; i32 h_cap; i32 lane_cells;
 	__device__ void finish(int tid) const
 	{
@@ -781,22 +731,23 @@
 	if (n_ub <= 0) return GSA_OK;
 	hipStream_t st = c->stream;
 	i32 *mail = c->d_mail.as<i32>();
-	i32 *d_order = dev_ensure<i32>(c, c->d_flag2, (size_t)n_ub + 2);
+	i32 *d_order = dev_ensure<i32>(c, c->d_flag2, 2 * ((size_t)n_ub + 2));
 	i32 *d_order_tiny = dev_ensure<i32>(c, c->d_dp_tiny, (size_t)n_ub + 2);
 	i32 *d_lg = dev_ensure<i32>(c, c->d_dp_large, 4 * ((size_t)n_ub + 1));
 	i32 *d_jlarge = d_lg ? d_lg + 3 * ((size_t)n_ub + 1) : nullptr;
 	uint8_t *rev = dev_ensure<uint8_t>(c, c->d_i64a, (size_t)ops_total + 64);
 	if (!d_order || !d_order_tiny || !d_lg || !rev) return GSA_ERR_NOMEM;
+	i32 *d_order_pair = d_order + (size_t)n_ub + 2;
 	if (!pin_ensure<i32>(c, c->p_dp, (size_t)MAIL_N + 3 * LG_CHUNK)) return GSA_ERR_NOMEM;
 	if (!mail_clean) GSA_CHECK(c, hipMemsetAsync(mail + M_DPERR, 0, 8 * sizeof(i32), st));
 	i32 *h = c->p_dp.as<i32>();
 	const size_t first_lg = (size_t)std::min<i64>(n_ub, LG_CHUNK);
 	const int dp_lane = c->opt.dp_lane;
-	{ OpClassify op = { len1, len2, d_order, d_order_tiny, d_lg, d_jlarge, mail, h, (i32)first_lg, dp_lane }; int rc = lb_launch<2>(c, n_ub, op); if (rc) return rc; }
+	{ OpClassify op = { len1, len2, d_order, d_order_tiny, d_order_pair, d_lg, d_jlarge, mail, h, (i32)first_lg, dp_lane }; int rc = lb_launch<3>(c, n_ub, op); if (rc) return rc; }
 	GSA_CHECK(c, hipStreamSynchronize(st));
 	if (h[M_LBERR]) return gsa_fail(c, GSA_ERR_STATE, "internal: look-back scan timed out");
 	if (h[M_DPERR]) return gsa_fail(c, GSA_ERR_ARG, "DP job with an empty side");
-	const i32 n = h[M_NJOB], nlarge = h[M_NLARGE], ntiny = h[M_NTINY], nsmall = n - nlarge - ntiny;
+	const i32 n = h[M_NJOB], nlarge = h[M_NLARGE], ntiny = h[M_NTINY], npair = h[M_NPAIR], nsmall = n - nlarge - ntiny;
 	out->n = n; out->nsmall = nsmall + ntiny; out->nlarge = nlarge;
 	if (n <= 0) return GSA_OK;
 	c->counters[5] += (u64)n;
@@ -815,7 +766,24 @@
 #else
 	const int dp_order = 0, dp_after_early = 0;
 #endif
-	if (nsmall + ntiny > 0 && dp_lane > 0) {
+	auto launch_small = [&](hipStream_t s2) {
+		const i32 nsingle = nsmall - npair;
+		if (nsingle > 0) {
+			const unsigned nb = (unsigned)((nsingle + SMALL_WAVES - 1) / SMALL_WAVES);
+			hipLaunchKernelGGL(k_dp_small<64>, dim3(nb), dim3(64 * SMALL_WAVES), 0, s2, nsingle, d_order, pool1, off1, len1, pool2, off2, len2, ops, ops_off, ops_len, jfrag, frag);
+		}
+		if (npair > 0) {
+			const unsigned nb = (unsigned)((npair + 2 * SMALL_WAVES - 1) / (2 * SMALL_WAVES));
+			hipLaunchKernelGGL(k_dp_small<32>, dim3(nb), dim3(64 * SMALL_WAVES), 0, s2, npair, d_order_pair, pool1, off1, len1, pool2, off2, len2, ops, ops_off, ops_len, jfrag, frag);
+		}
+	};
+	if (nsmall + ntiny > 0 && dp_order == 1 && dp_lane == 0) {
+		launch_small(st);
+		GSA_CHECK(c, hipGetLastError());
+		GSA_CHECK(c, hipEventRecord(ev_j2, st));
+		GSA_CHECK(c, hipStreamWaitEvent(c->stream_aux[1], ev_j2, 0));
+		out->small_in_flight = true;
+	} else if (nsmall + ntiny > 0) {
 		GSA_CHECK(c, hipEventRecord(ev_fork, st));
 		GSA_CHECK(c, hipStreamWaitEvent(c->stream_aux[1], ev_fork, 0));
 		if (dp_after_early && c->early_in_flight) GSA_CHECK(c, hipStreamWaitEvent(c->stream_aux[1], c->ev[14], 0));
@@ -833,38 +801,7 @@
 			const bool own = c->opt.dp_small_side && c->stream_aux[3] && ntiny > 0;
 			hipStream_t s2 = own ? c->stream_aux[3] : (ntiny > 0 ? st : c->stream_aux[1]);
 			if (own) GSA_CHECK(c, hipStreamWaitEvent(s2, ev_fork, 0));
-			const unsigned nb = (unsigned)((nsmall + SMALL_WAVES - 1) / SMALL_WAVES);
-			hipLaunchKernelGGL(k_dp_small, dim3(nb), dim3(64 * SMALL_WAVES), 0, s2, nsmall, d_order, pool1, off1, len1, pool2, off2, len2, ops, ops_off, ops_len, jfrag, frag);
-			if (ntiny > 0) { GSA_CHECK(c, hipEventRecord(c->ev[18], s2)); GSA_CHECK(c, hipStreamWaitEvent(c->stream_aux[1], c->ev[18], 0)); }
-		}
-		GSA_CHECK(c, hipGetLastError());
-		GSA_CHECK(c, hipEventRecord(ev_j2, c->stream_aux[1]));
-		out->small_in_flight = true;
-	} else if (nsmall + ntiny > 0 && dp_order == 1) {
-		if (ntiny > 0) {
-			const unsigned nb = (unsigned)((ntiny + 4 * TINY_WAVES - 1) / (4 * TINY_WAVES));
-			hipLaunchKernelGGL(k_dp_tiny, dim3(nb), dim3(64 * TINY_WAVES), 0, st, ntiny, d_order_tiny, pool1, off1, len1, pool2, off2, len2, ops, ops_off, ops_len, jfrag, frag);
-		}
-		if (nsmall > 0) {
-			const unsigned nb = (unsigned)((nsmall + SMALL_WAVES - 1) / SMALL_WAVES);
-			hipLaunchKernelGGL(k_dp_small, dim3(nb), dim3(64 * SMALL_WAVES), 0, st, nsmall, d_order, pool1, off1, len1, pool2, off2, len2, ops, ops_off, ops_len, jfrag, frag);
-		}
-		GSA_CHECK(c, hipGetLastError());
-		GSA_CHECK(c, hipEventRecord(ev_j2, st));
-		GSA_CHECK(c, hipStreamWaitEvent(c->stream_aux[1], ev_j2, 0));
-		out->small_in_flight = true;
-	} else
-	if (nsmall + ntiny > 0) {
-		GSA_CHECK(c, hipEventRecord(ev_fork, st));
-		GSA_CHECK(c, hipStreamWaitEvent(c->stream_aux[1], ev_fork, 0));
-		if (ntiny > 0) {
-			const unsigned nb = (unsigned)((ntiny + 4 * TINY_WAVES - 1) / (4 * TINY_WAVES));
-			hipLaunchKernelGGL(k_dp_tiny, dim3(nb), dim3(64 * TINY_WAVES), 0, c->stream_aux[1], ntiny, d_order_tiny, pool1, off1, len1, pool2, off2, len2, ops, ops_off, ops_len, jfrag, frag);
-		}
-		if (nsmall > 0) {
-			hipStream_t s2 = ntiny > 0 ? st : c->stream_aux[1];
-			const unsigned nb = (unsigned)((nsmall + SMALL_WAVES - 1) / SMALL_WAVES);
-			hipLaunchKernelGGL(k_dp_small, dim3(nb), dim3(64 * SMALL_WAVES), 0, s2, nsmall, d_order, pool1, off1, len1, pool2, off2, len2, ops, ops_off, ops_len, jfrag, frag);
+			launch_small(s2);
 			if (ntiny > 0) { GSA_CHECK(c, hipEventRecord(c->ev[18], s2)); GSA_CHECK(c, hipStreamWaitEvent(c->stream_aux[1], c->ev[18], 0)); }
 		}
 		GSA_CHECK(c, hipGetLastError());
```

Result: no change. 33.18 Gbp/s, median of 4 (+0.3%).
